# phoreproject/bls

Hardware: AMD Instinct MI355X
Metric: BLS12-381 pairings/sec (batch verify) (higher is better)
Workload: dtype int32 (14 x 28-bit limbs in the pairing / hash / curve kernels, 15 x 27 in the latency programs; int64 accumulate)

## Files before the change

bls_amd/csrc/fp.cuh:

```cuda
#pragma once
#include <hip/hip_runtime.h>
#include <stdint.h>

namespace blsmi {

typedef int32_t i32;
typedef int64_t i64;
typedef uint32_t u32;
typedef uint64_t u64;
typedef uint8_t u8;

#ifdef BLSMI_LIMBS28
constexpr int NL = 14;
constexpr int LB = 28;
constexpr int VU = 2;
constexpr int LMAX = 7;
constexpr int LPROD_MAX = 8;
constexpr int VPROD_MAX = 4096;
constexpr int VSTORE = 22;
#else
constexpr int NL = 15;
constexpr int LB = 27;
constexpr int VU = 1;
constexpr int LMAX = 15;
constexpr int LPROD_MAX = 33;
constexpr int VPROD_MAX = 1 << 23;
constexpr int VSTORE = 256;
#endif
constexpr i32 MASK = (1 << LB) - 1;
constexpr int VMAX = 1 << 12;
constexpr int VMUL = VU + (VU + 1) / 2;
constexpr int VRED = 2 * VU + 1;
#define BLSMI_DEV __device__ __forceinline__
#ifndef BLSMI_HASH_PRIO
#define BLSMI_HASH_PRIO 2
#endif
__device__ __forceinline__ void hash_prio() {
#if BLSMI_HASH_PRIO
    __builtin_amdgcn_s_setprio(BLSMI_HASH_PRIO);
#endif
}

#ifndef BLSMI_PAIR_YIELD_YOUNGER_STAYS
#define BLSMI_PAIR_YIELD_YOUNGER_STAYS 1
#endif
__device__ __forceinline__ void pair_yield_drop() {
#if BLSMI_PAIR_YIELD_YOUNGER_STAYS
    if ((__builtin_amdgcn_s_getreg(4) & 1) == 0)
#endif
        __builtin_amdgcn_s_setprio(0);
}

template <int L_, int V_>
struct Fp {
    static constexpr int L = L_, V = V_;
    i32 v[NL];
};
using FpS = Fp<1, VSTORE>;
using FpC = Fp<1, VU>;

}
#include "tower_fwd.cuh"
#ifdef BLSMI_LIMBS28
#include "consts28.cuh"
#else
#include "consts.cuh"
#endif
namespace blsmi {

template <int L2, int V2, int L, int V>
BLSMI_DEV Fp<L2, V2> fp_relabel(const Fp<L, V>& a) {
    static_assert(L2 >= L && V2 >= V, "relabel may only widen bounds");
    Fp<L2, V2> r;
#pragma unroll
    for (int i = 0; i < NL; i++) r.v[i] = a.v[i];
    return r;
}

template <int L, int V>
BLSMI_DEV Fp<1, V> fp_norm(const Fp<L, V>& x) {
    static_assert(L <= LMAX, "limb bound exceeded before norm");
    Fp<1, V> r;
    if constexpr (L == 1) {
#pragma unroll
        for (int i = 0; i < NL; i++) r.v[i] = x.v[i];
    } else {
        r.v[0] = x.v[0] & MASK;
#pragma unroll
        for (int i = 1; i < NL - 1; i++) r.v[i] = (x.v[i] & MASK) + (x.v[i - 1] >> LB);
        r.v[NL - 1] = x.v[NL - 1] + (x.v[NL - 2] >> LB);
    }
    return r;
}
template <bool C, int L, int V>
BLSMI_DEV auto fp_norm_if(const Fp<L, V>& x) {
    if constexpr (C) return fp_norm(x); else return x;
}

template <int La, int Va, int Lb, int Vb>
BLSMI_DEV auto fp_add(const Fp<La, Va>& a, const Fp<Lb, Vb>& b) {
    if constexpr (La + Lb > LMAX) {
        if constexpr (La >= Lb) return fp_add(fp_norm(a), fp_norm_if<(1 + Lb > LMAX)>(b));
        else return fp_add(fp_norm_if<(La + 1 > LMAX)>(a), fp_norm(b));
    } else {
        static_assert(Va + Vb <= VMAX, "value bound exceeded: insert fp_reduce");
        Fp<La + Lb, Va + Vb> r;
#pragma unroll
        for (int i = 0; i < NL; i++) r.v[i] = a.v[i] + b.v[i];
        return r;
    }
}
template <int La, int Va, int Lb, int Vb>
BLSMI_DEV auto fp_sub(const Fp<La, Va>& a, const Fp<Lb, Vb>& b) {
    if constexpr (La + Lb > LMAX) {
        if constexpr (La >= Lb) return fp_sub(fp_norm(a), fp_norm_if<(1 + Lb > LMAX)>(b));
        else return fp_sub(fp_norm_if<(La + 1 > LMAX)>(a), fp_norm(b));
    } else {
        static_assert(Va + Vb <= VMAX, "value bound exceeded: insert fp_reduce");
        Fp<La + Lb, Va + Vb> r;
#pragma unroll
        for (int i = 0; i < NL; i++) r.v[i] = a.v[i] - b.v[i];
        return r;
    }
}
template <int L, int V>
BLSMI_DEV Fp<L, V> fp_neg(const Fp<L, V>& a) {
    Fp<L, V> r;
#pragma unroll
    for (int i = 0; i < NL; i++) r.v[i] = -a.v[i];
    return r;
}
template <int K, int L, int V>
BLSMI_DEV auto fp_muls(const Fp<L, V>& a) {
    if constexpr (K > LMAX) {
        static_assert(K % 4 == 0 && K / 4 <= LMAX, "factor the constant");
        return fp_muls<K / 4>(fp_norm(fp_muls<4>(a)));
    } else if constexpr (L * K > LMAX) return fp_muls<K>(fp_norm(a));
    else {
        static_assert(V * K <= VMAX, "value bound exceeded: insert fp_reduce");
        Fp<L * K, V * K> r;
#pragma unroll
        for (int i = 0; i < NL; i++) r.v[i] = a.v[i] * K;
        return r;
    }
}
template <int L, int V> BLSMI_DEV auto fp_dbl(const Fp<L, V>& a) { return fp_muls<2>(a); }

template <int L, int V>
BLSMI_DEV Fp<1, VRED> fp_reduce(const Fp<L, V>& x) {
    static_assert(V <= VMAX, "value bound exceeded");
    static_assert(L <= LMAX, "limb bound exceeded before reduce");
    const Fp<L, V>& y = x;
    const float top = (float)y.v[NL - 1] * (float)(1 << LB) + (float)y.v[NL - 2];
    const i32 k = (i32)floorf(top * BLSMI_Q_TOP2_INV);
    Fp<1, VRED> r;
    i64 c = 0;
#pragma unroll
    for (int i = 0; i < NL - 1; i++) {
        c += (i64)y.v[i] - (i64)k * C_Q[i];
        r.v[i] = (i32)c & MASK;
        c >>= LB;
    }
    c += (i64)y.v[NL - 1] - (i64)k * C_Q[NL - 1];
    r.v[NL - 1] = (i32)c;
    return r;
}
template <int VT, int L, int V>
BLSMI_DEV auto fp_fit(const Fp<L, V>& x) {
    if constexpr (V <= VT) return x; else { static_assert(VRED <= VT, "no reduction can make this operand fit"); return fp_reduce(x); }
}
constexpr int isqrt_floor(int n) { int r = 0; while ((long long)(r + 1) * (r + 1) <= n) r++; return r; }
typedef i32 vlimbs __attribute__((ext_vector_type(NL)));

BLSMI_DEV vlimbs fp_mul_body(vlimbs a, vlimbs b) {
    i32 m[NL];
    vlimbs r;
    i64 acc = 0;
#pragma unroll
    for (int k = 0; k < NL; k++) {
#pragma unroll
        for (int i = 0; i <= k; i++) acc += (i64)a[i] * b[k - i];
#pragma unroll
        for (int i = 0; i < k; i++) acc += (i64)m[i] * C_Q[k - i];
        m[k] = (i32)((u32)(i32)acc * BLSMI_QINV) & MASK;
        acc += (i64)m[k] * C_Q[0];
        acc >>= LB;
    }
#pragma unroll
    for (int k = NL; k < 2 * NL - 1; k++) {
#pragma unroll
        for (int i = k - NL + 1; i < NL; i++) acc += (i64)a[i] * b[k - i];
#pragma unroll
        for (int i = k - NL + 1; i < NL; i++) acc += (i64)m[i] * C_Q[k - i];
        r[k - NL] = (i32)acc & MASK;
        acc >>= LB;
    }
    r[NL - 1] = (i32)acc;
    return r;
}
BLSMI_DEV vlimbs fp_sqr_body(vlimbs a) {
    i32 m[NL], a2[NL];
    vlimbs r;
#pragma unroll
    for (int i = 0; i < NL; i++) a2[i] = a[i] * 2;
    i64 acc = 0;
#pragma unroll
    for (int k = 0; k < NL; k++) {
#pragma unroll
        for (int i = 0; 2 * i < k; i++) acc += (i64)a[i] * a2[k - i];
        if (k % 2 == 0) acc += (i64)a[k / 2] * a[k / 2];
#pragma unroll
        for (int i = 0; i < k; i++) acc += (i64)m[i] * C_Q[k - i];
        m[k] = (i32)((u32)(i32)acc * BLSMI_QINV) & MASK;
        acc += (i64)m[k] * C_Q[0];
        acc >>= LB;
    }
#pragma unroll
    for (int k = NL; k < 2 * NL - 1; k++) {
#pragma unroll
        for (int i = k - NL + 1; 2 * i < k; i++) acc += (i64)a[i] * a2[k - i];
        if (k % 2 == 0) acc += (i64)a[k / 2] * a[k / 2];
#pragma unroll
        for (int i = k - NL + 1; i < NL; i++) acc += (i64)m[i] * C_Q[k - i];
        r[k - NL] = (i32)acc & MASK;
        acc >>= LB;
    }
    r[NL - 1] = (i32)acc;
    return r;
}
__device__ __noinline__ vlimbs fp_mul_core(vlimbs a, vlimbs b) { return fp_mul_body(a, b); }
__device__ __noinline__ vlimbs fp_sqr_core(vlimbs a) { return fp_sqr_body(a); }

template <int La, int Va, int Lb, int Vb>
BLSMI_DEV auto fp_mul(const Fp<La, Va>& a, const Fp<Lb, Vb>& b) {
    if constexpr (La * Lb > LPROD_MAX) {
        if constexpr (La >= Lb) return fp_mul(fp_norm(a), b);
        else return fp_mul(a, fp_norm(b));
    } else if constexpr ((long long)Va * Vb > VPROD_MAX) {
        if constexpr (Va >= Vb) return fp_mul(fp_reduce(a), b); else return fp_mul(a, fp_reduce(b));
    } else {
        vlimbs x, y;
#pragma unroll
        for (int i = 0; i < NL; i++) { x[i] = a.v[i]; y[i] = b.v[i]; }
        vlimbs z = fp_mul_core(x, y);
        Fp<1, VMUL> r;
#pragma unroll
        for (int i = 0; i < NL; i++) r.v[i] = z[i];
        return r;
    }
}
template <int L, int V>
BLSMI_DEV auto fp_sqr(const Fp<L, V>& a) {
    if constexpr (2 * L * L > LPROD_MAX) return fp_sqr(fp_norm(a));
    else if constexpr ((long long)V * V > VPROD_MAX) return fp_sqr(fp_reduce(a));
    else {
        vlimbs x;
#pragma unroll
        for (int i = 0; i < NL; i++) x[i] = a.v[i];
        vlimbs z = fp_sqr_core(x);
        Fp<1, VMUL> r;
#pragma unroll
        for (int i = 0; i < NL; i++) r.v[i] = z[i];
        return r;
    }
}

template <int L, int V>
BLSMI_DEV FpS fp_store(const Fp<L, V>& x) {
    if constexpr (V > FpS::V) return fp_relabel<1, FpS::V>(fp_reduce(x));
    else return fp_relabel<1, FpS::V>(fp_norm(x));
}

BLSMI_DEV void limbs_addsub_q(const i32 in[NL], i32 out[NL], i32 addmask, i32 submask) {
    i32 c = 0;
#pragma unroll
    for (int i = 0; i < NL; i++) {
        const i32 s = in[i] + (C_Q[i] & addmask) - (C_Q[i] & submask) + c;
        out[i] = (i < NL - 1) ? (s & MASK) : s;
        c = s >> LB;
    }
}
template <int L, int V>
BLSMI_DEV FpC fp_canon(const Fp<L, V>& x) {
    Fp<1, VRED> r = fp_reduce(x);
    i32 t[NL], d[NL];
    limbs_addsub_q(r.v, t, r.v[NL - 1] >> 31, 0);
#pragma unroll
    for (int pass = 0; pass < 2; pass++) {
        limbs_addsub_q(t, d, 0, -1);
        const i32 lt = d[NL - 1] >> 31;
#pragma unroll
        for (int i = 0; i < NL; i++) t[i] = (t[i] & lt) | (d[i] & ~lt);
    }
    FpC o;
#pragma unroll
    for (int i = 0; i < NL; i++) o.v[i] = t[i];
    return o;
}
template <int L, int V>
BLSMI_DEV bool fp_is_zero(const Fp<L, V>& x) {
    FpC c = fp_canon(x);
    i32 o = 0;
#pragma unroll
    for (int i = 0; i < NL; i++) o |= c.v[i];
    return o == 0;
}
template <int La, int Va, int Lb, int Vb>
BLSMI_DEV bool fp_eq(const Fp<La, Va>& a, const Fp<Lb, Vb>& b) { return fp_is_zero(fp_sub(a, b)); }

template <int L, int V>
BLSMI_DEV Fp<L, V> fp_select(i32 m, const Fp<L, V>& a, const Fp<L, V>& b) {
    Fp<L, V> r;
#pragma unroll
    for (int i = 0; i < NL; i++) r.v[i] = (a.v[i] & m) | (b.v[i] & ~m);
    return r;
}
BLSMI_DEV FpS fp_zero() {
    FpS r;
// ... 249 lines not shown
```

bls_amd/csrc/fp2_pair.inc:

```

template <int L_, int V_> struct Fp2 { static constexpr int L = L_, V = V_; Fp<L_, V_> c; };
template <int L_, int V_> struct Fp6 { static constexpr int L = L_, V = V_; Fp2<L_, V_> c0, c1, c2; };
template <int L_, int V_> struct Fp12 { static constexpr int L = L_, V = V_; Fp6<L_, V_> c0, c1; };
using Fp2S = Fp2<FpS::L, FpS::V>;
using Fp6S = Fp6<FpS::L, FpS::V>;
using Fp12S = Fp12<FpS::L, FpS::V>;

BLSMI_DEV i32 lane_odd() { return -(i32)(threadIdx.x & 1); }
BLSMI_DEV i32 bfi(i32 mask, i32 a, i32 b) {
    i32 r;
    asm("v_bfi_b32 %0, %1, %2, %3" : "=v"(r) : "v"(mask), "v"(a), "v"(b));
    return r;
}
BLSMI_DEV i32 dpp_swap(i32 x) { return __builtin_amdgcn_update_dpp(0, x, 0xB1, 0xf, 0xf, true); }
BLSMI_DEV i32 dpp_even(i32 x) { return __builtin_amdgcn_update_dpp(0, x, 0xA0, 0xf, 0xf, true); }
BLSMI_DEV i32 dpp_odd(i32 x) { return __builtin_amdgcn_update_dpp(0, x, 0xF5, 0xf, 0xf, true); }
template <int L, int V> BLSMI_DEV Fp<L, V> fp_partner(const Fp<L, V>& a) {
    Fp<L, V> r;
#pragma unroll
    for (int i = 0; i < NL; i++) r.v[i] = dpp_swap(a.v[i]);
    return r;
}
template <int L, int V> BLSMI_DEV Fp<L, V> fp_cneg(i32 m, const Fp<L, V>& a) {
    Fp<L, V> r;
#pragma unroll
    for (int i = 0; i < NL; i++) r.v[i] = (a.v[i] ^ m) - m;
    return r;
}
template <int L, int V> BLSMI_DEV Fp2<L, V> wrap(const Fp<L, V>& c) { Fp2<L, V> r; r.c = c; return r; }

template <int L2, int V2, int L, int V>
BLSMI_DEV Fp2<L2, V2> fp2_relabel(const Fp2<L, V>& a) { return wrap(fp_relabel<L2, V2>(a.c)); }
template <int La, int Va, int Lb, int Vb> BLSMI_DEV auto fp2_add(const Fp2<La, Va>& a, const Fp2<Lb, Vb>& b) { return wrap(fp_add(a.c, b.c)); }
template <int La, int Va, int Lb, int Vb> BLSMI_DEV auto fp2_sub(const Fp2<La, Va>& a, const Fp2<Lb, Vb>& b) { return wrap(fp_sub(a.c, b.c)); }
template <int L, int V> BLSMI_DEV auto fp2_neg(const Fp2<L, V>& a) { return wrap(fp_neg(a.c)); }
template <int L, int V> BLSMI_DEV auto fp2_dbl(const Fp2<L, V>& a) { return wrap(fp_dbl(a.c)); }
template <int K, int L, int V> BLSMI_DEV auto fp2_muls(const Fp2<L, V>& a) { return wrap(fp_muls<K>(a.c)); }
template <int L, int V> BLSMI_DEV auto fp2_conj(const Fp2<L, V>& a) { return wrap(fp_cneg(lane_odd(), a.c)); }
template <int L, int V> BLSMI_DEV auto fp2_norm(const Fp2<L, V>& a) { return wrap(fp_norm(a.c)); }
template <int L, int V> BLSMI_DEV Fp2S fp2_store(const Fp2<L, V>& a) { return wrap(fp_store(a.c)); }
template <int L, int V> BLSMI_DEV bool fp2_is_zero(const Fp2<L, V>& a) {
    const int z = fp_is_zero(a.c) ? 1 : 0;
    return (z & __shfl_xor(z, 1)) != 0;
}
template <int La, int Va, int Lb, int Vb> BLSMI_DEV bool fp2_eq(const Fp2<La, Va>& a, const Fp2<Lb, Vb>& b) { return fp2_is_zero(fp2_sub(a, b)); }
template <int L, int V> BLSMI_DEV Fp2<L, V> fp2_select(i32 m, const Fp2<L, V>& a, const Fp2<L, V>& b) { return wrap(fp_select(m, a.c, b.c)); }
BLSMI_DEV Fp2S fp2_zero() { return wrap(fp_zero()); }
BLSMI_DEV Fp2S fp2_one() { return wrap(fp_select(lane_odd(), fp_zero(), fp_one())); }
#undef BLSMI_FP2_K
#define BLSMI_FP2_K(x) fp2_pair_const(x)
#undef BLSMI_FP4_SQR_BY_PRODUCTS
#ifndef BLSMI_FP4_SQR_PAIR
#define BLSMI_FP4_SQR_PAIR 1
#endif
#define BLSMI_FP4_SQR_BY_PRODUCTS BLSMI_FP4_SQR_PAIR
BLSMI_DEV Fp2S fp2_pair_const(const blsmi::Fp2S& k) { return wrap(fp_select(lane_odd(), FpS(k.c1), FpS(k.c0))); }

BLSMI_DEV Fp2S fp2_table_load(const i32* t, int e) {
    const i32* src = t + (2 * e + (threadIdx.x & 1)) * NL_IO;
    FpS r;
#pragma unroll
    for (int i = 0; i < NL; i++) r.v[i] = src[i];
    return wrap(r);
}
BLSMI_DEV void fp2_table_store(i32* t, int e, const Fp2S& a) {
    i32* dst = t + (2 * e + (threadIdx.x & 1)) * NL_IO;
#pragma unroll
    for (int i = 0; i < NL; i++) dst[i] = a.c.v[i];
}
BLSMI_DEV void fp2_table_to_limbs27(i32* t, int e) {
    i32 w[NL_IO];
    fp_to_limbs27(fp2_table_load(t, e).c, w);
    i32* dst = t + (2 * e + (threadIdx.x & 1)) * NL_IO;
#pragma unroll
    for (int i = 0; i < NL_IO; i++) dst[i] = w[i];
}
template <int L, int V> BLSMI_DEV auto fp2_mul_nr(const Fp2<L, V>& a) { return wrap(fp_add(a.c, fp_cneg(~lane_odd(), fp_partner(a.c)))); }

BLSMI_DEV vlimbs fp2p_mul_body(vlimbs am, vlimbs bm, i32 odd) {
    vlimbs ao, p, q;
    const i32 zero = 0;
#pragma unroll
    for (int i = 0; i < NL; i++) {
        ao[i] = dpp_swap(am[i]);
        p[i] = dpp_even(bm[i]);
        q[i] = bfi(odd, bm[i], zero - dpp_swap(bm[i]));
    }
    i32 m[NL];
    vlimbs r;
    i64 acc = 0;
#pragma unroll
    for (int k = 0; k < NL; k++) {
#pragma unroll
        for (int i = 0; i <= k; i++) { acc += (i64)am[i] * p[k - i]; acc += (i64)ao[i] * q[k - i]; }
#pragma unroll
        for (int i = 0; i < k; i++) acc += (i64)m[i] * C_Q[k - i];
        m[k] = (i32)((u32)(i32)acc * BLSMI_QINV) & MASK;
        acc += (i64)m[k] * C_Q[0];
        acc >>= LB;
    }
#pragma unroll
    for (int k = NL; k < 2 * NL - 1; k++) {
#pragma unroll
        for (int i = k - NL + 1; i < NL; i++) { acc += (i64)am[i] * p[k - i]; acc += (i64)ao[i] * q[k - i]; }
#pragma unroll
        for (int i = k - NL + 1; i < NL; i++) acc += (i64)m[i] * C_Q[k - i];
        r[k - NL] = (i32)acc & MASK;
        acc >>= LB;
    }
    r[NL - 1] = (i32)acc;
    return r;
}
#ifdef BLSMI_ASM_CORES
typedef i32 v16i __attribute__((ext_vector_type(16)));
BLSMI_DEV vlimbs fp2p_mul_core(vlimbs a, vlimbs b) BLSMI_CORE_MUL2_STMT(a, b)
#elif defined(BLSMI_PAIR_CORE_INLINE)
BLSMI_DEV vlimbs fp2p_mul_core(vlimbs am, vlimbs bm) { return fp2p_mul_body(am, bm, lane_odd()); }
#else
__device__ __noinline__ vlimbs fp2p_mul_core(vlimbs am, vlimbs bm) { return fp2p_mul_body(am, bm, lane_odd()); }
#endif
BLSMI_DEV vlimbs fp2p_sqr_body(vlimbs am, i32 odd) {
    vlimbs x, y;
#pragma unroll
    for (int i = 0; i < NL; i++) {
        const i32 ao = dpp_swap(am[i]);
        x[i] = am[i] + bfi(odd, am[i], ao);
        y[i] = bfi(odd, ao, am[i] - ao);
    }
    return fp_mul_body(x, y);
}
#ifdef BLSMI_ASM_CORES
BLSMI_DEV vlimbs fp2p_sqr_core(vlimbs a) BLSMI_CORE_SQR2_STMT(a)
#else
__device__ __noinline__ vlimbs fp2p_sqr_core(vlimbs am) { return fp2p_sqr_body(am, lane_odd()); }
#endif
constexpr int LPROD_MAX2 = LPROD_MAX / 2;
template <int La, int Va, int Lb, int Vb>
BLSMI_DEV auto fp2_mul(const Fp2<La, Va>& a, const Fp2<Lb, Vb>& b) {
    if constexpr (La * Lb > LPROD_MAX2) {
        if constexpr (La >= Lb) return fp2_mul(fp2_norm(a), b);
        else return fp2_mul(a, fp2_norm(b));
    } else if constexpr (2LL * Va * Vb > VPROD_MAX) {
        if constexpr (Va >= Vb) return fp2_mul(wrap(fp_reduce(a.c)), b); else return fp2_mul(a, wrap(fp_reduce(b.c)));
    } else {
        vlimbs x, y;
#pragma unroll
        for (int i = 0; i < NL; i++) { x[i] = a.c.v[i]; y[i] = b.c.v[i]; }
        const vlimbs z = fp2p_mul_core(x, y);
        Fp2<1, VMUL> r;
#pragma unroll
        for (int i = 0; i < NL; i++) r.c.v[i] = z[i];
        return r;
    }
}
#ifdef BLSMI_PAIR_CORE_INLINE
__device__ __noinline__ vlimbs fp2p_mul_core_out(vlimbs am, vlimbs bm) { return fp2p_mul_body(am, bm, lane_odd()); }
template <int La, int Va, int Lb, int Vb>
BLSMI_DEV auto fp2_mul_call(const Fp2<La, Va>& a, const Fp2<Lb, Vb>& b) {
    if constexpr (La * Lb > LPROD_MAX2) {
        if constexpr (La >= Lb) return fp2_mul_call(fp2_norm(a), b);
        else return fp2_mul_call(a, fp2_norm(b));
    } else if constexpr (2LL * Va * Vb > VPROD_MAX) {
        if constexpr (Va >= Vb) return fp2_mul_call(wrap(fp_reduce(a.c)), b); else return fp2_mul_call(a, wrap(fp_reduce(b.c)));
    } else {
        vlimbs x, y;
#pragma unroll
        for (int i = 0; i < NL; i++) { x[i] = a.c.v[i]; y[i] = b.c.v[i]; }
        const vlimbs z = fp2p_mul_core_out(x, y);
        Fp2<1, VMUL> r;
#pragma unroll
        for (int i = 0; i < NL; i++) r.c.v[i] = z[i];
        return r;
    }
}
#else
template <int La, int Va, int Lb, int Vb> BLSMI_DEV auto fp2_mul_call(const Fp2<La, Va>& a, const Fp2<Lb, Vb>& b) { return fp2_mul(a, b); }
#endif
template <int L, int V>
BLSMI_DEV auto fp2_sqr(const Fp2<L, V>& a) {
    if constexpr (4 * L * L > LPROD_MAX) return fp2_sqr(fp2_norm(a));
    else if constexpr (4LL * V * V > VPROD_MAX) return fp2_sqr(wrap(fp_reduce(a.c)));
    else {
        vlimbs x;
#pragma unroll
        for (int i = 0; i < NL; i++) x[i] = a.c.v[i];
        const vlimbs z = fp2p_sqr_core(x);
        Fp2<1, VMUL> r;
#pragma unroll
        for (int i = 0; i < NL; i++) r.c.v[i] = z[i];
        return r;
    }
}
template <int La, int Va, int Lb, int Vb>
// ... 77 lines not shown
```

bls_amd/csrc/fp2_single.inc:

```
template <int La, int Va, int Lb, int Vb>
BLSMI_DEV auto make_fp2(const Fp<La, Va>& a, const Fp<Lb, Vb>& b) {
    constexpr int L = imax(La, Lb), V = imax(Va, Vb);
    Fp2<L, V> r;
    r.c0 = fp_relabel<L, V>(a);
    r.c1 = fp_relabel<L, V>(b);
    return r;
}
template <int L2, int V2, int L, int V>
BLSMI_DEV Fp2<L2, V2> fp2_relabel(const Fp2<L, V>& a) {
    Fp2<L2, V2> r;
    r.c0 = fp_relabel<L2, V2>(a.c0);
    r.c1 = fp_relabel<L2, V2>(a.c1);
    return r;
}
template <int La, int Va, int Lb, int Vb> BLSMI_DEV auto fp2_add(const Fp2<La, Va>& a, const Fp2<Lb, Vb>& b) { return make_fp2(fp_add(a.c0, b.c0), fp_add(a.c1, b.c1)); }
template <int La, int Va, int Lb, int Vb> BLSMI_DEV auto fp2_sub(const Fp2<La, Va>& a, const Fp2<Lb, Vb>& b) { return make_fp2(fp_sub(a.c0, b.c0), fp_sub(a.c1, b.c1)); }
template <int L, int V> BLSMI_DEV auto fp2_neg(const Fp2<L, V>& a) { return make_fp2(fp_neg(a.c0), fp_neg(a.c1)); }
template <int L, int V> BLSMI_DEV auto fp2_dbl(const Fp2<L, V>& a) { return make_fp2(fp_dbl(a.c0), fp_dbl(a.c1)); }
template <int K, int L, int V> BLSMI_DEV auto fp2_muls(const Fp2<L, V>& a) { return make_fp2(fp_muls<K>(a.c0), fp_muls<K>(a.c1)); }
template <int L, int V> BLSMI_DEV auto fp2_conj(const Fp2<L, V>& a) { return make_fp2(a.c0, fp_neg(a.c1)); }
template <int L, int V> BLSMI_DEV auto fp2_norm(const Fp2<L, V>& a) { return make_fp2(fp_norm(a.c0), fp_norm(a.c1)); }
template <int L, int V> BLSMI_DEV Fp2S fp2_store(const Fp2<L, V>& a) { Fp2S r; r.c0 = fp_store(a.c0); r.c1 = fp_store(a.c1); return r; }
template <int L, int V> BLSMI_DEV bool fp2_is_zero(const Fp2<L, V>& a) { return fp_is_zero(a.c0) & fp_is_zero(a.c1); }
template <int La, int Va, int Lb, int Vb> BLSMI_DEV bool fp2_eq(const Fp2<La, Va>& a, const Fp2<Lb, Vb>& b) { return fp2_is_zero(fp2_sub(a, b)); }
template <int L, int V> BLSMI_DEV Fp2<L, V> fp2_select(i32 m, const Fp2<L, V>& a, const Fp2<L, V>& b) { Fp2<L, V> r; r.c0 = fp_select(m, a.c0, b.c0); r.c1 = fp_select(m, a.c1, b.c1); return r; }
BLSMI_DEV Fp2S fp2_zero() { Fp2S r; r.c0 = fp_zero(); r.c1 = fp_zero(); return r; }
BLSMI_DEV Fp2S fp2_one() { Fp2S r; r.c0 = fp_one(); r.c1 = fp_zero(); return r; }

template <int L, int V> BLSMI_DEV auto fp2_mul_nr(const Fp2<L, V>& a) { return make_fp2(fp_sub(a.c0, a.c1), fp_add(a.c0, a.c1)); }
template <int La, int Va, int Lb, int Vb>
BLSMI_DEV auto fp2_mul(const Fp2<La, Va>& a, const Fp2<Lb, Vb>& b) {
    const auto aa = fp_mul(a.c0, b.c0);
    const auto bb = fp_mul(a.c1, b.c1);
    const auto t = fp_mul(fp_add(a.c0, a.c1), fp_add(b.c0, b.c1));
    return make_fp2(fp_sub(aa, bb), fp_sub(fp_sub(t, aa), bb));
}
template <int L, int V>
BLSMI_DEV auto fp2_sqr(const Fp2<L, V>& a) {
    const auto ab = fp_mul(a.c0, a.c1);
    const auto c0 = fp_mul(fp_add(a.c0, a.c1), fp_sub(a.c0, a.c1));
    return make_fp2(c0, fp_dbl(ab));
}
template <int La, int Va, int Lb, int Vb>
BLSMI_DEV auto fp2_mul_fp(const Fp2<La, Va>& a, const Fp<Lb, Vb>& s) { return make_fp2(fp_mul(a.c0, s), fp_mul(a.c1, s)); }
template <int L, int V>
BLSMI_DEV auto fp2_inv(const Fp2<L, V>& a) {
    const FpS t = fp_inv(fp_add(fp_sqr(a.c0), fp_sqr(a.c1)));
    return make_fp2(fp_mul(a.c0, t), fp_neg(fp_mul(a.c1, t)));
}
template <int P, int L, int V>
BLSMI_DEV auto fp2_frob(const Fp2<L, V>& a) {
    if constexpr (P % 2 == 0) return a; else return fp2_conj(a);
}

template <int L, int V>
BLSMI_DEV Fp2S fp2_pow_const(const Fp2<L, V>& a, const u32* ebits, int nbits) {
    const Fp2S base = fp2_store(a);
    Fp2S res = base;
    for (int i = nbits - 2; i >= 0; i--) {
        res = fp2_store(fp2_sqr(res));
        if ((ebits[i >> 5] >> (i & 31)) & 1) res = fp2_store(fp2_mul(res, base));
    }
    return res;
}
template <int L, int V>
BLSMI_DEV Fp2S fp2_sqrt(const Fp2<L, V>& a_in, bool& ok) {
    const Fp2S a = fp2_store(a_in);
    const bool zero = fp2_is_zero(a);
    const Fp2S a1 = fp2_pow_const(a, C_QM3O4, BLSMI_QM3O4_BITS);
    const Fp2S alpha = fp2_store(fp2_mul(fp2_sqr(a1), a));
    const Fp2S a0 = fp2_store(fp2_mul(fp2_conj(alpha), alpha));
    Fp2S neg1; neg1.c0 = C_NEGONE; neg1.c1 = fp_zero();
    const bool nonres = fp2_eq(a0, neg1);
    const Fp2S x0 = fp2_store(fp2_mul(a1, a));
    const bool alpha_m1 = fp2_eq(alpha, neg1);
    Fp2S xu; xu.c0 = fp_store(fp_neg(x0.c1)); xu.c1 = x0.c0;
    const Fp2S b = fp2_pow_const(fp2_add(alpha, fp2_one()), C_QM1O2, BLSMI_QM1O2_BITS);
    const Fp2S xb = fp2_store(fp2_mul(b, x0));
    Fp2S r = fp2_select(alpha_m1 ? -1 : 0, xu, xb);
    r = fp2_select(zero ? -1 : 0, fp2_zero(), r);
    ok = zero | !nonres;
    return r;
}

template <int WAVE = 0>
BLSMI_DEV FpS fp2_norm_root(const Fp2S& a, FpS& n, bool& ok) {
    n = fp_store(fp_add(fp_sqr(a.c0), fp_sqr(a.c1)));
    FpS e;
    if constexpr (WAVE != 0) e = fp_pow_spread<WAVE>(n, C_QM3O4, BLSMI_QM3O4_BITS);
    else e = fp_pow_qm3o4(n);
    const FpS s = fp_store(fp_mul(e, n));
    ok = fp_eq(fp_sqr(s), n);
    return s;
}
template <int WAVE = 0>
BLSMI_DEV Fp2S fp2_sqrt_from_norm_root(const Fp2S& a, const FpS& s) {
    FpS d = fp_store(fp_mul(fp_add(a.c0, s), C_HALF));
    d = fp_select(fp_is_zero(d) ? -1 : 0, a.c0, d);
    FpS f;
    if constexpr (WAVE != 0) f = fp_pow_spread<WAVE>(d, C_QM3O4, BLSMI_QM3O4_BITS);
    else f = fp_pow_qm3o4(d);
    const FpS r = fp_store(fp_mul(f, d));
    const FpS h = fp_store(fp_mul(fp_mul(a.c1, f), C_HALF));
    const i32 plus = fp_eq(fp_sqr(r), d) ? -1 : 0;
    Fp2S x;
    x.c0 = fp_select(plus, r, fp_store(fp_neg(h)));
    x.c1 = fp_select(plus, h, r);
    return x;
}
template <int WAVE = 0, int L, int V>
BLSMI_DEV Fp2S fp2_sqrt_any(const Fp2<L, V>& a_in, bool& ok) {
    const Fp2S a = fp2_store(a_in);
    FpS n;
    const FpS s = fp2_norm_root<WAVE>(a, n, ok);
    return fp2_sqrt_from_norm_root<WAVE>(a, s);
}

BLSMI_DEV Fp2S fp2_table_load(const i32* t, int e) {
    Fp2S r;
#pragma unroll
    for (int i = 0; i < NL; i++) { r.c0.v[i] = t[(2 * e) * NL + i]; r.c1.v[i] = t[(2 * e + 1) * NL + i]; }
    return r;
}
BLSMI_DEV void fp2_table_store(i32* t, int e, const Fp2S& a) {
#pragma unroll
    for (int i = 0; i < NL; i++) { t[(2 * e) * NL + i] = a.c0.v[i]; t[(2 * e + 1) * NL + i] = a.c1.v[i]; }
}

#undef BLSMI_FP2_K
#define BLSMI_FP2_K(x) (x)
#undef BLSMI_FP4_SQR_BY_PRODUCTS
#define BLSMI_FP4_SQR_BY_PRODUCTS 0
```

bls_amd/csrc/k_pairing_pair.hip:

```cpp
#include "pairing.cuh"
#include "device_io.cuh"

#define BLSMI_PAIR_MILLER_ONLY
#include "pair_kernels.inc"

template <int W2>
__device__ void pair_rec_load(FpS* c, const u64* p, size_t t, int par) { for (int j = 0; j < W2; j++) c[j] = load_m384(p + (size_t)6 * (2 * W2 * t + 2 * j + par)); }
template <int W2>
__device__ void pair_rec_store(u64* p, size_t t, int par, const FpS* c) { for (int j = 0; j < W2; j++) store_m384(p + (size_t)6 * (2 * W2 * t + 2 * j + par), c[j]); }
__global__ void __launch_bounds__(WG, BLSMI_PAIR_WAVES) k_debug_pairl(int op, const u64* a, const u64* b, u64* out, size_t n) {
    namespace P2 = blsmi::pairl;
    const int par = threadIdx.x & 1;
    const size_t t0 = (size_t)blockIdx.x * (WG / 2) + (threadIdx.x >> 1);
    const size_t t = t0 < n ? t0 : n - 1;
    if (op == BLSMI_OP_ROW_DBL_STEP || op == BLSMI_OP_ROW_ADD_STEP) {
        P2::Fp12S x; pair_rec_load<6>(reinterpret_cast<FpS*>(&x), a, t, par);
        P2::G2Proj r; r.x = x.c0.c0; r.y = x.c0.c1; r.z = x.c0.c2;
        const FpS px = load_m384(a + (size_t)6 * (12 * t + 10)), py = load_m384(a + (size_t)6 * (12 * t + 11));
        P2::Fp2S o0, o1, o2;
        if (op == BLSMI_OP_ROW_DBL_STEP) P2::doubling_step_h(r, o0, o1, o2); else P2::addition_step_h(r, x.c1.c0, x.c1.c1, o0, o1, o2);
        const FpS res[6] = {r.x.c, r.y.c, r.z.c, o2.c, P2::fp2_store(P2::fp2_mul_fp(o1, px)).c, P2::fp2_store(P2::fp2_mul_fp(o0, py)).c};
        if (t0 < n) pair_rec_store<6>(out, t, par, res);
        return;
    }
    if (op < 32) {
        P2::Fp2S x, y, r; pair_rec_load<1>(&x.c, a, t, par); y = x; if (b) pair_rec_load<1>(&y.c, b, t, par);
        switch (op) {
            case BLSMI_OP_FQ2_MUL: r = P2::fp2_store(P2::fp2_mul(x, y)); break;
            case BLSMI_OP_FQ2_SQR: r = P2::fp2_store(P2::fp2_sqr(x)); break;
            case BLSMI_OP_FQ2_INV: r = P2::fp2_store(P2::fp2_inv(x)); break;
            default: r = P2::fp2_store(P2::fp2_mul_nr(x)); break;
        }
        if (t0 < n) pair_rec_store<1>(out, t, par, &r.c);
    } else if (op < 48) {
        P2::Fp6S x, y, r; pair_rec_load<3>(reinterpret_cast<FpS*>(&x), a, t, par); y = x; if (b) pair_rec_load<3>(reinterpret_cast<FpS*>(&y), b, t, par);
        switch (op) {
            case BLSMI_OP_FQ6_MUL: r = P2::fp6_store(P2::fp6_mul(x, y)); break;
            case BLSMI_OP_FQ6_SQR: r = P2::fp6_store(P2::fp6_sqr(x)); break;
            case BLSMI_OP_FQ6_INV: r = P2::fp6_store(P2::fp6_inv(x)); break;
            case BLSMI_OP_FQ6_MUL_BY_1: r = P2::fp6_store(P2::fp6_mul_by_1(x, y.c0)); break;
            case BLSMI_OP_FQ6_MUL_BY_01: r = P2::fp6_store(P2::fp6_mul_by_01(x, y.c0, y.c1)); break;
            default: r = P2::fp6_store(P2::fp6_frob<1>(x)); break;
        }
        if (t0 < n) pair_rec_store<3>(out, t, par, reinterpret_cast<const FpS*>(&r));
    } else {
        P2::Fp12S x, y, r; pair_rec_load<6>(reinterpret_cast<FpS*>(&x), a, t, par); y = x; if (b) pair_rec_load<6>(reinterpret_cast<FpS*>(&y), b, t, par);
        switch (op) {
            case BLSMI_OP_FQ12_MUL: P2::nf_fp12_mul(r, x, y); break;
            case BLSMI_OP_FQ12_SQR: P2::nf_fp12_sqr(r, x); break;
            case BLSMI_OP_FQ12_INV: P2::nf_fp12_inv(r, x); break;
            case BLSMI_OP_FQ12_FROB1: P2::nf_fp12_frob1(r, x); break;
            case BLSMI_OP_FQ12_FROB2: P2::nf_fp12_frob2(r, x); break;
            case BLSMI_OP_FQ12_FROB3: P2::nf_fp12_frob3(r, x); break;
            case BLSMI_OP_FQ12_CYCLO_SQR: P2::nf_fp12_cyc_sqr(r, x); break;
            case BLSMI_OP_FQ12_CYCLO_RUN16: r = P2::cyc_sqr_run(x, 16); break;
            case BLSMI_OP_FQ12_MUL_BY_014: r = P2::fp12_store(P2::fp12_mul_by_014(x, y.c0.c0, y.c0.c1, y.c0.c2)); break;
            default: {
                const P2::LinePair m = P2::line_pair_product(y.c0.c0, y.c0.c1, y.c0.c2, y.c1.c0, y.c1.c1, y.c1.c2);
                r = P2::fp12_store(P2::fp12_mul_by_line_pair(x, m)); break;
            }
        }
        if (t0 < n) pair_rec_store<6>(out, t, par, reinterpret_cast<const FpS*>(&r));
    }
}
__global__ void __launch_bounds__(WG, 2) k_debug_prepare_pair(const u8* g2, i32* table) {
    namespace P2 = blsmi::pairl;
    if (threadIdx.x >= 2) return;
    const int par = threadIdx.x & 1;
    P2::prepare_lines(P2::wrap(load_be48(g2 + 48 * par)), P2::wrap(load_be48(g2 + 96 + 48 * par)), table);
    for (int e = 0; e < 68 * 3; e++) P2::fp2_table_to_limbs27(table, e);
}
__global__ void __launch_bounds__(WG, 2) k_prepare_generator_lines_pair(const u8* g2, i32* table) {
    namespace P2 = blsmi::pairl;
    if (threadIdx.x >= 2) return;
    const int par = threadIdx.x & 1;
    P2::prepare_lines(P2::wrap(load_be48(g2 + 48 * par)), P2::wrap(load_be48(g2 + 96 + 48 * par)), table);
}
```

bls_amd/csrc/k_wire.hip:

```cpp
#include "hash.cuh"
#include "device_io.cuh"
#include "subgroup.cuh"

BLSMI_DEV FpS load_be48_masked(const u8* p) {
    const u32* w32 = reinterpret_cast<const u32*>(p);
    u32 w[12];
#pragma unroll
    for (int j = 0; j < 12; j++) w[j] = __builtin_bswap32(w32[11 - j]);
    w[11] &= 0x1fffffffu;
    return fp_from_words(w);
}
struct WireRecord {
    using out_t = u8; static constexpr bool inf_optional = false;
    static BLSMI_DEV void put(u8* out, size_t t, const G1Aff& a) { store_g1(out + 96 * t, a); }
    static BLSMI_DEV void put(u8* out, size_t t, const G2Aff& a) { store_g2(out + 192 * t, a); }
};
struct JacRecord {
    using out_t = u64; static constexpr bool inf_optional = true;
    static BLSMI_DEV void put(u64* out, size_t t, const G1Aff& a) { store_jac_m384(out + 18 * t, a); }
    static BLSMI_DEV void put(u64* out, size_t t, const G2Aff& a) { store_jac_m384(out + 36 * t, a); }
};
template <bool WAVE, class W = WireRecord>
BLSMI_DEV void g1_decompress_body(const u8* in, int check, typename W::out_t* out, u8* out_inf, u8* err, size_t n) {
    const size_t t = WAVE ? (size_t)blockIdx.x : (size_t)blockIdx.x * WG + threadIdx.x;
// ... 9 lines not shown
    const i32 greatest = (b0 & 0x20) ? -1 : 0;
    G1Aff a; a.x = x; a.y = fp_select(lt ^ greatest, y, fp_store(fp_neg(y))); a.inf = 0;
    const bool sub = check == 2 ? in_subgroup_by_order(a) : check ? in_subgroup(a) : true;
    u8 e = 0; u8 inf = 0;
    if (!(b0 & 0x80)) e = 1;
    else if (b0 & 0x40) { if (rest) e = 2; else inf = 1; }
    else if (!ok) e = 3;
    else if (!sub) e = 4;
    if (t < n && (!WAVE || threadIdx.x == 0)) {
        a.inf = (inf || e) ? -1 : 0;
        W::put(out, t, a);
        if (!W::inf_optional || out_inf) out_inf[t] = inf;
        err[t] = e;
    }
}
KERNEL2 k_g1_decompress(const u8* in, int check, u8* out, u8* out_inf, u8* err, size_t n) { g1_decompress_body<false>(in, check, out, out_inf, err, n); }
KERNEL2 k_g1_decompress_jac(const u8* in, int check, u64* out, u8* out_inf, u8* err, size_t n) { g1_decompress_body<false, JacRecord>(in, check, out, out_inf, err, n); }
__global__ void __launch_bounds__(64, 2) k_g1_decompress_waves(const u8* in, u8* out, u8* out_inf, u8* err, size_t n) { g1_decompress_body<true>(in, 0, out, out_inf, err, n); }
template <bool WAVE, class W = WireRecord>
BLSMI_DEV void g2_decompress_body(const u8* in, int check, typename W::out_t* out, u8* out_inf, u8* err, size_t n) {
    const size_t t = WAVE ? (size_t)blockIdx.x : (size_t)blockIdx.x * WG + threadIdx.x;
    const size_t tt = t < n ? t : n - 1;
    const u8* c = in + 96 * tt;
    const u8 b0 = c[0];
    u32 rest = b0 & 0x3f;
    for (int i = 1; i < 96; i++) rest |= c[i];
    Fp2S x; x.c1 = load_be48_masked(c); x.c0 = load_be48(c + 48);
    bool ok;
    const Fp2S y = fp2_sqrt_any<WAVE>(fp2_add(fp2_mul(fp2_sqr(x), x), C_B2), ok);
    const i32 lt = ~fp2_sign_is_neg(y);
    const i32 greatest = (b0 & 0x20) ? -1 : 0;
    G2Aff a; a.x = x; a.y = fp2_select(lt ^ greatest, y, fp2_store(fp2_neg(y))); a.inf = 0;
    const bool sub = check == 2 ? in_subgroup_by_order(a) : check ? in_subgroup(a) : true;
    u8 e = 0; u8 inf = 0;
    if (!(b0 & 0x80)) e = 1;
    else if (b0 & 0x40) { if (rest) e = 2; else inf = 1; }
    else if (!ok) e = 3;
    else if (!sub) e = 4;
    if (t < n && (!WAVE || threadIdx.x == 0)) {
        a.inf = (inf || e) ? -1 : 0;
        W::put(out, t, a);
        if (!W::inf_optional || out_inf) out_inf[t] = inf;
        err[t] = e;
    }
}
KERNEL k_g2_decompress(const u8* in, int check, u8* out, u8* out_inf, u8* err, size_t n) { g2_decompress_body<false>(in, check, out, out_inf, err, n); }
KERNEL k_g2_decompress_jac(const u8* in, int check, u64* out, u8* out_inf, u8* err, size_t n) { g2_decompress_body<false, JacRecord>(in, check, out, out_inf, err, n); }
__global__ void __launch_bounds__(64) k_g2_decompress_waves(const u8* in, u8* out, u8* out_inf, u8* err, size_t n) { g2_decompress_body<true>(in, 0, out, out_inf, err, n); }
KERNEL k_apply_subgroup(const u8* in_subgroup, u8* out, int rec_words, const u8* out_inf, u8* err, size_t n) {
    const size_t t = (size_t)blockIdx.x * WG + threadIdx.x;
    if (t >= n || err[t] || out_inf[t] || in_subgroup[t]) return;
    err[t] = 4;
    u32* w = reinterpret_cast<u32*>(out) + (size_t)rec_words * t;
    for (int i = 0; i < rec_words; i++) w[i] = 0;
}
KERNEL k_merge_flags(const u8* inf_pk, const u8* err_pk, const u8* inf_sig, const u8* err_sig, u8* flags, size_t n) {
    const size_t t = (size_t)blockIdx.x * WG + threadIdx.x;
    if (t < n) flags[t] = (u8)(((inf_pk[t] | err_pk[t]) ? 1 : 0) | ((inf_sig[t] | err_sig[t]) ? 2 : 0));
}
KERNEL k_flag_zero_records(const u8* pks, int pk_words, const u8* sigs, int sig_words, const u8* in_flags, u8* flags, int* any, size_t n) {
    const size_t t = (size_t)blockIdx.x * WG + threadIdx.x;
    if (t >= n) return;
    u32 a = 0, b = 1;
    const u32* p = reinterpret_cast<const u32*>(pks) + (size_t)pk_words * t;
    for (int i = 0; i < pk_words; i++) a |= p[i];
    if (sigs) {
        b = 0;
        const u32* q = reinterpret_cast<const u32*>(sigs) + (size_t)sig_words * t;
        for (int i = 0; i < sig_words; i++) b |= q[i];
    }
    const u8 f = (u8)((in_flags ? in_flags[t] : 0) | (a ? 0 : 1) | (b ? 0 : 2));
    flags[t] = f;
    if (f && any) atomicOr(any, 1);
}
KERNEL k_flag_to_byte(const i32* flag, u8* out) { if (blockIdx.x == 0 && threadIdx.x == 0) *out = *flag ? 1 : 0; }
KERNEL k_pack_bitmap(const u8* ok, u8* bitmap, size_t n) {
    const size_t b = (size_t)blockIdx.x * WG + threadIdx.x;
    if (8 * b >= n) return;
    u32 v = 0;
    for (int i = 0; i < 8; i++) if (8 * b + i < n && ok[8 * b + i]) v |= 1u << i;
    bitmap[b] = (u8)v;
}
KERNEL k_g1_compress(const u8* pts, const u8* in_inf, u8* out, size_t n) {
    const size_t t = (size_t)blockIdx.x * WG + threadIdx.x;
    if (t >= n) return;
    u8* o = out + 48 * t;
    if (in_inf && in_inf[t]) { for (int i = 0; i < 48; i++) o[i] = 0; o[0] = 0xc0; return; }
    const u8* p = pts + 96 * t;
    for (int i = 0; i < 48; i++) o[i] = p[i];
    const FpS y = load_be48(p + 48);
    o[0] |= 0x80 | (fp_gt_half(y) ? 0x20 : 0);
}
KERNEL k_g2_compress(const u8* pts, const u8* in_inf, u8* out, size_t n) {
    const size_t t = (size_t)blockIdx.x * WG + threadIdx.x;
    if (t >= n) return;
    u8* o = out + 96 * t;
    if (in_inf && in_inf[t]) { for (int i = 0; i < 96; i++) o[i] = 0; o[0] = 0xc0; return; }
    const u8* p = pts + 192 * t;
    for (int i = 0; i < 48; i++) { o[i] = p[48 + i]; o[48 + i] = p[i]; }
    Fp2S y; y.c0 = load_be48(p + 96); y.c1 = load_be48(p + 144);
    o[0] |= 0x80 | (fp2_sign_is_neg(y) ? 0x20 : 0);
}

template <class F, int PB>
BLSMI_DEV void jac_to_affine_body(const u64* in, u8* out, u8* out_inf, size_t n) {
    constexpr int NC = sizeof(F) / sizeof(FpS);
    const size_t t = (size_t)blockIdx.x * WG + threadIdx.x;
    const size_t tt = t < n ? t : n - 1;
    bool z_one;
    const Jac<F> j = load_jac_m384<F>(in + (size_t)18 * NC * tt, &z_one);
    Aff<F> a;
    if (__all(z_one || j.inf)) { a.x = j.x; a.y = j.y; a.inf = j.inf; }
    else a = jac_to_affine(j);
    if (t < n) {
        if constexpr (NC == 1) store_g1(out + (size_t)PB * t, a); else store_g2(out + (size_t)PB * t, a);
        if (out_inf) out_inf[t] = a.inf ? 1 : 0;
    }
}
KERNEL2 k_g1_jac_to_affine(const u64* in, u8* out, u8* out_inf, size_t n) { jac_to_affine_body<FpS, 96>(in, out, out_inf, n); }
KERNEL k_g2_jac_to_affine(const u64* in, u8* out, u8* out_inf, size_t n) { jac_to_affine_body<Fp2S, 192>(in, out, out_inf, n); }
template <class F>
BLSMI_DEV void compress_jac_body(const u64* in, u8* out, size_t n) {
    constexpr int NC = sizeof(F) / sizeof(FpS);
    const size_t t = (size_t)blockIdx.x * WG + threadIdx.x;
    const size_t tt = t < n ? t : n - 1;
    bool z_one;
    const Jac<F> j = load_jac_m384<F>(in + (size_t)18 * NC * tt, &z_one);
    Aff<F> a;
    if (__all(z_one || j.inf)) { a.x = j.x; a.y = j.y; a.inf = j.inf; }
    else a = jac_to_affine(j);
    if (t >= n) return;
    u8* o = out + (size_t)48 * NC * t;
    if constexpr (NC == 1) store_wire48(o, a.x, a.inf, a.inf ? 0xc0u : 0x80u | (fp_gt_half(a.y) ? 0x20u : 0u));
    else {
        store_wire48(o, a.x.c1, a.inf, a.inf ? 0xc0u : 0x80u | (fp2_sign_is_neg(a.y) ? 0x20u : 0u));
        store_wire48(o + 48, a.x.c0, a.inf, 0u);
    }
}
KERNEL2 k_g1_compress_jac(const u64* in, u8* out, size_t n) { compress_jac_body<FpS>(in, out, n); }
KERNEL k_g2_compress_jac(const u64* in, u8* out, size_t n) { compress_jac_body<Fp2S>(in, out, n); }
KERNEL k_affine_to_jac(const u8* in, const void* in_inf, int inf_u8, int group, u64* out, size_t n) {
    const size_t t = (size_t)blockIdx.x * WG + threadIdx.x;
    if (t >= n) return;
    const bool inf = in_inf && (inf_u8 ? static_cast<const u8*>(in_inf)[t] != 0 : static_cast<const i32*>(in_inf)[t] != 0);
    if (group == 1) { G1Aff a = load_g1(in + 96 * t); if (inf) a.inf = -1; store_jac_m384(out + 18 * t, a); }
    else { G2Aff a = load_g2(in + 192 * t); if (inf) a.inf = -1; store_jac_m384(out + 36 * t, a); }
}

KERNEL k_debug_fq(int op, const u64* a, const u64* b, u64* out, u8* flag, size_t n) {
    const size_t t = (size_t)blockIdx.x * WG + threadIdx.x;
    if (t >= n) return;
    const FpS x = load_m384(a + 6 * t);
    FpS y = fp_zero();
    if (op == BLSMI_OP_FQ_MUL || op == BLSMI_OP_FQ_ADD || op == BLSMI_OP_FQ_SUB || op == BLSMI_OP_FQ_CMP) y = load_m384(b + 6 * t);
    FpS r = fp_zero();
    bool ok = true;
    int code = -1;
    switch (op) {
        case BLSMI_OP_FQ_DBL: r = fp_store(fp_dbl(x)); break;
        case BLSMI_OP_FQ_CMP: {
            u32 wx[12], wy[12];
            fp_to_words(x, wx); fp_to_words(y, wy);
            int c = 0;
            for (int j = 0; j < 12; j++) if (wx[j] != wy[j]) c = wx[j] > wy[j] ? 1 : -1;
            code = c + 1; r = x; break;
        }
        case BLSMI_OP_FQ_PARITY: code = fp_gt_half(x) ? 1 : 0; r = x; break;
        case BLSMI_OP_FQ_MUL: r = fp_store(fp_mul(x, y)); break;
        case BLSMI_OP_FQ_SQR: r = fp_store(fp_sqr(x)); break;
        case BLSMI_OP_FQ_ADD: r = fp_store(fp_add(x, y)); break;
        case BLSMI_OP_FQ_SUB: r = fp_store(fp_sub(x, y)); break;
        case BLSMI_OP_FQ_NEG: r = fp_store(fp_neg(x)); break;
        case BLSMI_OP_FQ_INV: r = fp_inv(x); ok = !fp_is_zero(x); break;
        case BLSMI_OP_FQ_SQRT: r = fp_sqrt(x, ok); break;
    }
    store_m384(out + 6 * t, r);
    if (flag) flag[t] = code >= 0 ? (u8)code : (ok ? 1 : 0);
}
KERNEL k_debug_fq2(int op, const u64* a, const u64* b, u64* out, u8* flag, size_t n) {
    const size_t t = (size_t)blockIdx.x * WG + threadIdx.x;
    if (t >= n) return;
    Rec<2> ra = rec_load<2>(a, t), rb = ra, ro;
    if (op == BLSMI_OP_FQ2_MUL) rb = rec_load<2>(b, t);
    const Fp2S x = as<Fp2S>(ra), y = as<Fp2S>(rb);
    Fp2S r = fp2_zero();
    bool ok = true;
    switch (op) {
        case BLSMI_OP_FQ2_MUL: r = fp2_store(fp2_mul(x, y)); break;
        case BLSMI_OP_FQ2_SQR: r = fp2_store(fp2_sqr(x)); break;
        case BLSMI_OP_FQ2_INV: r = fp2_store(fp2_inv(x)); ok = !fp2_is_zero(x); break;
        case BLSMI_OP_FQ2_MUL_NR: r = fp2_store(fp2_mul_nr(x)); break;
        case BLSMI_OP_FQ2_SQRT: r = fp2_sqrt(x, ok); break;
        case BLSMI_OP_FQ2_SQRT_ANY: r = fp2_sqrt_any(x, ok); break;
        case BLSMI_OP_FQ2_PARITY: ok = fp2_sign_is_neg(x) != 0; r = x; break;
    }
    as<Fp2S>(ro) = r;
    rec_store<2>(out, t, ro);
    if (flag) flag[t] = ok ? 1 : 0;
}
KERNEL2 k_debug_swu_g1(const u64* a, u64* out, size_t n) {
    const size_t t = (size_t)blockIdx.x * WG + threadIdx.x;
    if (t >= n) return;
    Rec<3> r = rec_load<3>(a, t);
    G1Aff p; swu_g1_helper(p, reinterpret_cast<FpS*>(&r)[0]);
    reinterpret_cast<FpS*>(&r)[0] = p.x; reinterpret_cast<FpS*>(&r)[1] = p.y; reinterpret_cast<FpS*>(&r)[2] = fp_zero();
    rec_store<3>(out, t, r);
}
KERNEL k_debug_swu_g2(const u64* a, u64* out, size_t n) {
    const size_t t = (size_t)blockIdx.x * WG + threadIdx.x;
    if (t >= n) return;
    Rec<6> r = rec_load<6>(a, t);
    G2Aff p; swu_g2_helper(p, reinterpret_cast<Fp2S*>(&r)[0]);
    reinterpret_cast<Fp2S*>(&r)[0] = p.x; reinterpret_cast<Fp2S*>(&r)[1] = p.y; reinterpret_cast<Fp2S*>(&r)[2] = fp2_zero();
    rec_store<6>(out, t, r);
}
```

bls_amd/csrc/pair_kernels.inc:

```
#ifndef BLSMI_PAIR_WAVES
#define BLSMI_PAIR_WAVES 2
#endif
#define KERNEL_PAIR __global__ void __launch_bounds__(WG, BLSMI_PAIR_WAVES)
namespace P2 = blsmi::pairl;
struct PairG1 { FpS x, y; };
struct PairG2 { P2::Fp2S x, y; };
constexpr int PT = WG / 2;

#ifndef BLSMI_PAIR_YIELD
#define BLSMI_PAIR_YIELD 1
#endif
#ifndef BLSMI_PAIR_YIELD_MILLER
#define BLSMI_PAIR_YIELD_MILLER 50
#endif
#ifndef BLSMI_PAIR_YIELD_FE
#define BLSMI_PAIR_YIELD_FE 4
#endif
constexpr int PAIR_YIELD_MILLER_BITS = BLSMI_PAIR_YIELD ? BLSMI_PAIR_YIELD_MILLER : 0;
constexpr int PAIR_YIELD_FE_EXP_X = BLSMI_PAIR_YIELD_FE;
BLSMI_DEV void pair_yield_enter() {
#if BLSMI_PAIR_YIELD
    __builtin_amdgcn_s_setprio(1);
#endif
}
struct PairYieldOps : P2::Fp12Ops {
    static BLSMI_DEV void before_exp_x(int k) { if (k == PAIR_YIELD_FE_EXP_X) pair_yield_drop(); }
};
BLSMI_DEV void final_exponentiation_yield(P2::Fp12S& f) {
#if BLSMI_PAIR_YIELD
    P2::final_exp_chain<PairYieldOps>(f);
#else
    P2::final_exponentiation(f);
#endif
}

#ifdef BLSMI_WAVE_CENSUS
constexpr int CENSUS_WAVES = 4096, CENSUS_WORDS = 4;
#ifdef BLSMI_PAIR_FE_ONLY
#define BLSMI_CENSUS_BUF blsmi_census_fe
#define BLSMI_CENSUS_READ blsmi_census_read_fe
#else
#define BLSMI_CENSUS_BUF blsmi_census_miller
#define BLSMI_CENSUS_READ blsmi_census_read_miller
#endif
__device__ unsigned long long BLSMI_CENSUS_BUF[CENSUS_WAVES * CENSUS_WORDS];
extern "C" __attribute__((visibility("default"))) int BLSMI_CENSUS_READ(unsigned long long* out) {
    return (int)hipMemcpyFromSymbol(out, HIP_SYMBOL(BLSMI_CENSUS_BUF), sizeof(BLSMI_CENSUS_BUF));
}
struct WaveCensus {
    u64 t0;
    BLSMI_DEV WaveCensus() : t0(__builtin_amdgcn_s_memrealtime()) {}
    BLSMI_DEV void leave(int kernel) const {
        const u64 t1 = __builtin_amdgcn_s_memrealtime();
        const u32 hw = __builtin_amdgcn_s_getreg(4 | (31 << 11)), xcc = __builtin_amdgcn_s_getreg(20 | (31 << 11));
        if (threadIdx.x == 0 && blockIdx.x < CENSUS_WAVES) {
            unsigned long long* rec = BLSMI_CENSUS_BUF + (size_t)blockIdx.x * CENSUS_WORDS;
            rec[0] = (u64)hw | ((u64)xcc << 32); rec[1] = t0; rec[2] = t1; rec[3] = (u64)kernel + 1;
        }
    }
};
#else
struct WaveCensus { BLSMI_DEV void leave(int) const {} };
#endif

template <int WORDS>
BLSMI_DEV void tile_load_pair(u32* lds, const u8* gbase, size_t first, size_t n) {
    const u32* g = reinterpret_cast<const u32*>(gbase) + first * WORDS;
    const size_t valid = (n - first < (size_t)PT ? n - first : (size_t)PT) * WORDS;
    for (int idx = threadIdx.x; idx < PT * WORDS; idx += WG)
        if ((size_t)idx < valid) lds[(idx / WORDS) * (WORDS + 1) + (idx % WORDS)] = g[idx];
    __syncthreads();
}
template <int WORDS>
BLSMI_DEV void tile_store_pair(const u32* lds, u8* gbase, size_t first, size_t n) {
    __syncthreads();
    u32* g = reinterpret_cast<u32*>(gbase) + first * WORDS;
    const size_t valid = (n - first < (size_t)PT ? n - first : (size_t)PT) * WORDS;
    for (int idx = threadIdx.x; idx < PT * WORDS; idx += WG)
        if ((size_t)idx < valid) g[idx] = lds[(idx / WORDS) * (WORDS + 1) + (idx % WORDS)];
}
BLSMI_DEV void pair_store12(i32* buf, size_t n, size_t t, int par, const P2::Fp12S& f) {
    const FpS* c = reinterpret_cast<const FpS*>(&f);
#pragma unroll
    for (int j = 0; j < 6; j++) soa_store(buf, n, t, 2 * j + par, c[j]);
}
BLSMI_DEV P2::Fp12S pair_load12(const i32* buf, size_t n, size_t t, int par) {
    P2::Fp12S f;
    FpS* c = reinterpret_cast<FpS*>(&f);
#pragma unroll
    for (int j = 0; j < 6; j++) c[j] = soa_load(buf, n, t, 2 * j + par);
    return f;
}
#ifndef BLSMI_PAIR_FE_ONLY
template <bool EXACT> BLSMI_DEV void miller1_pair_body(const u8* g1, const u8* g2, i32* fbuf, size_t n) {
    __shared__ u32 lds[PT * 49];
    const int par = threadIdx.x & 1, loc = threadIdx.x >> 1;
    const size_t first = (size_t)blockIdx.x * PT;
    const size_t t = first + loc;
    const int rec = (t < n) ? loc : (int)(n - 1 - first);
    PairG1 p[1]; PairG2 q[1];
    const WaveCensus census;
    pair_yield_enter();
    tile_load_pair<24>(lds, g1, first, n);
    p[0].x = lds_be48(lds + rec * 25); p[0].y = lds_be48(lds + rec * 25 + 12);
    __syncthreads();
    tile_load_pair<48>(lds, g2, first, n);
    q[0].x = P2::wrap(lds_be48(lds + rec * 49 + 12 * par));
    q[0].y = P2::wrap(lds_be48(lds + rec * 49 + 24 + 12 * par));
    P2::Fp12S f;
    if constexpr (EXACT) P2::miller_loop<1, false, EXACT, false, PAIR_YIELD_MILLER_BITS>(f, p, q);
    else {
        __shared__ i32 lds_r[45 * WG];
        __syncthreads();
        P2::miller_loop<1, false, EXACT, false, PAIR_YIELD_MILLER_BITS>(f, p, q, nullptr, nullptr, lds_r);
    }
    if (t < n) pair_store12(fbuf, n, t, par, f);
    census.leave(0);
}
KERNEL_PAIR k_miller1_pair(const u8* g1, const u8* g2, i32* fbuf, size_t n) { miller1_pair_body<true>(g1, g2, fbuf, n); }
KERNEL_PAIR k_miller1h_pair(const u8* g1, const u8* g2, i32* fbuf, size_t n) { miller1_pair_body<false>(g1, g2, fbuf, n); }
#endif
#ifndef BLSMI_PAIR_MILLER_ONLY
KERNEL_PAIR k_final_exp_pair(const i32* fbuf, u64* out, size_t n, int mode) {
    __shared__ u32 lds[PT * 145];
    const int par = threadIdx.x & 1, loc = threadIdx.x >> 1;
    const size_t first = (size_t)blockIdx.x * PT;
    const size_t t = first + loc;
    const size_t tt = t < n ? t : n - 1;
    const WaveCensus census;
    pair_yield_enter();
    P2::Fp12S f = pair_load12(fbuf, n, tt, par);
    if (mode == 0) final_exponentiation_yield(f);
    const FpS* c = reinterpret_cast<const FpS*>(&f);
    for (int j = 0; j < 6; j++) {
        u32 w[12];
        fp_to_mont384_words(c[j], w);
#pragma unroll
        for (int k = 0; k < 12; k++) lds[loc * 145 + 12 * (2 * j + par) + k] = w[k];
    }
    tile_store_pair<144>(lds, reinterpret_cast<u8*>(out), first, n);
    census.leave(1);
}
#endif
#ifndef BLSMI_PAIR_FE_ONLY

KERNEL_PAIR k_miller1x2_pair(const u8* g1, const u8* g2, i32* fbuf, size_t n, size_t m) {
    const int par = threadIdx.x & 1;
    const size_t t = (size_t)blockIdx.x * PT + (threadIdx.x >> 1);
    const size_t tt = t < m ? t : m - 1;
    const size_t i0 = 2 * tt, i1 = 2 * tt + 1 < n ? 2 * tt + 1 : i0;
    PairG1 p[2]; PairG2 q[2];
    p[0].x = load_be48(g1 + 96 * i0); p[0].y = load_be48(g1 + 96 * i0 + 48);
    p[1].x = load_be48(g1 + 96 * i1); p[1].y = load_be48(g1 + 96 * i1 + 48);
    q[0].x = P2::wrap(load_be48(g2 + 192 * i0 + 48 * par)); q[0].y = P2::wrap(load_be48(g2 + 192 * i0 + 96 + 48 * par));
    q[1].x = P2::wrap(load_be48(g2 + 192 * i1 + 48 * par)); q[1].y = P2::wrap(load_be48(g2 + 192 * i1 + 96 + 48 * par));
    P2::Fp12S f;
    __shared__ i32 lds_r[45 * WG];
    if (__all(2 * tt + 1 < n)) P2::miller_loop<2, false, false>(f, p, q, nullptr, nullptr, lds_r);
    else {
        P2::Fp12S f2, f1;
        P2::miller_loop<2, false, false>(f2, p, q, nullptr, nullptr, lds_r);
        PairG1 p1[1] = {p[0]}; PairG2 q1[1] = {q[0]};
        P2::miller_loop<1, false, false>(f1, p1, q1, nullptr, nullptr, lds_r);
        const i32 both = 2 * tt + 1 < n ? -1 : 0;
        FpS* a = reinterpret_cast<FpS*>(&f2); const FpS* b = reinterpret_cast<const FpS*>(&f1);
        for (int j = 0; j < 6; j++) a[j] = fp_select(both, a[j], b[j]);
        f = f2;
    }
    if (t < m) pair_store12(fbuf, m, t, par, f);
}

KERNEL_PAIR k_miller2_pair(const u8* p0, size_t sp0, const u8* q0, size_t sq0, const u8* p1, size_t sp1, const u8* q1, size_t sq1, i32* fbuf, size_t n, const i32* pre) {
    __shared__ u32 lds[PT * 49];
    const int par = threadIdx.x & 1, loc = threadIdx.x >> 1;
    const size_t first = (size_t)blockIdx.x * PT;
    const size_t t = first + loc;
    const int rec = (t < n) ? loc : (int)(n - 1 - first);
    PairG1 p[2]; PairG2 q[2];
    const WaveCensus census;
    pair_yield_enter();
    if (sp0) { tile_load_pair<24>(lds, p0, first, n); p[0].x = lds_be48(lds + rec * 25); p[0].y = lds_be48(lds + rec * 25 + 12); __syncthreads(); }
    else { p[0].x = load_be48(p0); p[0].y = load_be48(p0 + 48); }
    if (sq0) { tile_load_pair<48>(lds, q0, first, n); q[0].x = P2::wrap(lds_be48(lds + rec * 49 + 12 * par)); q[0].y = P2::wrap(lds_be48(lds + rec * 49 + 24 + 12 * par)); __syncthreads(); }
    else { q[0].x = P2::wrap(load_be48(q0 + 48 * par)); q[0].y = P2::wrap(load_be48(q0 + 96 + 48 * par)); }
    tile_load_pair<24>(lds, p1, first, n);
    p[1].x = lds_be48(lds + rec * 25); p[1].y = fp_store(fp_neg(lds_be48(lds + rec * 25 + 12)));
    __syncthreads();
    tile_load_pair<48>(lds, q1, first, n);
    q[1].x = P2::wrap(lds_be48(lds + rec * 49 + 12 * par)); q[1].y = P2::wrap(lds_be48(lds + rec * 49 + 24 + 12 * par));
    (void)sp1; (void)sq1;
    P2::Fp12S f;
    __shared__ i32 lds_r[45 * WG];
    __syncthreads();
    if (pre) P2::miller_loop<2, true, false, false, PAIR_YIELD_MILLER_BITS>(f, p, q, pre, nullptr, lds_r);
    else P2::miller_loop<2, false, false, false, PAIR_YIELD_MILLER_BITS>(f, p, q, nullptr, nullptr, lds_r);
    if (t < n) pair_store12(fbuf, n, t, par, f);
    census.leave(2);
}
#endif
#ifndef BLSMI_PAIR_MILLER_ONLY
KERNEL_PAIR k_final_exp_is_one_pair(const i32* fbuf, const u8* inf_flags, u8* ok, size_t n) {
    const int par = threadIdx.x & 1, loc = threadIdx.x >> 1;
    const size_t t = (size_t)blockIdx.x * PT + loc;
    const size_t tt = t < n ? t : n - 1;
    const WaveCensus census;
    pair_yield_enter();
    P2::Fp12S f = pair_load12(fbuf, n, tt, par);
    final_exponentiation_yield(f);
    const bool one = P2::fp12_eq(f, P2::fp12_one());
    if (t < n && par == 0) ok[t] = (one && !(inf_flags && inf_flags[t])) ? 1 : 0;
    census.leave(3);
}
#endif
```

bls_amd/csrc/pairing_body.inc:

```

struct G2Proj { Fp2S x, y, z; };

BLSMI_NOINLINE void nf_fp12_mul(Fp12S& r, const Fp12S& a, const Fp12S& b) { r = fp12_store(fp12_mul(a, b)); }
BLSMI_NOINLINE void nf_fp12_sqr(Fp12S& r, const Fp12S& a) { r = fp12_store(fp12_sqr(a)); }
BLSMI_NOINLINE void nf_fp12_cyc_sqr(Fp12S& r, const Fp12S& a) { r = fp12_cyclotomic_sqr(a); }
BLSMI_NOINLINE void nf_fp12_inv(Fp12S& r, const Fp12S& a) { r = fp12_store(fp12_inv(a)); }
BLSMI_NOINLINE void nf_fp12_frob1(Fp12S& r, const Fp12S& a) { r = fp12_store(fp12_frob<1>(a)); }
BLSMI_NOINLINE void nf_fp12_frob2(Fp12S& r, const Fp12S& a) { r = fp12_store(fp12_frob<2>(a)); }
BLSMI_NOINLINE void nf_fp12_frob3(Fp12S& r, const Fp12S& a) { r = fp12_store(fp12_frob<3>(a)); }
BLSMI_DEV void fp12_conj_inplace(Fp12S& a) { a.c1 = fp6_store(fp6_neg(a.c1)); }

BLSMI_NOINLINE void doubling_step(G2Proj& r, Fp2S& o0, Fp2S& o1, Fp2S& o2) {
    const auto tmp0 = fp2_norm(fp2_sqr(r.x));
    const auto tmp1 = fp2_norm(fp2_sqr(r.y));
    const auto tmp2 = fp2_norm(fp2_sqr(tmp1));
    const auto tmp3 = fp2_norm(fp2_dbl(fp2_sub(fp2_sub(fp2_sqr(fp2_add(tmp1, r.x)), tmp0), tmp2)));
    const auto tmp4 = fp2_norm(fp2_muls<3>(tmp0));
    const auto tmp6 = fp2_norm(fp2_add(r.x, tmp4));
    const auto tmp5 = fp2_norm(fp2_sqr(tmp4));
    const auto zsq = fp2_norm(fp2_sqr(r.z));
    const auto nx = fp2_norm(fp2_sub(fp2_sub(tmp5, tmp3), tmp3));
    const auto nz = fp2_norm(fp2_sub(fp2_sub(fp2_sqr(fp2_add(r.z, r.y)), tmp1), zsq));
    const auto ny = fp2_norm(fp2_sub(fp2_mul(fp2_sub(tmp3, nx), tmp4), fp2_muls<8>(tmp2)));
    o1 = fp2_store(fp2_neg(fp2_dbl(fp2_mul(tmp4, zsq))));
    o2 = fp2_store(fp2_sub(fp2_sub(fp2_sub(fp2_sqr(tmp6), tmp0), tmp5), fp2_muls<4>(tmp1)));
    o0 = fp2_store(fp2_dbl(fp2_mul(nz, zsq)));
    r.x = fp2_store(nx); r.y = fp2_store(ny); r.z = fp2_store(nz);
}
BLSMI_NOINLINE void addition_step(G2Proj& r, const Fp2S& qx, const Fp2S& qy, Fp2S& o0, Fp2S& o1, Fp2S& o2) {
    const auto zsq = fp2_norm(fp2_sqr(r.z));
    const auto ysq = fp2_norm(fp2_sqr(qy));
    const auto t0 = fp2_norm(fp2_mul(zsq, qx));
    const auto t1 = fp2_norm(fp2_mul(fp2_sub(fp2_sub(fp2_sqr(fp2_add(qy, r.z)), ysq), zsq), zsq));
    const auto t2 = fp2_norm(fp2_sub(t0, r.x));
    const auto t3 = fp2_norm(fp2_sqr(t2));
    const auto t4 = fp2_norm(fp2_muls<4>(t3));
    const auto t5 = fp2_norm(fp2_mul(t4, t2));
    const auto t6 = fp2_norm(fp2_sub(fp2_sub(t1, r.y), r.y));
    const auto t9 = fp2_norm(fp2_mul(t6, qx));
    const auto t7 = fp2_norm(fp2_mul(t4, r.x));
    const auto nx = fp2_norm(fp2_sub(fp2_sub(fp2_sub(fp2_sqr(t6), t5), t7), t7));
    const auto nz = fp2_norm(fp2_sub(fp2_sub(fp2_sqr(fp2_add(r.z, t2)), zsq), t3));
    const auto t8 = fp2_norm(fp2_mul(fp2_sub(t7, nx), t6));
    const auto ny = fp2_norm(fp2_sub(t8, fp2_dbl(fp2_mul(r.y, t5))));
    const auto t10 = fp2_norm(fp2_sub(fp2_sub(fp2_sqr(fp2_add(qy, nz)), ysq), fp2_sqr(nz)));
    o2 = fp2_store(fp2_sub(fp2_dbl(t9), t10));
    o0 = fp2_store(fp2_dbl(nz));
    o1 = fp2_store(fp2_dbl(fp2_neg(t6)));
    r.x = fp2_store(nx); r.y = fp2_store(ny); r.z = fp2_store(nz);
}
BLSMI_DEV void doubling_step_h_i(G2Proj& r, Fp2S& o0, Fp2S& o1, Fp2S& o2) {
    const auto A = fp2_norm(fp2_mul(r.x, r.y));
    const auto B = fp2_norm(fp2_sqr(r.y));
    const auto X2 = fp2_norm(fp2_sqr(r.x));
    const auto H = fp2_norm(fp2_dbl(fp2_mul(r.y, r.z)));
    const auto E = fp2_norm(fp2_muls<12>(fp2_norm(fp2_mul_nr(fp2_norm(fp2_sqr(r.z))))));
    const auto F = fp2_norm(fp2_muls<3>(E));
    const auto G = fp2_norm(fp2_add(B, F));
    const auto nx = fp2_norm(fp2_dbl(fp2_mul(A, fp2_norm(fp2_sub(B, F)))));
    const auto ny = fp2_norm(fp2_sub(fp2_sqr(G), fp2_muls<12>(fp2_norm(fp2_sqr(E)))));
    const auto nz = fp2_norm(fp2_muls<4>(fp2_norm(fp2_mul(B, H))));
    o2 = fp2_store(fp2_sub(B, E));
    o1 = fp2_store(fp2_neg(fp2_muls<3>(X2)));
    o0 = fp2_store(H);
    r.x = fp2_store(nx); r.y = fp2_store(ny); r.z = fp2_store(nz);
}
BLSMI_NOINLINE void doubling_step_h(G2Proj& r, Fp2S& o0, Fp2S& o1, Fp2S& o2) { doubling_step_h_i(r, o0, o1, o2); }
BLSMI_NOINLINE void addition_step_h(G2Proj& r, const Fp2S& qx, const Fp2S& qy, Fp2S& o0, Fp2S& o1, Fp2S& o2) {
    const auto th = fp2_norm(fp2_sub(r.y, fp2_mul(qy, r.z)));
    const auto la = fp2_norm(fp2_sub(r.x, fp2_mul(qx, r.z)));
    const auto C = fp2_norm(fp2_sqr(th));
    const auto D = fp2_norm(fp2_sqr(la));
    const auto E = fp2_norm(fp2_mul(la, D));
    const auto F = fp2_norm(fp2_mul(r.z, C));
    const auto G = fp2_norm(fp2_mul(r.x, D));
    const auto Hh = fp2_norm(fp2_sub(fp2_add(E, F), fp2_dbl(G)));
    const auto nx = fp2_norm(fp2_mul(la, Hh));
    const auto ny = fp2_norm(fp2_sub(fp2_mul(th, fp2_norm(fp2_sub(G, Hh))), fp2_mul(E, r.y)));
    const auto nz = fp2_norm(fp2_mul(r.z, E));
    o2 = fp2_store(fp2_sub(fp2_mul(th, qx), fp2_mul(la, qy)));
    o1 = fp2_store(fp2_neg(th));
    o0 = fp2_store(la);
    r.x = fp2_store(nx); r.y = fp2_store(ny); r.z = fp2_store(nz);
}
template <bool EXACT> BLSMI_DEV void dbl_step(G2Proj& r, Fp2S& o0, Fp2S& o1, Fp2S& o2) {
    if constexpr (EXACT) doubling_step(r, o0, o1, o2); else doubling_step_h(r, o0, o1, o2);
}
template <bool EXACT> BLSMI_DEV void add_step(G2Proj& r, const Fp2S& qx, const Fp2S& qy, Fp2S& o0, Fp2S& o1, Fp2S& o2) {
    if constexpr (EXACT) addition_step(r, qx, qy, o0, o1, o2); else addition_step_h(r, qx, qy, o0, o1, o2);
}
BLSMI_NOINLINE void ell(Fp12S& f, const Fp2S& o0, const Fp2S& o1, const Fp2S& o2, const FpS& px, const FpS& py) {
    const auto c0 = fp2_mul_fp(o0, py);
    const auto c1 = fp2_mul_fp(o1, px);
    f = fp12_store(fp12_mul_by_014(f, o2, c1, c0));
}

BLSMI_NOINLINE void ell_sqr(Fp12S& f, const Fp2S& o0, const Fp2S& o1, const Fp2S& o2, const FpS& px, const FpS& py) {
    const auto c0 = fp2_mul_fp(o0, py);
    const auto c1 = fp2_mul_fp(o1, px);
    const Fp12S g = fp12_store(fp12_mul_by_014(f, o2, c1, c0));
    f = fp12_store(fp12_sqr(g));
}

template <bool SQR>
BLSMI_NOINLINE void ell2(Fp12S& f, const Fp2S& a0, const Fp2S& a1, const Fp2S& a2, const FpS& ax, const FpS& ay,
                         const Fp2S& b0, const Fp2S& b1, const Fp2S& b2, const FpS& bx, const FpS& by) {
    const LinePair m = line_pair_product(a2, fp2_mul_fp(a1, ax), fp2_mul_fp(a0, ay), b2, fp2_mul_fp(b1, bx), fp2_mul_fp(b0, by));
    const Fp12S g = fp12_store(fp12_mul_by_line_pair(f, m));
    if (SQR) f = fp12_store(fp12_sqr(g)); else f = g;
}

struct NoTick { BLSMI_DEV void operator()(int) const {} };
template <class Dbl, class Add, class Mul, class MulSqr, class Tick = NoTick>
BLSMI_DEV void x_bit_walk(Dbl dbl, Add add, Mul mul, MulSqr mul_sqr, Tick tick = Tick()) {
    const u64 xr = BLSMI_X_ABS >> 1;
    for (int i = 61; i >= 0; i--) {
        tick(61 - i);
        dbl();
        if ((xr >> i) & 1) { mul(); add(); }
        mul_sqr();
    }
    dbl();
    mul();
}

BLSMI_DEV void load_line(const i32* pre, int line, Fp2S& o0, Fp2S& o1, Fp2S& o2) {
    o0 = fp2_table_load(pre, 3 * line); o1 = fp2_table_load(pre, 3 * line + 1); o2 = fp2_table_load(pre, 3 * line + 2);
}
BLSMI_DEV void store_line(i32* table, int line, const Fp2S& o0, const Fp2S& o1, const Fp2S& o2) {
    fp2_table_store(table, 3 * line, o0); fp2_table_store(table, 3 * line + 1, o1); fp2_table_store(table, 3 * line + 2, o2);
}
BLSMI_DEV void lds_put_proj(i32* l, const G2Proj& r) {
    const FpS* c = reinterpret_cast<const FpS*>(&r);
#pragma unroll
    for (int j = 0; j < 3; j++)
#pragma unroll
        for (int i = 0; i < NL; i++) l[(j * NL + i) * 64 + threadIdx.x] = c[j].v[i];
}
BLSMI_DEV G2Proj lds_get_proj(const i32* l) {
    G2Proj r;
    FpS* c = reinterpret_cast<FpS*>(&r);
#pragma unroll
    for (int j = 0; j < 3; j++)
#pragma unroll
        for (int i = 0; i < NL; i++) c[j].v[i] = l[(j * NL + i) * 64 + threadIdx.x];
    return r;
}
template <int NP, bool PRE0 = false, bool EXACT = true, bool PRE1 = false, int YIELD = 0, class G1P, class G2P>
BLSMI_DEV void miller_loop(Fp12S& f, const G1P (&p)[NP], const G2P (&q)[NP], const i32* pre = nullptr, const i32* pre1 = nullptr, i32* lds_r = nullptr) {
    static_assert(NP == 1 || NP == 2, "one pair, or two pairs sharing the squarings");
    constexpr int LAST = NP - 1;
    constexpr bool PRE_LAST = NP == 1 ? PRE0 : PRE1;
    G2Proj r[NP];
#pragma unroll
    for (int k = 0; k < NP; k++) { r[k].x = q[k].x; r[k].y = q[k].y; r[k].z = fp2_one(); }
    f = fp12_one();
    const bool in_lds = !EXACT && !PRE_LAST && lds_r != nullptr;
    if (in_lds) lds_put_proj(lds_r, r[LAST]);
    auto dbl_last = [&](Fp2S& a0, Fp2S& a1, Fp2S& a2) {
        if (in_lds) { G2Proj t = lds_get_proj(lds_r); doubling_step_h_i(t, a0, a1, a2); lds_put_proj(lds_r, t); }
        else dbl_step<EXACT>(r[LAST], a0, a1, a2);
    };
    auto add_last = [&](Fp2S& a0, Fp2S& a1, Fp2S& a2) {
        if (in_lds) { G2Proj t = lds_get_proj(lds_r); add_step<EXACT>(t, q[LAST].x, q[LAST].y, a0, a1, a2); lds_put_proj(lds_r, t); }
        else add_step<EXACT>(r[LAST], q[LAST].x, q[LAST].y, a0, a1, a2);
    };
    Fp2S o0, o1, o2;
    int line = 0;
    auto tick = [](int done) {
        if constexpr (YIELD > 0) { if (done == YIELD) pair_yield_drop(); }
        else (void)done;
    };
    if constexpr (NP == 1) {
        x_bit_walk([&] { if (PRE0) load_line(pre, line++, o0, o1, o2); else dbl_last(o0, o1, o2); },
                   [&] { if (PRE0) load_line(pre, line++, o0, o1, o2); else add_last(o0, o1, o2); },
                   [&] { ell(f, o0, o1, o2, p[0].x, p[0].y); },
                   [&] { ell_sqr(f, o0, o1, o2, p[0].x, p[0].y); }, tick);
    } else {
        Fp2S n0, n1, n2;
        int line1 = 0;
        x_bit_walk([&] { if (PRE0) load_line(pre, line++, o0, o1, o2); else dbl_step<EXACT>(r[0], o0, o1, o2);
                         if (PRE1) load_line(pre1, line1++, n0, n1, n2); else dbl_last(n0, n1, n2); },
                   [&] { if (PRE0) load_line(pre, line++, o0, o1, o2); else add_step<EXACT>(r[0], q[0].x, q[0].y, o0, o1, o2);
                         if (PRE1) load_line(pre1, line1++, n0, n1, n2); else add_last(n0, n1, n2); },
                   [&] { ell2<false>(f, o0, o1, o2, p[0].x, p[0].y, n0, n1, n2, p[1].x, p[1].y); },
                   [&] { ell2<true>(f, o0, o1, o2, p[0].x, p[0].y, n0, n1, n2, p[1].x, p[1].y); }, tick);
    }
    fp12_conj_inplace(f);
}
BLSMI_DEV void prepare_lines(const Fp2S& qx, const Fp2S& qy, i32* table) {
    G2Proj r; r.x = qx; r.y = qy; r.z = fp2_one();
    Fp2S o0, o1, o2;
    int line = 0;
    x_bit_walk([&] { doubling_step(r, o0, o1, o2); store_line(table, line++, o0, o1, o2); },
               [&] { addition_step(r, qx, qy, o0, o1, o2); store_line(table, line++, o0, o1, o2); },
               [] {}, [] {});
}

template <class O>
BLSMI_DEV void exp_by_x_loop(typename O::T& out, const typename O::T& f, u64 e) {
    typename O::T res = f;
    int i = 62 - __builtin_clzll(e);
    while (i >= 0) {
        const u64 below = e & ((2ull << i) - 1);
        const int next = below ? 63 - __builtin_clzll(below) : -1;
        const int run = next < 0 ? i + 1 : i - next + 1;
        bool plain = true;
        if constexpr (O::MIN_RUN > 0)
            if (run >= O::MIN_RUN) { O::x_sqr_run(res, res, run); plain = false; }
        if (plain) for (int j = 0; j < run; j++) O::x_sqr(res, res);
        if (next >= 0) { typename O::T t = res; O::mul(t, t, f); res = t; }
        i = next - 1;
        if (next < 0) break;
    }
    O::conj(res);
    out = res;
}
template <class O, class = void> struct ExpXHook { static BLSMI_DEV void at(int) {} };
template <class O> struct ExpXHook<O, decltype(O::before_exp_x(0))> { static BLSMI_DEV void at(int k) { O::before_exp_x(k); } };
template <class O>
BLSMI_DEV void final_exp_chain(typename O::T& r) {
    typename O::T f2, y0, y1, y2, y3;
    O::inv(f2, r);
    O::conj(r);
    O::mul(r, r, f2);
    O::frob2(f2, r);
    O::mul(r, f2, r);
    const u64 x = BLSMI_X_ABS;
    O::cyc_sqr(y0, r);
    ExpXHook<O>::at(0); O::exp_x(y1, y0, x);
    ExpXHook<O>::at(1); O::exp_x(y2, y1, x >> 1);
    y3 = r; O::conj(y3);
    O::mul(y1, y1, y3);
    O::conj(y1);
    O::mul(y1, y1, y2);
    ExpXHook<O>::at(2); O::exp_x(y2, y1, x);
    ExpXHook<O>::at(3); O::exp_x(y3, y2, x);
    O::conj(y1);
    O::mul(y3, y3, y1);
    O::conj(y1);
    O::frob3(y1, y1);
    O::frob2(y2, y2);
    O::mul(y1, y1, y2);
    ExpXHook<O>::at(4); O::exp_x(y2, y3, x);
    O::mul(y2, y2, y0);
    O::mul(y2, y2, r);
    O::mul(y1, y1, y2);
    O::frob1(y3, y3);
    O::mul(r, y1, y3);
}

BLSMI_DEV Fp12S cyc_sqr_run(const Fp12S& g, int m) {
    CycCompressed c = cyc_compress(g);
    for (int j = 0; j < m; j++) c = cyc_compressed_sqr(c);
    Fp2S num, den;
    cyc_z1_fraction(c, num, den);
    return cyc_decompress(c, fp2_store(fp2_mul(num, fp2_store(fp2_inv(den)))));
}
BLSMI_NOINLINE void exp_by_x(Fp12S& out, const Fp12S& f, u64 e);
struct Fp12Ops {
    using T = Fp12S;
    static constexpr int MIN_RUN = 12;
    static BLSMI_DEV void inv(T& r, const T& a) { nf_fp12_inv(r, a); }
    static BLSMI_DEV void mul(T& r, const T& a, const T& b) { nf_fp12_mul(r, a, b); }
    static BLSMI_DEV void cyc_sqr(T& r, const T& a) { nf_fp12_cyc_sqr(r, a); }
    static BLSMI_DEV void x_sqr(T& r, const T& a) { r = fp12_cyclotomic_sqr(a); }
    static BLSMI_DEV void x_sqr_run(T& r, const T& a, int m) { r = cyc_sqr_run(a, m); }
    static BLSMI_DEV void frob1(T& r, const T& a) { nf_fp12_frob1(r, a); }
    static BLSMI_DEV void frob2(T& r, const T& a) { nf_fp12_frob2(r, a); }
    static BLSMI_DEV void frob3(T& r, const T& a) { nf_fp12_frob3(r, a); }
    static BLSMI_DEV void conj(T& a) { fp12_conj_inplace(a); }
    static BLSMI_DEV void exp_x(T& r, const T& a, u64 e) { exp_by_x(r, a, e); }
};
BLSMI_NOINLINE void exp_by_x(Fp12S& out, const Fp12S& f, u64 e) { exp_by_x_loop<Fp12Ops>(out, f, e); }
BLSMI_DEV void final_exponentiation(Fp12S& r) { final_exp_chain<Fp12Ops>(r); }
```

bls_amd/csrc/tower_body.inc:

```
template <int L2, int V2, int L, int V>
BLSMI_DEV Fp6<L2, V2> fp6_relabel(const Fp6<L, V>& a) {
    Fp6<L2, V2> r;
    r.c0 = fp2_relabel<L2, V2>(a.c0);
    r.c1 = fp2_relabel<L2, V2>(a.c1);
    r.c2 = fp2_relabel<L2, V2>(a.c2);
    return r;
}
template <int La, int Va, int Lb, int Vb, int Lc, int Vc>
BLSMI_DEV auto make_fp6(const Fp2<La, Va>& a, const Fp2<Lb, Vb>& b, const Fp2<Lc, Vc>& c) {
    constexpr int L = imax(La, imax(Lb, Lc)), V = imax(Va, imax(Vb, Vc));
    Fp6<L, V> r;
    r.c0 = fp2_relabel<L, V>(a);
    r.c1 = fp2_relabel<L, V>(b);
    r.c2 = fp2_relabel<L, V>(c);
    return r;
}
template <int La, int Va, int Lb, int Vb>
BLSMI_DEV auto make_fp12(const Fp6<La, Va>& a, const Fp6<Lb, Vb>& b) {
    constexpr int L = imax(La, Lb), V = imax(Va, Vb);
    Fp12<L, V> r;
    r.c0 = fp6_relabel<L, V>(a);
    r.c1 = fp6_relabel<L, V>(b);
    return r;
}

template <int La, int Va, int Lb, int Vb> BLSMI_DEV auto fp6_add(const Fp6<La, Va>& a, const Fp6<Lb, Vb>& b) { return make_fp6(fp2_add(a.c0, b.c0), fp2_add(a.c1, b.c1), fp2_add(a.c2, b.c2)); }
template <int La, int Va, int Lb, int Vb> BLSMI_DEV auto fp6_sub(const Fp6<La, Va>& a, const Fp6<Lb, Vb>& b) { return make_fp6(fp2_sub(a.c0, b.c0), fp2_sub(a.c1, b.c1), fp2_sub(a.c2, b.c2)); }
template <int L, int V> BLSMI_DEV auto fp6_neg(const Fp6<L, V>& a) { return make_fp6(fp2_neg(a.c0), fp2_neg(a.c1), fp2_neg(a.c2)); }
template <int L, int V> BLSMI_DEV auto fp6_norm(const Fp6<L, V>& a) { return make_fp6(fp2_norm(a.c0), fp2_norm(a.c1), fp2_norm(a.c2)); }
template <int L, int V> BLSMI_DEV Fp6S fp6_store(const Fp6<L, V>& a) { Fp6S r; r.c0 = fp2_store(a.c0); r.c1 = fp2_store(a.c1); r.c2 = fp2_store(a.c2); return r; }
BLSMI_DEV Fp6S fp6_zero() { Fp6S r; r.c0 = fp2_zero(); r.c1 = fp2_zero(); r.c2 = fp2_zero(); return r; }
BLSMI_DEV Fp6S fp6_one() { Fp6S r; r.c0 = fp2_one(); r.c1 = fp2_zero(); r.c2 = fp2_zero(); return r; }
template <int L, int V> BLSMI_DEV auto fp6_mul_nr(const Fp6<L, V>& a) { return make_fp6(fp2_mul_nr(a.c2), a.c0, a.c1); }
template <int La, int Va, int Lb, int Vb>
BLSMI_DEV auto fp6_mul(const Fp6<La, Va>& a, const Fp6<Lb, Vb>& b) {
    const auto aa = fp2_mul(a.c0, b.c0);
    const auto bb = fp2_mul(a.c1, b.c1);
    const auto cc = fp2_mul(a.c2, b.c2);
    const auto t1 = fp2_add(fp2_mul_nr(fp2_sub(fp2_sub(fp2_mul(fp2_add(b.c1, b.c2), fp2_add(a.c1, a.c2)), bb), cc)), aa);
    const auto t3 = fp2_sub(fp2_add(fp2_sub(fp2_mul(fp2_add(b.c0, b.c2), fp2_add(a.c0, a.c2)), aa), bb), cc);
    const auto t2 = fp2_add(fp2_sub(fp2_sub(fp2_mul(fp2_add(b.c0, b.c1), fp2_add(a.c0, a.c1)), aa), bb), fp2_mul_nr(cc));
    return make_fp6(t1, t2, t3);
}
template <int L, int V>
BLSMI_DEV auto fp6_sqr(const Fp6<L, V>& a) {
    const auto s0 = fp2_sqr(a.c0);
    const auto s1 = fp2_dbl(fp2_mul(a.c0, a.c1));
    const auto s2 = fp2_sqr(fp2_add(fp2_sub(a.c0, a.c1), a.c2));
    const auto s3 = fp2_dbl(fp2_mul(a.c1, a.c2));
    const auto s4 = fp2_sqr(a.c2);
    const auto c0 = fp2_add(fp2_mul_nr(s3), s0);
    const auto c1 = fp2_add(fp2_mul_nr(s4), s1);
    const auto c2 = fp2_sub(fp2_sub(fp2_add(fp2_add(s1, s2), s3), s0), s4);
    return make_fp6(c0, c1, c2);
}
template <int L, int V, int Lc, int Vc>
BLSMI_DEV auto fp6_mul_by_1(const Fp6<L, V>& a, const Fp2<Lc, Vc>& c1) {
    const auto b = fp2_mul(a.c1, c1);
    const auto t1 = fp2_mul_nr(fp2_sub(fp2_mul(c1, fp2_add(a.c1, a.c2)), b));
    const auto t2 = fp2_sub(fp2_mul(c1, fp2_add(a.c0, a.c1)), b);
    return make_fp6(t1, t2, b);
}
template <int L, int V, int L0, int V0, int L1, int V1>
BLSMI_DEV auto fp6_mul_by_01(const Fp6<L, V>& a, const Fp2<L0, V0>& c0, const Fp2<L1, V1>& c1) {
    const auto aa = fp2_mul(a.c0, c0);
    const auto b = fp2_mul(a.c1, c1);
    const auto t1 = fp2_add(fp2_mul_nr(fp2_sub(fp2_mul(c1, fp2_add(a.c1, a.c2)), b)), aa);
    const auto t3 = fp2_add(fp2_sub(fp2_mul(c0, fp2_add(a.c0, a.c2)), aa), b);
    const auto t2 = fp2_sub(fp2_sub(fp2_mul(fp2_add(c0, c1), fp2_add(a.c0, a.c1)), aa), b);
    return make_fp6(t1, t2, t3);
}
template <int L, int V>
BLSMI_DEV auto fp6_inv(const Fp6<L, V>& a) {
    const Fp2S c0 = fp2_store(fp2_add(fp2_neg(fp2_mul(fp2_mul_nr(a.c2), a.c1)), fp2_sqr(a.c0)));
    const Fp2S c1 = fp2_store(fp2_sub(fp2_mul_nr(fp2_sqr(a.c2)), fp2_mul(a.c0, a.c1)));
    const Fp2S c2 = fp2_store(fp2_sub(fp2_sqr(a.c1), fp2_mul(a.c0, a.c2)));
    auto t = fp2_mul_nr(fp2_add(fp2_mul(a.c2, c1), fp2_mul(a.c1, c2)));
    const Fp2S ti = fp2_store(fp2_inv(fp2_store(fp2_add(t, fp2_mul(a.c0, c0)))));
    return make_fp6(fp2_mul(ti, c0), fp2_mul(ti, c1), fp2_mul(ti, c2));
}
template <int P, int L, int V>
BLSMI_DEV auto fp6_frob(const Fp6<L, V>& a) {
    return make_fp6(fp2_frob<P>(a.c0), fp2_mul(fp2_frob<P>(a.c1), BLSMI_FP2_K(C_FROB6_C1[P % 6])), fp2_mul(fp2_frob<P>(a.c2), BLSMI_FP2_K(C_FROB6_C2[P % 6])));
}

template <int L, int V> BLSMI_DEV Fp12S fp12_store(const Fp12<L, V>& a) { Fp12S r; r.c0 = fp6_store(a.c0); r.c1 = fp6_store(a.c1); return r; }
BLSMI_DEV Fp12S fp12_one() { Fp12S r; r.c0 = fp6_one(); r.c1 = fp6_zero(); return r; }
template <int L, int V> BLSMI_DEV auto fp12_conj(const Fp12<L, V>& a) { return make_fp12(a.c0, fp6_neg(a.c1)); }
template <int La, int Va, int Lb, int Vb>
BLSMI_DEV auto fp12_mul(const Fp12<La, Va>& a, const Fp12<Lb, Vb>& b) {
    const auto aa = fp6_norm(fp6_mul(a.c0, b.c0));
    const auto bb = fp6_norm(fp6_mul(a.c1, b.c1));
    const auto t = fp6_mul(fp6_add(a.c1, a.c0), fp6_add(b.c0, b.c1));
    return make_fp12(fp6_add(fp6_mul_nr(bb), aa), fp6_sub(fp6_sub(t, aa), bb));
}
template <int L, int V>
BLSMI_DEV auto fp12_sqr(const Fp12<L, V>& a) {
    const auto ab = fp6_norm(fp6_mul(a.c0, a.c1));
    const auto t = fp6_mul(fp6_add(fp6_mul_nr(a.c1), a.c0), fp6_add(a.c0, a.c1));
    return make_fp12(fp6_sub(fp6_sub(t, ab), fp6_mul_nr(ab)), fp6_add(ab, ab));
}
template <int L, int V, int L0, int V0, int L1, int V1, int L4, int V4>
BLSMI_DEV auto fp12_mul_by_014(const Fp12<L, V>& a, const Fp2<L0, V0>& c0, const Fp2<L1, V1>& c1, const Fp2<L4, V4>& c4) {
    const auto aa = fp6_norm(fp6_mul_by_01(a.c0, c0, c1));
    const auto bb = fp6_norm(fp6_mul_by_1(a.c1, c4));
    const auto t = fp6_mul_by_01(fp6_add(a.c1, a.c0), c0, fp2_add(c1, c4));
    return make_fp12(fp6_add(fp6_mul_nr(bb), aa), fp6_sub(fp6_sub(t, aa), bb));
}
template <int L, int V>
BLSMI_DEV auto fp12_inv(const Fp12<L, V>& a) {
    const Fp6S t = fp6_store(fp6_inv(fp6_store(fp6_sub(fp6_sqr(a.c0), fp6_mul_nr(fp6_store(fp6_sqr(a.c1)))))));
    return make_fp12(fp6_mul(t, a.c0), fp6_neg(fp6_mul(t, a.c1)));
}
template <int P, int L, int V>
BLSMI_DEV auto fp12_frob(const Fp12<L, V>& a) {
    const auto c0 = fp6_frob<P>(a.c0);
    const auto c1 = fp6_frob<P>(a.c1);
    const Fp2S k = BLSMI_FP2_K(C_FROB12_C1[P % 12]);
    return make_fp12(c0, make_fp6(fp2_mul(fp2_store(c1.c0), k), fp2_mul(fp2_store(c1.c1), k), fp2_mul(fp2_store(c1.c2), k)));
}
struct LinePair { Fp2S l0, l1, l2, l4, l5; };
template <int L0, int V0, int L1, int V1, int L4, int V4, int M0, int W0, int M1, int W1, int M4, int W4>
BLSMI_DEV LinePair line_pair_product(const Fp2<L0, V0>& a0, const Fp2<L1, V1>& a1, const Fp2<L4, V4>& a4,
                                     const Fp2<M0, W0>& b0, const Fp2<M1, W1>& b1, const Fp2<M4, W4>& b4) {
    const auto p00 = fp2_norm(fp2_mul(a0, b0)), p11 = fp2_norm(fp2_mul(a1, b1)), p44 = fp2_norm(fp2_mul(a4, b4));
    LinePair r;
    r.l0 = fp2_store(fp2_add(p00, fp2_mul_nr(p44)));
    r.l1 = fp2_store(fp2_sub(fp2_sub(fp2_mul(fp2_add(a0, a1), fp2_add(b0, b1)), p00), p11));
    r.l2 = fp2_store(p11);
    r.l4 = fp2_store(fp2_sub(fp2_sub(fp2_mul(fp2_add(a0, a4), fp2_add(b0, b4)), p00), p44));
    r.l5 = fp2_store(fp2_sub(fp2_sub(fp2_mul(fp2_add(a1, a4), fp2_add(b1, b4)), p11), p44));
    return r;
}
template <int L, int V>
BLSMI_DEV auto fp6_mul_by_12(const Fp6<L, V>& a, const Fp2S& b1, const Fp2S& b2) {
    const auto p11 = fp2_norm(fp2_mul(a.c1, b1)), p22 = fp2_norm(fp2_mul(a.c2, b2));
    const auto cross = fp2_sub(fp2_sub(fp2_mul(fp2_add(a.c1, a.c2), fp2_add(b1, b2)), p11), p22);
    const auto c0 = fp2_mul_nr(cross);
    const auto c1 = fp2_add(fp2_mul(a.c0, b1), fp2_mul_nr(p22));
    const auto c2 = fp2_add(fp2_mul(a.c0, b2), p11);
    return make_fp6(c0, c1, c2);
}
template <int L, int V>
BLSMI_DEV auto fp12_mul_by_line_pair(const Fp12<L, V>& f, const LinePair& m) {
    const Fp6S m0 = make_fp6(m.l0, m.l1, m.l2);
    const auto t0 = fp6_norm(fp6_mul(f.c0, m0));
    const auto t1 = fp6_norm(fp6_mul_by_12(f.c1, m.l4, m.l5));
    const auto m01 = make_fp6(m.l0, fp2_add(m.l1, m.l4), fp2_add(m.l2, m.l5));
    const auto t2 = fp6_mul(fp6_add(f.c0, f.c1), m01);
    return make_fp12(fp6_add(fp6_mul_nr(t1), t0), fp6_sub(fp6_sub(t2, t0), t1));
}
template <class A, class B> struct Pair { A first; B second; };
template <int La, int Va, int Lb, int Vb>
BLSMI_DEV auto fp4_sqr(const Fp2<La, Va>& a, const Fp2<Lb, Vb>& b) {
#if BLSMI_FP4_SQR_BY_PRODUCTS
    const auto v = fp2_mul(a, b);
    const auto c0 = fp2_sub(fp2_sub(fp2_mul(fp2_add(a, b), fp2_add(a, fp2_mul_nr(b))), v), fp2_mul_nr(v));
    const auto c1 = fp2_dbl(v);
    return Pair<decltype(c0), decltype(c1)>{c0, c1};
#else
    const auto t0 = fp2_norm(fp2_sqr(a));
    const auto t1 = fp2_norm(fp2_sqr(b));
    const auto c0 = fp2_add(fp2_mul_nr(t1), t0);
    const auto c1 = fp2_sub(fp2_sub(fp2_sqr(fp2_add(a, b)), t0), t1);
    return Pair<decltype(c0), decltype(c1)>{c0, c1};
#endif
}
BLSMI_DEV Fp12S fp12_cyclotomic_sqr(const Fp12S& f) {
    const Fp2S z0 = f.c0.c0, z4 = f.c0.c1, z3 = f.c0.c2, z2 = f.c1.c0, z1 = f.c1.c1, z5 = f.c1.c2;
    Fp12S r;
    const auto a = fp4_sqr(z0, z1);
    r.c0.c0 = fp2_store(fp2_add(fp2_dbl(fp2_sub(a.first, z0)), a.first));
    r.c1.c1 = fp2_store(fp2_add(fp2_dbl(fp2_add(a.second, z1)), a.second));
    const auto b = fp4_sqr(z2, z3);
    const auto c = fp4_sqr(z4, z5);
    r.c0.c1 = fp2_store(fp2_add(fp2_dbl(fp2_sub(b.first, z4)), b.first));
    r.c1.c2 = fp2_store(fp2_add(fp2_dbl(fp2_add(b.second, z5)), b.second));
    const auto t3n = fp2_mul_nr(c.second);
    r.c1.c0 = fp2_store(fp2_add(fp2_dbl(fp2_add(t3n, z2)), t3n));
    r.c0.c2 = fp2_store(fp2_add(fp2_dbl(fp2_sub(c.first, z3)), c.first));
    return r;
}
struct CycCompressed { Fp2S z2, z3, z4, z5; };
BLSMI_DEV CycCompressed cyc_compress(const Fp12S& f) {
    CycCompressed c; c.z4 = f.c0.c1; c.z3 = f.c0.c2; c.z2 = f.c1.c0; c.z5 = f.c1.c2; return c;
}
BLSMI_DEV CycCompressed cyc_compressed_sqr(const CycCompressed& g) {
    CycCompressed r;
    const auto b = fp4_sqr(g.z2, g.z3);
    const auto c = fp4_sqr(g.z4, g.z5);
    r.z4 = fp2_store(fp2_add(fp2_dbl(fp2_sub(b.first, g.z4)), b.first));
    r.z5 = fp2_store(fp2_add(fp2_dbl(fp2_add(b.second, g.z5)), b.second));
    const auto t3n = fp2_mul_nr(c.second);
    r.z2 = fp2_store(fp2_add(fp2_dbl(fp2_add(t3n, g.z2)), t3n));
    r.z3 = fp2_store(fp2_add(fp2_dbl(fp2_sub(c.first, g.z3)), c.first));
    return r;
}
BLSMI_DEV void cyc_z1_fraction(const CycCompressed& g, Fp2S& num, Fp2S& den) {
    const i32 z2zero = fp2_is_zero(g.z2) ? -1 : 0;
    const Fp2S n_reg = fp2_store(fp2_sub(fp2_add(fp2_mul_nr(fp2_sqr(g.z5)), fp2_muls<3>(fp2_sqr(g.z4))), fp2_dbl(g.z3)));
    const Fp2S n_alt = fp2_store(fp2_dbl(fp2_mul(g.z4, g.z5)));
    const Fp2S d_reg = fp2_store(fp2_muls<4>(g.z2));
    num = fp2_select(z2zero, n_alt, n_reg);
    den = fp2_select(z2zero, g.z3, d_reg);
    den = fp2_select(fp2_is_zero(den) ? -1 : 0, fp2_one(), den);
}
BLSMI_DEV Fp12S cyc_decompress(const CycCompressed& g, const Fp2S& z1) {
    const Fp2S z0 = fp2_store(fp2_add(fp2_mul_nr(fp2_sub(fp2_add(fp2_dbl(fp2_sqr(z1)), fp2_mul(g.z2, g.z5)), fp2_muls<3>(fp2_mul(g.z3, g.z4)))), fp2_one()));
    Fp12S r;
    r.c0.c0 = z0; r.c0.c1 = g.z4; r.c0.c2 = g.z3; r.c1.c0 = g.z2; r.c1.c1 = z1; r.c1.c2 = g.z5;
    return r;
}
template <int La, int Va, int Lb, int Vb>
BLSMI_DEV bool fp12_eq(const Fp12<La, Va>& a, const Fp12<Lb, Vb>& b) {
    bool e = true;
    e &= fp2_eq(a.c0.c0, b.c0.c0); e &= fp2_eq(a.c0.c1, b.c0.c1); e &= fp2_eq(a.c0.c2, b.c0.c2);
    e &= fp2_eq(a.c1.c0, b.c1.c0); e &= fp2_eq(a.c1.c1, b.c1.c1); e &= fp2_eq(a.c1.c2, b.c1.c2);
    return e;
}
```

bls_amd/csrc/tower_fwd.cuh:

```cuda
#pragma once
namespace blsmi {
template <int L_, int V_> struct Fp2 { static constexpr int L = L_, V = V_; Fp<L_, V_> c0, c1; };
template <int L_, int V_> struct Fp6 { static constexpr int L = L_, V = V_; Fp2<L_, V_> c0, c1, c2; };
template <int L_, int V_> struct Fp12 { static constexpr int L = L_, V = V_; Fp6<L_, V_> c0, c1; };
using Fp2S = Fp2<FpS::L, FpS::V>;
using Fp6S = Fp6<FpS::L, FpS::V>;
using Fp12S = Fp12<FpS::L, FpS::V>;
}
```

bls_amd/engine.py:

```python
import ctypes as C

import numpy as np

from . import _native

_u8p = C.POINTER(C.c_uint8)
_u32p = C.POINTER(C.c_uint32)
_u64p = C.POINTER(C.c_uint64)


class BlsmiError(RuntimeError):
    pass


_ERR = {-1: "no usable HIP device", -2: "HIP runtime call failed", -3: "bad argument", -4: "out of memory", -5: "RCCL unavailable or collective failed", -6: "OS random source failed"}


def _check(rc, what):
    if rc != 0:
        raise BlsmiError("%s failed: %s (%d)" % (what, _ERR.get(rc, "unknown"), rc))


def _lib():
    return _native.load()
# ... 462 lines not shown
def _scalars(scalars, n):
    if scalars is None:
        return None
    r = np.ascontiguousarray(np.asarray([int(x) for x in scalars], dtype=np.uint64))
    if r.shape != (n,):
        raise ValueError("need one scalar per tuple")
    return _p64(r)


def _block(block):
    block = int(block)
    if block < 0:
        raise ValueError("block is 0 (automatic) or a number of items, got %d" % block)
    return block


def _msg_idx(msg_idx, n):
    ix = np.ascontiguousarray(np.asarray(msg_idx, dtype=np.uint32))
    if ix.shape != (n,):
        raise ValueError("need one message index per tuple")
    return _p32(ix) if n else None


def _grouped_head(msgs, msg_idx, n, domain8=None):
    pix = _msg_idx(msg_idx, n)
    return (_msg_head(msgs) if domain8 is None else _domain_head(msgs, domain8, 32)) + (len(msgs), pix)


def _verify(name, kind, jac, head, n, pks, sigs, inf_flags=None, rlc=False, scalars=None, block=None, bitmap=True):
    pkb, sgb = _sizes(kind, jac)
    args = head + (_recs(pks, pkb * n, jac), _recs(sigs, sgb * n, jac)) + (() if jac else (_flags(inf_flags, n),))
    ok = np.zeros(n, dtype=np.uint8)
    bm = np.zeros((n + 7) // 8, dtype=np.uint8)
    comb, nre = C.c_int(0), C.c_size_t(0)
    if rlc:
        args += (_scalars(scalars, n),)
    if block is not None:
        args += (_block(block),)
    args += (_p8(ok), _p8(bm) if bitmap else None, n) + ((C.byref(comb),) if rlc else ()) + ((C.byref(nre),) if block is not None else ())
    _call(name, *args)
    return (ok.astype(bool), bm) + ((comb.value,) if rlc else ()) + ((nre.value,) if block is not None else ())


def g2pubs_verify_batch(msgs, pks, sigs, inf_flags=None):
    return _verify("blsmi_g2pubs_verify_batch", 0, False, _msg_head(msgs), len(msgs), pks, sigs, inf_flags)


def g1pubs_verify_batch(msgs, pks, sigs, inf_flags=None):
    return _verify("blsmi_g1pubs_verify_batch", 1, False, _msg_head(msgs), len(msgs), pks, sigs, inf_flags)


def g2pubs_verify_batch_rlc(msgs, pks, sigs, inf_flags=None, scalars=None):
    return _verify("blsmi_g2pubs_verify_batch_rlc", 0, False, _msg_head(msgs), len(msgs), pks, sigs, inf_flags, True, scalars)


def g1pubs_verify_batch_rlc(msgs, pks, sigs, inf_flags=None, scalars=None):
    return _verify("blsmi_g1pubs_verify_batch_rlc", 1, False, _msg_head(msgs), len(msgs), pks, sigs, inf_flags, True, scalars)


def g1pubs_verify_with_domain_batch_rlc(msgs32, domain8, pks, sigs, inf_flags=None, scalars=None):
    ok, _, comb = _verify("blsmi_g1pubs_verify_with_domain_batch_rlc", 1, False, _domain_head(msgs32, domain8), len(msgs32), pks, sigs, inf_flags, True, scalars, bitmap=False)
    return ok, comb


def verify_serialized_batch(group, msgs, pks, sigs, check_subgroup=True):
    n = len(msgs)
    pkc, sgc = (96, 48) if group == "g2pubs" else (48, 96)
    ok = np.zeros(n, dtype=np.uint8); ep = np.zeros(n, dtype=np.uint8); es = np.zeros(n, dtype=np.uint8)
    _call("blsmi_%s_verify_serialized_batch" % _pubs(group), *_msg_head(msgs), _recs(pks, pkc * n, pad=True), _recs(sigs, sgc * n, pad=True), 1 if check_subgroup else 0,
          _p8(ok), _p8(ep), _p8(es), n)
    return ok.astype(bool), ep, es


def g1pubs_verify_with_domain_batch(msgs32, domain8, pks, sigs, inf_flags=None):
    return _verify("blsmi_g1pubs_verify_with_domain_batch", 1, False, _domain_head(msgs32, domain8), len(msgs32), pks, sigs, inf_flags, bitmap=False)[0]


def _verify_aggregate(name, kind, jac, head, n, pks, sig):
    pkb, sgb = _sizes(kind, jac)
    ok = C.c_int(0)
    _call(name, *head, _recs(pks, pkb * n, jac, pad=True), _recs(sig, sgb, jac), n, C.byref(ok))
    return bool(ok.value)


def g2pubs_verify_aggregate(msgs, pks, sig):
    return _verify_aggregate("blsmi_g2pubs_verify_aggregate", 0, False, _msg_head(msgs), len(msgs), pks, sig)


def g1pubs_verify_aggregate(msgs, pks, sig):
    return _verify_aggregate("blsmi_g1pubs_verify_aggregate", 1, False, _msg_head(msgs), len(msgs), pks, sig)


def g1pubs_verify_aggregate_with_domain(msgs32, domain8, pks, sig):
    return _verify_aggregate("blsmi_g1pubs_verify_aggregate_with_domain", 1, False, _domain_head(msgs32, domain8, 1), len(msgs32), pks, sig)


def g2pubs_verify_aggregate_common(msg, pks, sig, n):
    return _verify_aggregate("blsmi_g2pubs_verify_aggregate_common", 0, False, _one_msg(msg), n, pks, sig)


def g1pubs_verify_aggregate_common(msg, pks, sig, n):
    return _verify_aggregate("blsmi_g1pubs_verify_aggregate_common", 1, False, _one_msg(msg), n, pks, sig)


def g1pubs_verify_aggregate_common_with_domain(msg32, domain8, pks, sig, n):
    return _verify_aggregate("blsmi_g1pubs_verify_aggregate_common_with_domain", 1, False, (_p8(_u8(msg32, 32)), _p8(_u8(domain8, 8))), n, pks, sig)


def aggregate_partial(group, msgs, pks):
    n = len(msgs)
    out = np.zeros(72, dtype=np.uint64)
    bad = C.c_int(0)
    _call("blsmi_%s_aggregate_partial" % _pubs(group), *_msg_head(msgs), _recs(pks, (192 if group == "g2pubs" else 96) * n, pad=True), n, _p64(out), C.byref(bad))
    return out, bool(bad.value)


def fq12_product(vals):
    x = np.ascontiguousarray(vals, dtype=np.uint64).reshape(-1, 72)
    out = np.zeros(72, dtype=np.uint64)
    _call("blsmi_fq12_product", _p64(x), x.shape[0], _p64(out))
    return out


def _decompress(name, ib, ob, data, n, check):
    out = np.zeros((n, ob), dtype=np.uint8)
    inf = np.zeros(n, dtype=np.uint8)
    err = np.zeros(n, dtype=np.uint8)
    _call(name, _recs(data, ib * n), int(check), _p8(out.reshape(-1)), _p8(inf), _p8(err), n)
    return out, inf.astype(bool), err


def g1_decompress_batch(data, n, check_subgroup=True):
    return _decompress("blsmi_g1_decompress_batch", 48, 96, data, n, check_subgroup)


def g2_decompress_batch(data, n, check_subgroup=True):
    return _decompress("blsmi_g2_decompress_batch", 96, 192, data, n, check_subgroup)


def _compress(name, ib, ob, pts, n, in_inf):
    out = np.zeros((n, ob), dtype=np.uint8)
    _call(name, _recs(pts, ib * n), _flags(in_inf, n), _p8(out.reshape(-1)), n)
    return out


def g1_compress_batch(pts, n, in_inf=None):
    return _compress("blsmi_g1_compress_batch", 96, 48, pts, n, in_inf)


def g2_compress_batch(pts, n, in_inf=None):
    return _compress("blsmi_g2_compress_batch", 192, 96, pts, n, in_inf)


OPS = dict(FQ_MUL=1, FQ_SQR=2, FQ_ADD=3, FQ_SUB=4, FQ_NEG=5, FQ_INV=6, FQ_SQRT=7, FQ_DBL=8, FQ_CMP=9, FQ_PARITY=10,
           FQ2_MUL=16, FQ2_SQR=17, FQ2_INV=18, FQ2_MUL_NR=19, FQ2_SQRT=20, FQ2_SQRT_ANY=21, FQ2_PARITY=22,
           FQ6_MUL=32, FQ6_SQR=33, FQ6_INV=34, FQ6_FROB1=35, FQ6_MUL_BY_1=36, FQ6_MUL_BY_01=37,
           FQ12_MUL=48, FQ12_SQR=49, FQ12_INV=50, FQ12_FROB1=51, FQ12_FROB2=52, FQ12_FROB3=53, FQ12_CYCLO_SQR=54, FQ12_CYCLO_RUN16=55,
           FQ12_MUL_BY_014=56, FQ12_MUL_BY_LINE_PAIR=57, FQ12_FINAL_EXP=58,
           G1_DOUBLE=64, G1_ADD=65, G2_DOUBLE=66, G2_ADD=67, SWU_G1=68, SWU_G2=69, G1_MUL_U64=70,
           ROW_DBL_STEP=80, ROW_DBL_STEP_REF=81, ROW_ADD_STEP=82, ROW_ADD_STEP_REF=83, ROW_G2_DOUBLE=84, ROW_G2_ADD=85, ROW_CLEAR_H2=86)


LANE_PAIR = 0x100


def debug_g2_prepare(g2_aff=None, mode=0):
    out = np.zeros(68 * 3 * 12, dtype=np.uint64)
    _call("blsmi_debug_g2_prepare", _p8(_u8(g2_aff, 192)) if g2_aff is not None else None, mode, _p64(out))
    return out.reshape(68, 3, 12)


def debug_hash_tail(kind, pts, n):
    rec, hb = (384 if kind == 1 else 192), (96 if kind == 0 else 192)
    out = np.zeros((n, hb), dtype=np.uint8); good = np.zeros(n, dtype=np.uint8)
    _call("blsmi_debug_hash_tail", kind, _recs(pts, rec * n), _p8(out.reshape(-1)), _p8(good), n)
    return out, good


def debug_hash_redo(kind, msgs, good, out, domain8=None):
    n = len(msgs)
    hb = 96 if kind == 0 else 192
    o = np.ascontiguousarray(out, dtype=np.uint8).reshape(n, hb).copy()
    g = _u8(good, n)
    if kind == 2:
        head = _p8(_u8(b"".join(bytes(m) for m in msgs), 32 * n)), _p64(_u8(domain8, 8))
    else:
        head = _msg_head(msgs)
    _call("blsmi_debug_hash_redo", kind, *head, _p8(g), _p8(o.reshape(-1)), n)
    return o


def debug_lat_unit(which, in_raw, nout):
    a = np.ascontiguousarray(in_raw, dtype=np.int32)
    n, nin, nl = a.shape
    assert nl == 15
    out = np.zeros((nout, 15, n), dtype=np.int32)
    ok = np.zeros(n, dtype=np.uint8)
    i32p = C.POINTER(C.c_int32)
    _call("blsmi_debug_lat_unit", which, _ptr(a, i32p), nin, n, _ptr(out, i32p) if nout else None, _p8(ok))
    return np.ascontiguousarray(out.transpose(2, 0, 1)), ok


LANE_QUAD = 0x200
LANE_ROW = 0x400


def debug_op(name, a, b=None, lane_pair=False, raw_flag=False, lane_quad=False, lane_row=False):
    op = OPS[name]
    width = 1 if op < 16 else 2 if op < 32 else 6 if op < 48 else 12 if op < 64 or op >= 80 else (3 if op in (64, 65, 68, 70) else 6)
    a = np.ascontiguousarray(a, dtype=np.uint64).reshape(-1, 6 * width)
    n = a.shape[0]
    out = np.zeros_like(a)
    flag = np.zeros(n, dtype=np.uint8)
    bp = None
    if b is not None:
        b = np.ascontiguousarray(b, dtype=np.uint64).reshape(-1, 6 * width)
        assert b.shape == a.shape
        bp = _p64(b)
    _call("blsmi_debug_op", op | (LANE_PAIR if lane_pair else 0) | (LANE_QUAD if lane_quad else 0) | (LANE_ROW if lane_row else 0), _p64(a), bp, _p64(out), _p8(flag), n)
    return out, (flag.copy() if raw_flag else flag.astype(bool))


G1_JAC_BYTES, G2_JAC_BYTES = 144, 288


def _jac_to_affine(name, jb, wb, jac, n):
    out = np.zeros(max(1, wb * n), dtype=np.uint8)
    inf = np.zeros(max(1, n), dtype=np.uint8)
    _call(name, _recs(jac, jb * n, True), _p8(out), _p8(inf), n)
    return out[:wb * n].tobytes(), inf[:n].astype(bool)


def g1_jac_to_affine_batch(jac, n):
    return _jac_to_affine("blsmi_g1_jac_to_affine_batch", 144, 96, jac, n)


def g2_jac_to_affine_batch(jac, n):
    return _jac_to_affine("blsmi_g2_jac_to_affine_batch", 288, 192, jac, n)


def pairing_batch_jac(g1_jac, g2_jac, n):
    out = np.zeros((n, 72), dtype=np.uint64)
    _call("blsmi_pairing_batch_jac", _recs(g1_jac, 144 * n, True), _recs(g2_jac, 288 * n, True), _p64(out), n)
    return out


def _sum_jac(name, jb, pts, n):
    out = np.zeros(jb // 8, dtype=np.uint64)
    oinf = C.c_int(0)
    _call(name, _recs(pts, jb * n, True), n, _p64(out), C.byref(oinf))
    return out.tobytes(), bool(oinf.value)


def g1_sum_jac(pts, n):
    return _sum_jac("blsmi_g1_sum_jac", 144, pts, n)


def g2_sum_jac(pts, n):
    return _sum_jac("blsmi_g2_sum_jac", 288, pts, n)


def g2pubs_verify_batch_jac(msgs, pks, sigs):
    return _verify("blsmi_g2pubs_verify_batch_jac", 0, True, _msg_head(msgs), len(msgs), pks, sigs)


def g1pubs_verify_batch_jac(msgs, pks, sigs):
    return _verify("blsmi_g1pubs_verify_batch_jac", 1, True, _msg_head(msgs), len(msgs), pks, sigs)


def g1pubs_verify_with_domain_batch_jac(msgs32, domain8, pks, sigs):
    return _verify("blsmi_g1pubs_verify_with_domain_batch_jac", 1, True, _domain_head(msgs32, domain8), len(msgs32), pks, sigs, bitmap=False)[0]


def g2pubs_verify_batch_rlc_jac(msgs, pks, sigs, scalars=None):
    return _verify("blsmi_g2pubs_verify_batch_rlc_jac", 0, True, _msg_head(msgs), len(msgs), pks, sigs, None, True, scalars)


def g1pubs_verify_batch_rlc_jac(msgs, pks, sigs, scalars=None):
    return _verify("blsmi_g1pubs_verify_batch_rlc_jac", 1, True, _msg_head(msgs), len(msgs), pks, sigs, None, True, scalars)


def g1pubs_verify_with_domain_batch_rlc_jac(msgs32, domain8, pks, sigs, scalars=None):
    ok, _, comb = _verify("blsmi_g1pubs_verify_with_domain_batch_rlc_jac", 1, True, _domain_head(msgs32, domain8), len(msgs32), pks, sigs, None, True, scalars, bitmap=False)
    return ok, comb


def g2pubs_verify_aggregate_jac(msgs, pks, sig):
    return _verify_aggregate("blsmi_g2pubs_verify_aggregate_jac", 0, True, _msg_head(msgs), len(msgs), pks, sig)


def g1pubs_verify_aggregate_jac(msgs, pks, sig):
    return _verify_aggregate("blsmi_g1pubs_verify_aggregate_jac", 1, True, _msg_head(msgs), len(msgs), pks, sig)


def g1pubs_verify_aggregate_with_domain_jac(msgs32, domain8, pks, sig):
    return _verify_aggregate("blsmi_g1pubs_verify_aggregate_with_domain_jac", 1, True, _domain_head(msgs32, domain8, 1), len(msgs32), pks, sig)


def g2pubs_verify_aggregate_common_jac(msg, pks, sig, n):
    return _verify_aggregate("blsmi_g2pubs_verify_aggregate_common_jac", 0, True, _one_msg(msg), n, pks, sig)


def g1pubs_verify_aggregate_common_jac(msg, pks, sig, n):
    return _verify_aggregate("blsmi_g1pubs_verify_aggregate_common_jac", 1, True, _one_msg(msg), n, pks, sig)


def g1pubs_verify_aggregate_common_with_domain_jac(msg32, domain8, pks, sig, n):
# ... 513 lines not shown
```

include/blsmi.h:

```cpp
#ifndef BLSMI_H
#define BLSMI_H
#include <stddef.h>
#include <stdint.h>

#ifdef __cplusplus
extern "C" {
#endif

#define BLSMI_OK 0
#define BLSMI_E_NODEVICE (-1)
#define BLSMI_E_HIP (-2)
#define BLSMI_E_ARG (-3)
#define BLSMI_E_NOMEM (-4)
#define BLSMI_E_RCCL (-5)
#define BLSMI_E_RNG (-6)

int blsmi_init(int device);
int blsmi_init_devices(int ndev);
int blsmi_debug_alias_own(const void *d_ptr, size_t bytes, int device_index);
int blsmi_device_count(void);
long long blsmi_debug_device_leases(int device_index);
int blsmi_shard_count(void);
void blsmi_shutdown(void);
const char *blsmi_version(void);
// ... 54 lines not shown

int blsmi_g2pubs_verify_batch(const uint8_t *msgs, const uint64_t *off, const uint8_t *pks , const uint8_t *sigs ,
                              const uint8_t *inf_flags, uint8_t *ok , uint8_t *ok_bitmap , size_t n);
int blsmi_g2pubs_verify_aggregate(const uint8_t *msgs, const uint64_t *off, const uint8_t *pks, const uint8_t sig[96], size_t n, int *ok);
int blsmi_g2pubs_verify_aggregate_common(const uint8_t *msg, size_t msg_len, const uint8_t *pks, const uint8_t sig[96], size_t n, int *ok);

int blsmi_g1pubs_verify_batch(const uint8_t *msgs, const uint64_t *off, const uint8_t *pks , const uint8_t *sigs ,
                              const uint8_t *inf_flags, uint8_t *ok, uint8_t *ok_bitmap, size_t n);
int blsmi_g1pubs_verify_aggregate(const uint8_t *msgs, const uint64_t *off, const uint8_t *pks, const uint8_t sig[192], size_t n, int *ok);
int blsmi_g1pubs_verify_aggregate_common(const uint8_t *msg, size_t msg_len, const uint8_t *pks, const uint8_t sig[192], size_t n, int *ok);
int blsmi_g1pubs_verify_with_domain_batch(const uint8_t *msgs32, const uint8_t domain[8], const uint8_t *pks, const uint8_t *sigs,
                                          const uint8_t *inf_flags, uint8_t *ok, uint8_t *ok_bitmap, size_t n);
int blsmi_g1pubs_verify_aggregate_with_domain(const uint8_t *msgs32, const uint8_t domain[8], const uint8_t *pks, const uint8_t sig[192], size_t n, int *ok);
int blsmi_g1pubs_verify_aggregate_common_with_domain(const uint8_t msg32[32], const uint8_t domain[8], const uint8_t *pks, const uint8_t sig[192], size_t n, int *ok);

#define BLSMI_G2_PREPARED_BYTES 24704
int blsmi_g2_prepare_batch_dev(const void *d_g2_aff , size_t n, void *d_prepared , void *stream);
int blsmi_g2_prepared_export_dev(const void *d_prepared, size_t n, void *d_out , void *stream);
int blsmi_g2_prepare_batch(const uint8_t *g2_aff , size_t n, uint64_t *out_coeffs );
int blsmi_g2_prepared_create(const uint8_t *g2_aff , size_t n, void **handle);
int blsmi_g2_prepared_destroy(void *handle);
int blsmi_g2pubs_verify_batch_prepared(const uint8_t *msgs, const uint64_t *msg_off, const void *d_prepared, const uint32_t *key_idx ,
                                       const uint8_t *sigs, const uint8_t *inf_flags, uint8_t *ok, uint8_t *ok_bitmap, size_t n);
int blsmi_pairing_batch_prepared_dev(const void *d_g1_aff, const void *d_prepared, const void *d_key_idx, void *d_out_fq12, size_t n, void *stream);
int blsmi_g2pubs_verify_batch_prepared_dev(const void *d_msgs, const void *d_off, const void *d_prepared, const void *d_key_idx,
                                           const void *d_sigs, const void *d_inf_flags, void *d_ok, size_t n, void *stream);
int blsmi_g2pubs_verify_aggregate_prepared(const uint8_t *msgs, const uint64_t *msg_off, const void *d_prepared, const uint32_t *key_idx ,
                                           const uint8_t sig[96], size_t n, int *ok);
int blsmi_g2pubs_verify_aggregate_prepared_dev(const void *d_msgs, const void *d_off, const void *d_prepared, const void *d_key_idx,
                                               const uint8_t sig[96], size_t n, int *ok, void *stream);

#define BLSMI_G1_JAC_BYTES 144
#define BLSMI_G2_JAC_BYTES 288
int blsmi_g1_jac_to_affine_batch(const uint64_t *g1_jac , uint8_t *out , uint8_t *out_inf , size_t n);
int blsmi_g2_jac_to_affine_batch(const uint64_t *g2_jac , uint8_t *out , uint8_t *out_inf , size_t n);
int blsmi_pairing_batch_jac(const uint64_t *g1_jac , const uint64_t *g2_jac , uint64_t *out_fq12 , size_t n);
int blsmi_g1_sum_jac(const uint64_t *g1_jac , size_t n, uint64_t out_jac[18], int *out_inf);
int blsmi_g2_sum_jac(const uint64_t *g2_jac , size_t n, uint64_t out_jac[36], int *out_inf);
int blsmi_g1_mul_generator_batch_jac(const uint8_t *scalars , uint64_t *out_jac , size_t n);
int blsmi_g2_mul_generator_batch_jac(const uint8_t *scalars , uint64_t *out_jac , size_t n);
int blsmi_g2pubs_sign_batch_jac(const uint8_t *msgs, const uint64_t *off , const uint8_t *sks , uint64_t *out_sigs_jac , size_t n);
int blsmi_g1pubs_sign_batch_jac(const uint8_t *msgs, const uint64_t *off , const uint8_t *sks , uint64_t *out_sigs_jac , size_t n);
int blsmi_g1pubs_sign_with_domain_batch_jac(const uint8_t *msgs32 , const uint8_t domain[8], const uint8_t *sks , uint64_t *out_sigs_jac , size_t n);
int blsmi_g2pubs_verify_batch_jac(const uint8_t *msgs, const uint64_t *off, const uint64_t *pks , const uint64_t *sigs ,
                                  uint8_t *ok , uint8_t *ok_bitmap , size_t n);
int blsmi_g2pubs_verify_aggregate_jac(const uint8_t *msgs, const uint64_t *off, const uint64_t *pks , const uint64_t sig[18], size_t n, int *ok);
int blsmi_g2pubs_verify_aggregate_common_jac(const uint8_t *msg, size_t msg_len, const uint64_t *pks , const uint64_t sig[18], size_t n, int *ok);
int blsmi_g1pubs_verify_batch_jac(const uint8_t *msgs, const uint64_t *off, const uint64_t *pks , const uint64_t *sigs ,
                                  uint8_t *ok, uint8_t *ok_bitmap, size_t n);
int blsmi_g1pubs_verify_with_domain_batch_jac(const uint8_t *msgs32, const uint8_t domain[8], const uint64_t *pks , const uint64_t *sigs ,
                                              uint8_t *ok, uint8_t *ok_bitmap, size_t n);
int blsmi_g1pubs_verify_aggregate_jac(const uint8_t *msgs, const uint64_t *off, const uint64_t *pks , const uint64_t sig[36], size_t n, int *ok);
int blsmi_g1pubs_verify_aggregate_with_domain_jac(const uint8_t *msgs32, const uint8_t domain[8], const uint64_t *pks , const uint64_t sig[36], size_t n, int *ok);
int blsmi_g1pubs_verify_aggregate_common_jac(const uint8_t *msg, size_t msg_len, const uint64_t *pks , const uint64_t sig[36], size_t n, int *ok);
int blsmi_g1pubs_verify_aggregate_common_with_domain_jac(const uint8_t msg32[32], const uint8_t domain[8], const uint64_t *pks , const uint64_t sig[36], size_t n, int *ok);
int blsmi_g2pubs_verify_batch_rlc(const uint8_t *msgs, const uint64_t *off, const uint8_t *pks , const uint8_t *sigs , const uint8_t *inf_flags,
                                  const uint64_t *scalars , uint8_t *ok , uint8_t *ok_bitmap , size_t n, int *combined);
int blsmi_g1pubs_verify_batch_rlc(const uint8_t *msgs, const uint64_t *off, const uint8_t *pks , const uint8_t *sigs , const uint8_t *inf_flags,
                                  const uint64_t *scalars, uint8_t *ok, uint8_t *ok_bitmap, size_t n, int *combined);
int blsmi_g1pubs_verify_with_domain_batch_rlc(const uint8_t *msgs32, const uint8_t domain[8], const uint8_t *pks, const uint8_t *sigs, const uint8_t *inf_flags,
                                              const uint64_t *scalars, uint8_t *ok, uint8_t *ok_bitmap, size_t n, int *combined);
int blsmi_g2pubs_verify_batch_rlc_jac(const uint8_t *msgs, const uint64_t *off, const uint64_t *pks , const uint64_t *sigs ,
                                      const uint64_t *scalars, uint8_t *ok, uint8_t *ok_bitmap, size_t n, int *combined);
int blsmi_g1pubs_verify_batch_rlc_jac(const uint8_t *msgs, const uint64_t *off, const uint64_t *pks , const uint64_t *sigs ,
                                      const uint64_t *scalars, uint8_t *ok, uint8_t *ok_bitmap, size_t n, int *combined);
int blsmi_g1pubs_verify_with_domain_batch_rlc_jac(const uint8_t *msgs32, const uint8_t domain[8], const uint64_t *pks , const uint64_t *sigs ,
                                                  const uint64_t *scalars, uint8_t *ok, uint8_t *ok_bitmap, size_t n, int *combined);
int blsmi_g2pubs_verify_batch_rlc_grouped(const uint8_t *msgs, const uint64_t *msg_off , size_t d, const uint32_t *msg_idx ,
                                          const uint8_t *pks , const uint8_t *sigs , const uint8_t *inf_flags,
                                          const uint64_t *scalars , uint8_t *ok , uint8_t *ok_bitmap , size_t n, int *combined);
int blsmi_g1pubs_verify_batch_rlc_grouped(const uint8_t *msgs, const uint64_t *msg_off , size_t d, const uint32_t *msg_idx ,
                                          const uint8_t *pks , const uint8_t *sigs , const uint8_t *inf_flags,
                                          const uint64_t *scalars, uint8_t *ok, uint8_t *ok_bitmap, size_t n, int *combined);
int blsmi_g1pubs_verify_with_domain_batch_rlc_grouped(const uint8_t *msgs32 , const uint8_t domain[8], size_t d, const uint32_t *msg_idx ,
                                                      const uint8_t *pks, const uint8_t *sigs, const uint8_t *inf_flags,
                                                      const uint64_t *scalars, uint8_t *ok, uint8_t *ok_bitmap, size_t n, int *combined);
int blsmi_g2pubs_verify_batch_rlc_grouped_jac(const uint8_t *msgs, const uint64_t *msg_off, size_t d, const uint32_t *msg_idx, const uint64_t *pks , const uint64_t *sigs ,
                                              const uint64_t *scalars, uint8_t *ok, uint8_t *ok_bitmap, size_t n, int *combined);
int blsmi_g1pubs_verify_batch_rlc_grouped_jac(const uint8_t *msgs, const uint64_t *msg_off, size_t d, const uint32_t *msg_idx, const uint64_t *pks , const uint64_t *sigs ,
                                              const uint64_t *scalars, uint8_t *ok, uint8_t *ok_bitmap, size_t n, int *combined);
int blsmi_g1pubs_verify_with_domain_batch_rlc_grouped_jac(const uint8_t *msgs32, const uint8_t domain[8], size_t d, const uint32_t *msg_idx, const uint64_t *pks ,
                                                          const uint64_t *sigs , const uint64_t *scalars, uint8_t *ok, uint8_t *ok_bitmap, size_t n, int *combined);
int blsmi_g2pubs_verify_batch_rlc_locate(const uint8_t *msgs, const uint64_t *off, const uint8_t *pks , const uint8_t *sigs , const uint8_t *inf_flags,
                                         const uint64_t *scalars , size_t block, uint8_t *ok , uint8_t *ok_bitmap , size_t n,
                                         int *combined, size_t *rechecked);
int blsmi_g1pubs_verify_batch_rlc_locate(const uint8_t *msgs, const uint64_t *off, const uint8_t *pks , const uint8_t *sigs , const uint8_t *inf_flags,
                                         const uint64_t *scalars, size_t block, uint8_t *ok, uint8_t *ok_bitmap, size_t n, int *combined, size_t *rechecked);
int blsmi_g1pubs_verify_with_domain_batch_rlc_locate(const uint8_t *msgs32, const uint8_t domain[8], const uint8_t *pks, const uint8_t *sigs, const uint8_t *inf_flags,
                                                     const uint64_t *scalars, size_t block, uint8_t *ok, uint8_t *ok_bitmap, size_t n, int *combined, size_t *rechecked);
int blsmi_g2pubs_verify_batch_rlc_locate_jac(const uint8_t *msgs, const uint64_t *off, const uint64_t *pks , const uint64_t *sigs ,
                                             const uint64_t *scalars, size_t block, uint8_t *ok, uint8_t *ok_bitmap, size_t n, int *combined, size_t *rechecked);
int blsmi_g1pubs_verify_batch_rlc_locate_jac(const uint8_t *msgs, const uint64_t *off, const uint64_t *pks , const uint64_t *sigs ,
                                             const uint64_t *scalars, size_t block, uint8_t *ok, uint8_t *ok_bitmap, size_t n, int *combined, size_t *rechecked);
int blsmi_g1pubs_verify_with_domain_batch_rlc_locate_jac(const uint8_t *msgs32, const uint8_t domain[8], const uint64_t *pks , const uint64_t *sigs ,
                                                         const uint64_t *scalars, size_t block, uint8_t *ok, uint8_t *ok_bitmap, size_t n, int *combined, size_t *rechecked);
int blsmi_g2pubs_verify_batch_rlc_grouped_locate(const uint8_t *msgs, const uint64_t *msg_off , size_t d, const uint32_t *msg_idx ,
                                                 const uint8_t *pks , const uint8_t *sigs , const uint8_t *inf_flags,
                                                 const uint64_t *scalars , size_t block, uint8_t *ok , uint8_t *ok_bitmap ,
                                                 size_t n, int *combined, size_t *rechecked);
int blsmi_g1pubs_verify_batch_rlc_grouped_locate(const uint8_t *msgs, const uint64_t *msg_off , size_t d, const uint32_t *msg_idx ,
                                                 const uint8_t *pks , const uint8_t *sigs , const uint8_t *inf_flags,
                                                 const uint64_t *scalars, size_t block, uint8_t *ok, uint8_t *ok_bitmap, size_t n, int *combined, size_t *rechecked);
int blsmi_g1pubs_verify_with_domain_batch_rlc_grouped_locate(const uint8_t *msgs32 , const uint8_t domain[8], size_t d, const uint32_t *msg_idx ,
                                                             const uint8_t *pks, const uint8_t *sigs, const uint8_t *inf_flags,
                                                             const uint64_t *scalars, size_t block, uint8_t *ok, uint8_t *ok_bitmap, size_t n, int *combined, size_t *rechecked);
int blsmi_g2pubs_verify_batch_rlc_grouped_locate_jac(const uint8_t *msgs, const uint64_t *msg_off, size_t d, const uint32_t *msg_idx, const uint64_t *pks ,
                                                     const uint64_t *sigs , const uint64_t *scalars, size_t block, uint8_t *ok, uint8_t *ok_bitmap, size_t n,
                                                     int *combined, size_t *rechecked);
int blsmi_g1pubs_verify_batch_rlc_grouped_locate_jac(const uint8_t *msgs, const uint64_t *msg_off, size_t d, const uint32_t *msg_idx, const uint64_t *pks ,
                                                     const uint64_t *sigs , const uint64_t *scalars, size_t block, uint8_t *ok, uint8_t *ok_bitmap, size_t n,
                                                     int *combined, size_t *rechecked);
int blsmi_g1pubs_verify_with_domain_batch_rlc_grouped_locate_jac(const uint8_t *msgs32, const uint8_t domain[8], size_t d, const uint32_t *msg_idx, const uint64_t *pks ,
                                                                 const uint64_t *sigs , const uint64_t *scalars, size_t block, uint8_t *ok, uint8_t *ok_bitmap, size_t n,
                                                                 int *combined, size_t *rechecked);
int blsmi_pairing_batch_jac_dev(const void *d_g1_jac, const void *d_g2_jac, void *d_out_fq12, size_t n, void *stream);
int blsmi_g2pubs_verify_batch_jac_dev(const void *d_msgs, const void *d_off, const void *d_pks_jac, const void *d_sigs_jac, void *d_ok, size_t n, void *stream);
int blsmi_g1pubs_verify_batch_jac_dev(const void *d_msgs, const void *d_off, const void *d_pks_jac, const void *d_sigs_jac, void *d_ok, size_t n, void *stream);
int blsmi_g1pubs_verify_with_domain_batch_jac_dev(const void *d_msgs32, const void *d_domain8, const void *d_pks_jac, const void *d_sigs_jac, void *d_ok, size_t n, void *stream);
int blsmi_g2_prepared_create_jac(const uint64_t *g2_jac , size_t n, void **handle);
int blsmi_g2pubs_verify_batch_prepared_jac(const uint8_t *msgs, const uint64_t *msg_off, const void *d_prepared, const uint32_t *key_idx ,
                                           const uint64_t *sigs , uint8_t *ok, uint8_t *ok_bitmap, size_t n);
int blsmi_g2pubs_verify_aggregate_prepared_jac(const uint8_t *msgs, const uint64_t *msg_off, const void *d_prepared, const uint32_t *key_idx ,
                                               const uint64_t sig[18], size_t n, int *ok);

int blsmi_g2pubs_aggregate_partial(const uint8_t *msgs, const uint64_t *off, const uint8_t *pks, size_t n, uint64_t *out_fq12 , int *bad );
int blsmi_g1pubs_aggregate_partial(const uint8_t *msgs, const uint64_t *off, const uint8_t *pks, size_t n, uint64_t *out_fq12 , int *bad);
int blsmi_fq12_product(const uint64_t *in_fq12 , size_t n, uint64_t *out_fq12 );

int blsmi_g2pubs_verify_batch_dev(const void *d_msgs, const void *d_off, const void *d_pks, const void *d_sigs, const void *d_inf_flags, void *d_ok, size_t n, void *stream);
int blsmi_g1pubs_verify_batch_dev(const void *d_msgs, const void *d_off, const void *d_pks, const void *d_sigs, const void *d_inf_flags, void *d_ok, size_t n, void *stream);
int blsmi_g1pubs_verify_with_domain_batch_dev(const void *d_msgs32, const void *d_domain8, const void *d_pks, const void *d_sigs, const void *d_inf_flags, void *d_ok, size_t n, void *stream);

int blsmi_g2pubs_verify_aggregate_dev(const void *d_msgs, const void *d_off, const void *d_pks, const uint8_t sig[96], size_t n, int *ok, void *stream);
int blsmi_g1pubs_verify_aggregate_dev(const void *d_msgs, const void *d_off, const void *d_pks, const uint8_t sig[192], size_t n, int *ok, void *stream);
int blsmi_g1pubs_verify_aggregate_with_domain_dev(const void *d_msgs32, const void *d_domain, const void *d_pks, const uint8_t sig[192], size_t n, int *ok, void *stream);

int blsmi_g2pubs_verify_aggregate_common_dev(const void *d_pks , size_t n, const uint8_t *msg, size_t msg_len, const uint8_t sig[96], int *ok, void *stream);
int blsmi_g1pubs_verify_aggregate_common_dev(const void *d_pks , size_t n, const uint8_t *msg, size_t msg_len, const uint8_t sig[192], int *ok, void *stream);
int blsmi_g1pubs_verify_aggregate_common_with_domain_dev(const void *d_pks , size_t n, const uint8_t msg32[32], const uint8_t domain[8], const uint8_t sig[192], int *ok, void *stream);

int blsmi_g2pubs_verify_serialized_batch(const uint8_t *msgs, const uint64_t *off , const uint8_t *pks , const uint8_t *sigs ,
                                         int check_subgroup, uint8_t *ok , uint8_t *err_pk, uint8_t *err_sig, size_t n);
int blsmi_g1pubs_verify_serialized_batch(const uint8_t *msgs, const uint64_t *off , const uint8_t *pks , const uint8_t *sigs ,
                                         int check_subgroup, uint8_t *ok , uint8_t *err_pk, uint8_t *err_sig, size_t n);

int blsmi_g1_decompress_batch(const uint8_t *in , int check_subgroup, uint8_t *out , uint8_t *out_inf, uint8_t *err, size_t n);
int blsmi_g2_decompress_batch(const uint8_t *in , int check_subgroup, uint8_t *out , uint8_t *out_inf, uint8_t *err, size_t n);
int blsmi_g1_compress_batch(const uint8_t *pts, const uint8_t *in_inf, uint8_t *out , size_t n);
int blsmi_g2_compress_batch(const uint8_t *pts, const uint8_t *in_inf, uint8_t *out , size_t n);

enum blsmi_debug_op {
    BLSMI_OP_FQ_MUL = 1, BLSMI_OP_FQ_SQR, BLSMI_OP_FQ_ADD, BLSMI_OP_FQ_SUB, BLSMI_OP_FQ_NEG, BLSMI_OP_FQ_INV, BLSMI_OP_FQ_SQRT,
    BLSMI_OP_FQ_DBL , BLSMI_OP_FQ_CMP , BLSMI_OP_FQ_PARITY ,
    BLSMI_OP_FQ2_MUL = 16, BLSMI_OP_FQ2_SQR, BLSMI_OP_FQ2_INV, BLSMI_OP_FQ2_MUL_NR, BLSMI_OP_FQ2_SQRT, BLSMI_OP_FQ2_SQRT_ANY , BLSMI_OP_FQ2_PARITY ,
    BLSMI_OP_FQ6_MUL = 32, BLSMI_OP_FQ6_SQR, BLSMI_OP_FQ6_INV, BLSMI_OP_FQ6_FROB1,
    BLSMI_OP_FQ6_MUL_BY_1 , BLSMI_OP_FQ6_MUL_BY_01 ,
    BLSMI_OP_FQ12_MUL = 48, BLSMI_OP_FQ12_SQR, BLSMI_OP_FQ12_INV, BLSMI_OP_FQ12_FROB1, BLSMI_OP_FQ12_FROB2, BLSMI_OP_FQ12_FROB3, BLSMI_OP_FQ12_CYCLO_SQR, BLSMI_OP_FQ12_CYCLO_RUN16 ,
    BLSMI_OP_FQ12_MUL_BY_014 , BLSMI_OP_FQ12_MUL_BY_LINE_PAIR ,
    BLSMI_OP_FQ12_FINAL_EXP = 58 ,
    BLSMI_OP_G1_DOUBLE = 64, BLSMI_OP_G1_ADD, BLSMI_OP_G2_DOUBLE, BLSMI_OP_G2_ADD,
    BLSMI_OP_SWU_G1 = 68 , BLSMI_OP_SWU_G2 ,
    BLSMI_OP_G1_MUL_U64 = 70 ,
    BLSMI_OP_ROW_DBL_STEP = 80, BLSMI_OP_ROW_DBL_STEP_REF, BLSMI_OP_ROW_ADD_STEP, BLSMI_OP_ROW_ADD_STEP_REF,
    BLSMI_OP_ROW_G2_DOUBLE = 84, BLSMI_OP_ROW_G2_ADD, BLSMI_OP_ROW_CLEAR_H2
};
#define BLSMI_OP_LANE_PAIR 0x100
#define BLSMI_OP_LANE_QUAD 0x200
#define BLSMI_OP_LANE_ROW 0x400
int blsmi_debug_op(int op, const uint64_t *a, const uint64_t *b, uint64_t *out, uint8_t *flag , size_t n);
int blsmi_debug_g2_prepare(const uint8_t *g2_aff , int mode, uint64_t *out );

int blsmi_debug_hash_tail(int kind, const uint8_t *pts, uint8_t *out, uint8_t *good, size_t n);
int blsmi_debug_hash_g1_finish(const uint8_t *pts , int clear , uint8_t *out , int *special, size_t n);
int blsmi_debug_hash_redo(int kind, const uint8_t *msgs, const uint64_t *off_or_domain, const uint8_t *good, uint8_t *out , size_t n);
int blsmi_debug_lat_unit(int which, const int32_t *in_raw , size_t nin, size_t n, int32_t *out_raw , uint8_t *ok );

int blsmi_g1_sum_segmented(const uint8_t *pts , const uint8_t *in_inf , size_t npk,
                           const uint32_t *idx , const uint64_t *seg_off , size_t m,
                           uint8_t *out , uint8_t *out_inf );
int blsmi_g2_sum_segmented(const uint8_t *pts , const uint8_t *in_inf , size_t npk,
                           const uint32_t *idx , const uint64_t *seg_off , size_t m,
                           uint8_t *out , uint8_t *out_inf );
int blsmi_g1_sum_segmented_jac(const uint64_t *pts_jac , size_t npk, const uint32_t *idx, const uint64_t *seg_off, size_t m,
                               uint8_t *out , uint8_t *out_inf );
int blsmi_g2_sum_segmented_jac(const uint64_t *pts_jac , size_t npk, const uint32_t *idx, const uint64_t *seg_off, size_t m,
                               uint8_t *out , uint8_t *out_inf );
int blsmi_g1_sum_segmented_dev(const void *d_pts, const void *d_in_inf, size_t npk, const void *d_idx, const void *d_seg_off, size_t m,
                               void *d_out, void *d_out_inf, void *stream);
int blsmi_g2_sum_segmented_dev(const void *d_pts, const void *d_in_inf, size_t npk, const void *d_idx, const void *d_seg_off, size_t m,
                               void *d_out, void *d_out_inf, void *stream);
int blsmi_g1_sum_segmented_u64(const uint8_t *pts , const uint8_t *in_inf , size_t npk, const uint64_t *scalars ,
                               const uint32_t *idx , const uint64_t *seg_off , size_t m,
                               uint8_t *out , uint8_t *out_inf );
int blsmi_g2_sum_segmented_u64(const uint8_t *pts , const uint8_t *in_inf , size_t npk, const uint64_t *scalars ,
                               const uint32_t *idx , const uint64_t *seg_off , size_t m,
                               uint8_t *out , uint8_t *out_inf );
int blsmi_g2pubs_verify_aggregate_common_batch(const uint8_t *msgs, const uint64_t *msg_off , const uint8_t *pks , size_t npk,
                                               const uint32_t *idx, const uint64_t *seg_off , const uint8_t *sigs ,
                                               uint8_t *ok , uint8_t *ok_bitmap , size_t m);
int blsmi_g1pubs_verify_aggregate_common_batch(const uint8_t *msgs, const uint64_t *msg_off , const uint8_t *pks , size_t npk,
                                               const uint32_t *idx, const uint64_t *seg_off , const uint8_t *sigs ,
                                               uint8_t *ok, uint8_t *ok_bitmap, size_t m);
int blsmi_g1pubs_verify_aggregate_common_with_domain_batch(const uint8_t *msgs32 , const uint8_t domain[8], const uint8_t *pks , size_t npk,
                                                           const uint32_t *idx, const uint64_t *seg_off , const uint8_t *sigs ,
                                                           uint8_t *ok, uint8_t *ok_bitmap, size_t m);
int blsmi_g2pubs_verify_aggregate_common_batch_jac(const uint8_t *msgs, const uint64_t *msg_off, const uint64_t *pks , size_t npk,
                                                   const uint32_t *idx, const uint64_t *seg_off, const uint64_t *sigs ,
                                                   uint8_t *ok, uint8_t *ok_bitmap, size_t m);
int blsmi_g1pubs_verify_aggregate_common_batch_jac(const uint8_t *msgs, const uint64_t *msg_off, const uint64_t *pks , size_t npk,
                                                   const uint32_t *idx, const uint64_t *seg_off, const uint64_t *sigs ,
                                                   uint8_t *ok, uint8_t *ok_bitmap, size_t m);
int blsmi_g1pubs_verify_aggregate_common_with_domain_batch_jac(const uint8_t *msgs32, const uint8_t domain[8], const uint64_t *pks , size_t npk,
                                                               const uint32_t *idx, const uint64_t *seg_off, const uint64_t *sigs ,
                                                               uint8_t *ok, uint8_t *ok_bitmap, size_t m);
int blsmi_g2pubs_verify_aggregate_common_batch_dev(const void *d_msgs, const void *d_msg_off, const void *d_pks, size_t npk, const void *d_idx,
                                                   const void *d_seg_off, const void *d_sigs, void *d_ok, size_t m, void *stream);
int blsmi_g1pubs_verify_aggregate_common_batch_dev(const void *d_msgs, const void *d_msg_off, const void *d_pks, size_t npk, const void *d_idx,
                                                   const void *d_seg_off, const void *d_sigs, void *d_ok, size_t m, void *stream);
int blsmi_g1pubs_verify_aggregate_common_with_domain_batch_dev(const void *d_msgs32, const void *d_domain, const void *d_pks, size_t npk, const void *d_idx,
                                                               const void *d_seg_off, const void *d_sigs, void *d_ok, size_t m, void *stream);

int blsmi_pairing_product_batch(const uint8_t *g1_aff , const uint8_t *g2_aff ,
                                const uint8_t *inf_flags , size_t np,
                                const uint64_t *seg_off , size_t m,
                                uint64_t *out_fq12 , uint8_t *is_one );
int blsmi_pairing_product_batch_jac(const uint64_t *g1_jac , const uint64_t *g2_jac , size_t np,
                                    const uint64_t *seg_off, size_t m, uint64_t *out_fq12, uint8_t *is_one);
int blsmi_pairing_product_batch_dev(const void *d_g1_aff, const void *d_g2_aff, const void *d_inf_flags, size_t np,
                                    const void *d_seg_off, size_t m, void *d_out_fq12, void *d_is_one, void *stream);
int blsmi_pairing_product_batch_jac_dev(const void *d_g1_jac, const void *d_g2_jac, size_t np,
                                        const void *d_seg_off, size_t m, void *d_out_fq12, void *d_is_one, void *stream);

#define BLSMI_POINT_OK 0
#define BLSMI_POINT_INFINITY 1
#define BLSMI_POINT_NOT_ON_CURVE 3
#define BLSMI_POINT_NOT_IN_SUBGROUP 4
int blsmi_g1_check_batch(const uint8_t *pts , const uint8_t *in_inf , int check, uint8_t *status , size_t n);
int blsmi_g2_check_batch(const uint8_t *pts , const uint8_t *in_inf , int check, uint8_t *status , size_t n);
int blsmi_g1_check_batch_jac(const uint64_t *pts_jac , int check, uint8_t *status , size_t n);
int blsmi_g2_check_batch_jac(const uint64_t *pts_jac , int check, uint8_t *status , size_t n);
int blsmi_g1_check_batch_dev(const void *d_pts, const void *d_in_inf, int jac, int check, void *d_status, size_t n, void *stream);
int blsmi_g2_check_batch_dev(const void *d_pts, const void *d_in_inf, int jac, int check, void *d_status, size_t n, void *stream);

int blsmi_g1_decompress_batch_jac(const uint8_t *in , int check_subgroup, uint64_t *out_jac , uint8_t *out_inf ,
                                  uint8_t *err , size_t n);
int blsmi_g2_decompress_batch_jac(const uint8_t *in , int check_subgroup, uint64_t *out_jac , uint8_t *out_inf ,
                                  uint8_t *err , size_t n);
int blsmi_g1_compress_batch_jac(const uint64_t *pts_jac , uint8_t *out , size_t n);
int blsmi_g2_compress_batch_jac(const uint64_t *pts_jac , uint8_t *out , size_t n);
int blsmi_g1_decompress_batch_jac_dev(const void *d_in, int check_subgroup, void *d_out_jac, void *d_out_inf , void *d_err, size_t n, void *stream);
int blsmi_g2_decompress_batch_jac_dev(const void *d_in, int check_subgroup, void *d_out_jac, void *d_out_inf , void *d_err, size_t n, void *stream);
int blsmi_g1_compress_batch_jac_dev(const void *d_pts_jac, void *d_out, size_t n, void *stream);
int blsmi_g2_compress_batch_jac_dev(const void *d_pts_jac, void *d_out, size_t n, void *stream);

int blsmi_g2pubs_verify_aggregate_common_batch_rlc(const uint8_t *msgs, const uint64_t *msg_off , size_t d, const uint32_t *msg_idx ,
                                                   const uint8_t *pks , size_t npk, const uint32_t *idx, const uint64_t *seg_off ,
                                                   const uint8_t *sigs , const uint64_t *scalars ,
                                                   uint8_t *ok , uint8_t *ok_bitmap , size_t m, int *combined);
int blsmi_g1pubs_verify_aggregate_common_batch_rlc(const uint8_t *msgs, const uint64_t *msg_off , size_t d, const uint32_t *msg_idx ,
                                                   const uint8_t *pks , size_t npk, const uint32_t *idx, const uint64_t *seg_off ,
                                                   const uint8_t *sigs , const uint64_t *scalars, uint8_t *ok, uint8_t *ok_bitmap, size_t m, int *combined);
int blsmi_g1pubs_verify_aggregate_common_with_domain_batch_rlc(const uint8_t *msgs32 , const uint8_t domain[8], size_t d, const uint32_t *msg_idx ,
                                                               const uint8_t *pks , size_t npk, const uint32_t *idx, const uint64_t *seg_off ,
                                                               const uint8_t *sigs , const uint64_t *scalars, uint8_t *ok, uint8_t *ok_bitmap, size_t m, int *combined);
int blsmi_g2pubs_verify_aggregate_common_batch_rlc_jac(const uint8_t *msgs, const uint64_t *msg_off, size_t d, const uint32_t *msg_idx,
                                                       const uint64_t *pks , size_t npk, const uint32_t *idx, const uint64_t *seg_off,
                                                       const uint64_t *sigs , const uint64_t *scalars, uint8_t *ok, uint8_t *ok_bitmap, size_t m, int *combined);
int blsmi_g1pubs_verify_aggregate_common_batch_rlc_jac(const uint8_t *msgs, const uint64_t *msg_off, size_t d, const uint32_t *msg_idx,
                                                       const uint64_t *pks , size_t npk, const uint32_t *idx, const uint64_t *seg_off,
                                                       const uint64_t *sigs , const uint64_t *scalars, uint8_t *ok, uint8_t *ok_bitmap, size_t m, int *combined);
int blsmi_g1pubs_verify_aggregate_common_with_domain_batch_rlc_jac(const uint8_t *msgs32, const uint8_t domain[8], size_t d, const uint32_t *msg_idx,
                                                                   const uint64_t *pks , size_t npk, const uint32_t *idx, const uint64_t *seg_off,
                                                                   const uint64_t *sigs , const uint64_t *scalars, uint8_t *ok, uint8_t *ok_bitmap, size_t m, int *combined);
int blsmi_g2pubs_verify_aggregate_common_batch_rlc_dev(const void *d_msgs, const void *d_msg_off, size_t d, const void *d_msg_idx, const void *d_pks, size_t npk,
                                                       const void *d_idx, const void *d_seg_off, const void *d_sigs, const uint64_t *scalars ,
                                                       void *d_ok, size_t m, int *combined , void *stream);
int blsmi_g1pubs_verify_aggregate_common_batch_rlc_dev(const void *d_msgs, const void *d_msg_off, size_t d, const void *d_msg_idx, const void *d_pks, size_t npk,
                                                       const void *d_idx, const void *d_seg_off, const void *d_sigs, const uint64_t *scalars, void *d_ok, size_t m,
                                                       int *combined, void *stream);
int blsmi_g1pubs_verify_aggregate_common_with_domain_batch_rlc_dev(const void *d_msgs32, const void *d_domain, size_t d, const void *d_msg_idx, const void *d_pks, size_t npk,
                                                                   const void *d_idx, const void *d_seg_off, const void *d_sigs, const uint64_t *scalars, void *d_ok, size_t m,
                                                                   int *combined, void *stream);
int blsmi_debug_g2_sum_segmented_u64_pair(const uint8_t *pts , const uint8_t *in_inf , size_t npk, const uint64_t *scalars ,
                                          const uint32_t *idx , const uint64_t *seg_off , size_t m,
                                          uint8_t *out , uint8_t *out_inf );

int blsmi_pairing_product_batch_rlc(const uint8_t *g1_aff , const uint8_t *inf_flags ,
                                    const uint8_t *g2_tab , size_t nq, const uint32_t *q_idx ,
                                    size_t np, const uint64_t *seg_off , size_t m,
                                    const uint64_t *scalars , uint8_t *is_one , int *combined );
int blsmi_pairing_product_batch_rlc_jac(const uint64_t *g1_jac , const uint64_t *g2_tab_jac , size_t nq, const uint32_t *q_idx,
                                        size_t np, const uint64_t *seg_off, size_t m, const uint64_t *scalars, uint8_t *is_one, int *combined);
int blsmi_pairing_product_batch_rlc_dev(const void *d_g1_aff, const void *d_inf_flags, const void *d_g2_tab, size_t nq, const void *d_q_idx,
                                        size_t np, const void *d_seg_off, size_t m, const uint64_t *scalars ,
                                        void *d_is_one, int *combined , void *stream);
int blsmi_pairing_product_batch_rlc_jac_dev(const void *d_g1_jac, const void *d_g2_tab_jac, size_t nq, const void *d_q_idx,
                                            size_t np, const void *d_seg_off, size_t m, const uint64_t *scalars, void *d_is_one, int *combined, void *stream);
int blsmi_debug_pairing_product_batch_rlc_dev_nosplit(const void *d_g1_aff, const void *d_inf_flags, const void *d_g2_tab, size_t nq, const void *d_q_idx,
                                                      size_t np, const void *d_seg_off, size_t m, const uint64_t *scalars, void *d_is_one, int *combined,
                                                      void *stream);

int blsmi_pairing_product_batch_rlc_locate(const uint8_t *g1_aff , const uint8_t *inf_flags ,
                                           const uint8_t *g2_tab , size_t nq, const uint32_t *q_idx ,
                                           size_t np, const uint64_t *seg_off , size_t m,
                                           const uint64_t *scalars , size_t block ,
                                           uint8_t *is_one , int *combined , size_t *rechecked );
// ... 50 lines not shown
```

Baseline: 3.909 million.

## Keep Fp12 accumulators in reduced work form and use int32 carries in reduce

Introduces a work representation (FpW) for Fp12 values in the Miller loop and final exponentiation. In the 28-bit limb build it keeps results only partially reduced (VRED bound) instead of converting to the storage form after every tower operation, which removes the full store normalisation from the hot path. It also narrows the carry in fp_reduce from int64 to int32, with static asserts on the bounds, so the carry chain uses cheaper arithmetic. A debug op is added to exercise the lazy bound chain. The risk is that the tighter bounds flow into the multiply routines differently, which may change register pressure or force extra reductions elsewhere.

```diff
diff --git a/bls_amd/csrc/fp.cuh b/bls_amd/csrc/fp.cuh
--- a/bls_amd/csrc/fp.cuh
+++ b/bls_amd/csrc/fp.cuh
@@ -1,6 +1,7 @@
 #pragma once
 #include <hip/hip_runtime.h>
 #include <stdint.h>
+#include <type_traits>
 
 namespace blsmi {
 
@@ -58,6 +59,12 @@
 };
 using FpS = Fp<1, VSTORE>;
 using FpC = Fp<1, VU>;
+using FpR = Fp<1, VRED>;
+#ifdef BLSMI_LIMBS28
+using FpW = FpR;
+#else
+using FpW = FpS;
+#endif
 
 }
 #include "tower_fwd.cuh"
@@ -153,17 +160,22 @@
     const Fp<L, V>& y = x;
     const float top = (float)y.v[NL - 1] * (float)(1 << LB) + (float)y.v[NL - 2];
     const i32 k = (i32)floorf(top * BLSMI_Q_TOP2_INV);
+    static_assert((i64)LMAX * ((1ll << LB) + 64) + (1ll << 13) < (1ll << 31), "limb plus carry must fit int32");
+    static_assert((1 << (31 - LB)) + VMAX / VU + 2 < (1 << 13), "carry bound");
     Fp<1, VRED> r;
-    i64 c = 0;
+    i32 c = 0;
 #pragma unroll
     for (int i = 0; i < NL - 1; i++) {
-        c += (i64)y.v[i] - (i64)k * C_Q[i];
-        r.v[i] = (i32)c & MASK;
-        c >>= LB;
-    }
-    c += (i64)y.v[NL - 1] - (i64)k * C_Q[NL - 1];
-    r.v[NL - 1] = (i32)c;
-    return r;
+        const i64 s = (i64)(y.v[i] + c) - (i64)k * C_Q[i];
+        r.v[i] = (i32)s & MASK;
+        c = (i32)(s >> LB);
+    }
+    r.v[NL - 1] = (i32)((i64)(y.v[NL - 1] + c) - (i64)k * C_Q[NL - 1]);
+    return r;
+}
+template <int L, int V>
+BLSMI_DEV Fp<1, VRED> fp_reduced(const Fp<L, V>& x) {
+    if constexpr (V <= VRED) return fp_relabel<1, VRED>(fp_norm(x)); else return fp_reduce(x);
 }
 template <int VT, int L, int V>
 BLSMI_DEV auto fp_fit(const Fp<L, V>& x) {
diff --git a/bls_amd/csrc/fp2_pair.inc b/bls_amd/csrc/fp2_pair.inc
--- a/bls_amd/csrc/fp2_pair.inc
+++ b/bls_amd/csrc/fp2_pair.inc
@@ -5,6 +5,12 @@
 using Fp2S = Fp2<FpS::L, FpS::V>;
 using Fp6S = Fp6<FpS::L, FpS::V>;
 using Fp12S = Fp12<FpS::L, FpS::V>;
+using Fp2R = Fp2<FpR::L, FpR::V>;
+using Fp6R = Fp6<FpR::L, FpR::V>;
+using Fp12R = Fp12<FpR::L, FpR::V>;
+using Fp2W = Fp2<FpW::L, FpW::V>;
+using Fp6W = Fp6<FpW::L, FpW::V>;
+using Fp12W = Fp12<FpW::L, FpW::V>;
 
 BLSMI_DEV i32 lane_odd() { return -(i32)(threadIdx.x & 1); }
 BLSMI_DEV i32 bfi(i32 mask, i32 a, i32 b) {
@@ -39,6 +45,7 @@
 template <int L, int V> BLSMI_DEV auto fp2_conj(const Fp2<L, V>& a) { return wrap(fp_cneg(lane_odd(), a.c)); }
 template <int L, int V> BLSMI_DEV auto fp2_norm(const Fp2<L, V>& a) { return wrap(fp_norm(a.c)); }
 template <int L, int V> BLSMI_DEV Fp2S fp2_store(const Fp2<L, V>& a) { return wrap(fp_store(a.c)); }
+template <int L, int V> BLSMI_DEV Fp2R fp2_reduced(const Fp2<L, V>& a) { return wrap(fp_reduced(a.c)); }
 template <int L, int V> BLSMI_DEV bool fp2_is_zero(const Fp2<L, V>& a) {
     const int z = fp_is_zero(a.c) ? 1 : 0;
     return (z & __shfl_xor(z, 1)) != 0;
diff --git a/bls_amd/csrc/fp2_single.inc b/bls_amd/csrc/fp2_single.inc
--- a/bls_amd/csrc/fp2_single.inc
+++ b/bls_amd/csrc/fp2_single.inc
@@ -21,6 +21,7 @@
 template <int L, int V> BLSMI_DEV auto fp2_conj(const Fp2<L, V>& a) { return make_fp2(a.c0, fp_neg(a.c1)); }
 template <int L, int V> BLSMI_DEV auto fp2_norm(const Fp2<L, V>& a) { return make_fp2(fp_norm(a.c0), fp_norm(a.c1)); }
 template <int L, int V> BLSMI_DEV Fp2S fp2_store(const Fp2<L, V>& a) { Fp2S r; r.c0 = fp_store(a.c0); r.c1 = fp_store(a.c1); return r; }
+template <int L, int V> BLSMI_DEV Fp2R fp2_reduced(const Fp2<L, V>& a) { Fp2R r; r.c0 = fp_reduced(a.c0); r.c1 = fp_reduced(a.c1); return r; }
 template <int L, int V> BLSMI_DEV bool fp2_is_zero(const Fp2<L, V>& a) { return fp_is_zero(a.c0) & fp_is_zero(a.c1); }
 template <int La, int Va, int Lb, int Vb> BLSMI_DEV bool fp2_eq(const Fp2<La, Va>& a, const Fp2<Lb, Vb>& b) { return fp2_is_zero(fp2_sub(a, b)); }
 template <int L, int V> BLSMI_DEV Fp2<L, V> fp2_select(i32 m, const Fp2<L, V>& a, const Fp2<L, V>& b) { Fp2<L, V> r; r.c0 = fp_select(m, a.c0, b.c0); r.c1 = fp_select(m, a.c1, b.c1); return r; }
diff --git a/bls_amd/csrc/k_pairing_pair.hip b/bls_amd/csrc/k_pairing_pair.hip
--- a/bls_amd/csrc/k_pairing_pair.hip
+++ b/bls_amd/csrc/k_pairing_pair.hip
@@ -45,15 +45,17 @@
         if (t0 < n) pair_rec_store<3>(out, t, par, reinterpret_cast<const FpS*>(&r));
     } else {
         P2::Fp12S x, y, r; pair_rec_load<6>(reinterpret_cast<FpS*>(&x), a, t, par); y = x; if (b) pair_rec_load<6>(reinterpret_cast<FpS*>(&y), b, t, par);
+        const P2::Fp12W xw = P2::fp12_work(x), yw = P2::fp12_work(y);
+        P2::Fp12W rw = xw;
         switch (op) {
-            case BLSMI_OP_FQ12_MUL: P2::nf_fp12_mul(r, x, y); break;
-            case BLSMI_OP_FQ12_SQR: P2::nf_fp12_sqr(r, x); break;
-            case BLSMI_OP_FQ12_INV: P2::nf_fp12_inv(r, x); break;
-            case BLSMI_OP_FQ12_FROB1: P2::nf_fp12_frob1(r, x); break;
-            case BLSMI_OP_FQ12_FROB2: P2::nf_fp12_frob2(r, x); break;
-            case BLSMI_OP_FQ12_FROB3: P2::nf_fp12_frob3(r, x); break;
-            case BLSMI_OP_FQ12_CYCLO_SQR: P2::nf_fp12_cyc_sqr(r, x); break;
-            case BLSMI_OP_FQ12_CYCLO_RUN16: r = P2::cyc_sqr_run(x, 16); break;
+            case BLSMI_OP_FQ12_MUL: P2::nf_fp12_mul(rw, xw, yw); r = P2::fp12_widen(rw); break;
+            case BLSMI_OP_FQ12_SQR: P2::nf_fp12_sqr(rw, xw); r = P2::fp12_widen(rw); break;
+            case BLSMI_OP_FQ12_INV: P2::nf_fp12_inv(rw, xw); r = P2::fp12_widen(rw); break;
+            case BLSMI_OP_FQ12_FROB1: P2::nf_fp12_frob1(rw, xw); r = P2::fp12_widen(rw); break;
+            case BLSMI_OP_FQ12_FROB2: P2::nf_fp12_frob2(rw, xw); r = P2::fp12_widen(rw); break;
+            case BLSMI_OP_FQ12_FROB3: P2::nf_fp12_frob3(rw, xw); r = P2::fp12_widen(rw); break;
+            case BLSMI_OP_FQ12_CYCLO_SQR: P2::nf_fp12_cyc_sqr(rw, xw); r = P2::fp12_widen(rw); break;
+            case BLSMI_OP_FQ12_CYCLO_RUN16: r = P2::fp12_widen(P2::cyc_sqr_run(xw, 16)); break;
             case BLSMI_OP_FQ12_MUL_BY_014: r = P2::fp12_store(P2::fp12_mul_by_014(x, y.c0.c0, y.c0.c1, y.c0.c2)); break;
             default: {
                 const P2::LinePair m = P2::line_pair_product(y.c0.c0, y.c0.c1, y.c0.c2, y.c1.c0, y.c1.c1, y.c1.c2);
diff --git a/bls_amd/csrc/k_wire.hip b/bls_amd/csrc/k_wire.hip
--- a/bls_amd/csrc/k_wire.hip
+++ b/bls_amd/csrc/k_wire.hip
@@ -185,7 +185,7 @@
     if (t >= n) return;
     const FpS x = load_m384(a + 6 * t);
     FpS y = fp_zero();
-    if (op == BLSMI_OP_FQ_MUL || op == BLSMI_OP_FQ_ADD || op == BLSMI_OP_FQ_SUB || op == BLSMI_OP_FQ_CMP) y = load_m384(b + 6 * t);
+    if (op == BLSMI_OP_FQ_MUL || op == BLSMI_OP_FQ_ADD || op == BLSMI_OP_FQ_SUB || op == BLSMI_OP_FQ_CMP || op == BLSMI_OP_FQ_LAZY) y = load_m384(b + 6 * t);
     FpS r = fp_zero();
     bool ok = true;
     int code = -1;
@@ -206,6 +206,13 @@
         case BLSMI_OP_FQ_NEG: r = fp_store(fp_neg(x)); break;
         case BLSMI_OP_FQ_INV: r = fp_inv(x); ok = !fp_is_zero(x); break;
         case BLSMI_OP_FQ_SQRT: r = fp_sqrt(x, ok); break;
+        case BLSMI_OP_FQ_LAZY: {
+            const auto p = fp_mul(x, y);
+            const auto big = fp_muls<3>(fp_norm(fp_muls<7>(fp_norm(fp_muls<7>(fp_norm(fp_muls<7>(p)))))));
+            const auto hi = fp_add(big, fp_muls<4>(x)), lo = fp_sub(fp_muls<4>(y), big);
+            static_assert(decltype(hi)::L == 7 && decltype(lo)::L == 7 && 4 * decltype(hi)::V > 3 * VMAX, "the chain reaches the bounds it is here for");
+            r = fp_store(fp_mul(fp_reduce(hi), fp_reduce(lo))); break;
+        }
     }
     store_m384(out + 6 * t, r);
     if (flag) flag[t] = code >= 0 ? (u8)code : (ok ? 1 : 0);
diff --git a/bls_amd/csrc/pair_kernels.inc b/bls_amd/csrc/pair_kernels.inc
--- a/bls_amd/csrc/pair_kernels.inc
+++ b/bls_amd/csrc/pair_kernels.inc
@@ -26,11 +26,11 @@
 struct PairYieldOps : P2::Fp12Ops {
     static BLSMI_DEV void before_exp_x(int k) { if (k == PAIR_YIELD_FE_EXP_X) pair_yield_drop(); }
 };
-BLSMI_DEV void final_exponentiation_yield(P2::Fp12S& f) {
+BLSMI_DEV void final_exponentiation_yield(P2::Fp12W& f) {
 #if BLSMI_PAIR_YIELD
     P2::final_exp_chain<PairYieldOps>(f);
 #else
-    P2::final_exponentiation(f);
+    P2::final_exp_chain<P2::Fp12Ops>(f);
 #endif
 }
 
@@ -129,9 +129,9 @@
     const size_t tt = t < n ? t : n - 1;
     const WaveCensus census;
     pair_yield_enter();
-    P2::Fp12S f = pair_load12(fbuf, n, tt, par);
+    P2::Fp12W f = P2::fp12_work(pair_load12(fbuf, n, tt, par));
     if (mode == 0) final_exponentiation_yield(f);
-    const FpS* c = reinterpret_cast<const FpS*>(&f);
+    const FpW* c = reinterpret_cast<const FpW*>(&f);
     for (int j = 0; j < 6; j++) {
         u32 w[12];
         fp_to_mont384_words(c[j], w);
@@ -205,7 +205,7 @@
     const size_t tt = t < n ? t : n - 1;
     const WaveCensus census;
     pair_yield_enter();
-    P2::Fp12S f = pair_load12(fbuf, n, tt, par);
+    P2::Fp12W f = P2::fp12_work(pair_load12(fbuf, n, tt, par));
     final_exponentiation_yield(f);
     const bool one = P2::fp12_eq(f, P2::fp12_one());
     if (t < n && par == 0) ok[t] = (one && !(inf_flags && inf_flags[t])) ? 1 : 0;
diff --git a/bls_amd/csrc/pairing_body.inc b/bls_amd/csrc/pairing_body.inc
--- a/bls_amd/csrc/pairing_body.inc
+++ b/bls_amd/csrc/pairing_body.inc
@@ -1,14 +1,14 @@
 
 struct G2Proj { Fp2S x, y, z; };
 
-BLSMI_NOINLINE void nf_fp12_mul(Fp12S& r, const Fp12S& a, const Fp12S& b) { r = fp12_store(fp12_mul(a, b)); }
-BLSMI_NOINLINE void nf_fp12_sqr(Fp12S& r, const Fp12S& a) { r = fp12_store(fp12_sqr(a)); }
-BLSMI_NOINLINE void nf_fp12_cyc_sqr(Fp12S& r, const Fp12S& a) { r = fp12_cyclotomic_sqr(a); }
-BLSMI_NOINLINE void nf_fp12_inv(Fp12S& r, const Fp12S& a) { r = fp12_store(fp12_inv(a)); }
-BLSMI_NOINLINE void nf_fp12_frob1(Fp12S& r, const Fp12S& a) { r = fp12_store(fp12_frob<1>(a)); }
-BLSMI_NOINLINE void nf_fp12_frob2(Fp12S& r, const Fp12S& a) { r = fp12_store(fp12_frob<2>(a)); }
-BLSMI_NOINLINE void nf_fp12_frob3(Fp12S& r, const Fp12S& a) { r = fp12_store(fp12_frob<3>(a)); }
-BLSMI_DEV void fp12_conj_inplace(Fp12S& a) { a.c1 = fp6_store(fp6_neg(a.c1)); }
+BLSMI_NOINLINE void nf_fp12_mul(Fp12W& r, const Fp12W& a, const Fp12W& b) { r = fp12_work(fp12_mul(a, b)); }
+BLSMI_NOINLINE void nf_fp12_sqr(Fp12W& r, const Fp12W& a) { r = fp12_work(fp12_sqr(a)); }
+BLSMI_NOINLINE void nf_fp12_cyc_sqr(Fp12W& r, const Fp12W& a) { r = fp12_cyclotomic_sqr(a); }
+BLSMI_NOINLINE void nf_fp12_inv(Fp12W& r, const Fp12W& a) { r = fp12_work(fp12_inv(a)); }
+BLSMI_NOINLINE void nf_fp12_frob1(Fp12W& r, const Fp12W& a) { r = fp12_work(fp12_frob<1>(a)); }
+BLSMI_NOINLINE void nf_fp12_frob2(Fp12W& r, const Fp12W& a) { r = fp12_work(fp12_frob<2>(a)); }
+BLSMI_NOINLINE void nf_fp12_frob3(Fp12W& r, const Fp12W& a) { r = fp12_work(fp12_frob<3>(a)); }
+BLSMI_DEV void fp12_conj_inplace(Fp12W& a) { a.c1 = fp6_work(fp6_neg(a.c1)); }
 
 BLSMI_NOINLINE void doubling_step(G2Proj& r, Fp2S& o0, Fp2S& o1, Fp2S& o2) {
     const auto tmp0 = fp2_norm(fp2_sqr(r.x));
@@ -54,7 +54,7 @@
     const auto B = fp2_norm(fp2_sqr(r.y));
     const auto X2 = fp2_norm(fp2_sqr(r.x));
     const auto H = fp2_norm(fp2_dbl(fp2_mul(r.y, r.z)));
-    const auto E = fp2_norm(fp2_muls<12>(fp2_norm(fp2_mul_nr(fp2_norm(fp2_sqr(r.z))))));
+    const auto E = fp2_trim(fp2_muls<12>(fp2_norm(fp2_mul_nr(fp2_norm(fp2_sqr(r.z))))));
     const auto F = fp2_norm(fp2_muls<3>(E));
     const auto G = fp2_norm(fp2_add(B, F));
     const auto nx = fp2_norm(fp2_dbl(fp2_mul(A, fp2_norm(fp2_sub(B, F)))));
@@ -89,25 +89,25 @@
 template <bool EXACT> BLSMI_DEV void add_step(G2Proj& r, const Fp2S& qx, const Fp2S& qy, Fp2S& o0, Fp2S& o1, Fp2S& o2) {
     if constexpr (EXACT) addition_step(r, qx, qy, o0, o1, o2); else addition_step_h(r, qx, qy, o0, o1, o2);
 }
-BLSMI_NOINLINE void ell(Fp12S& f, const Fp2S& o0, const Fp2S& o1, const Fp2S& o2, const FpS& px, const FpS& py) {
+BLSMI_NOINLINE void ell(Fp12W& f, const Fp2S& o0, const Fp2S& o1, const Fp2S& o2, const FpS& px, const FpS& py) {
     const auto c0 = fp2_mul_fp(o0, py);
     const auto c1 = fp2_mul_fp(o1, px);
-    f = fp12_store(fp12_mul_by_014(f, o2, c1, c0));
-}
-
-BLSMI_NOINLINE void ell_sqr(Fp12S& f, const Fp2S& o0, const Fp2S& o1, const Fp2S& o2, const FpS& px, const FpS& py) {
+    f = fp12_work(fp12_mul_by_014(fp12_widen(f), o2, c1, c0));
+}
+
+BLSMI_NOINLINE void ell_sqr(Fp12W& f, const Fp2S& o0, const Fp2S& o1, const Fp2S& o2, const FpS& px, const FpS& py) {
     const auto c0 = fp2_mul_fp(o0, py);
     const auto c1 = fp2_mul_fp(o1, px);
-    const Fp12S g = fp12_store(fp12_mul_by_014(f, o2, c1, c0));
-    f = fp12_store(fp12_sqr(g));
+    const Fp12W g = fp12_work(fp12_mul_by_014(f, o2, c1, c0));
+    f = fp12_work(fp12_sqr(g));
 }
 
 template <bool SQR>
-BLSMI_NOINLINE void ell2(Fp12S& f, const Fp2S& a0, const Fp2S& a1, const Fp2S& a2, const FpS& ax, const FpS& ay,
+BLSMI_NOINLINE void ell2(Fp12W& f, const Fp2S& a0, const Fp2S& a1, const Fp2S& a2, const FpS& ax, const FpS& ay,
                          const Fp2S& b0, const Fp2S& b1, const Fp2S& b2, const FpS& bx, const FpS& by) {
     const LinePair m = line_pair_product(a2, fp2_mul_fp(a1, ax), fp2_mul_fp(a0, ay), b2, fp2_mul_fp(b1, bx), fp2_mul_fp(b0, by));
-    const Fp12S g = fp12_store(fp12_mul_by_line_pair(f, m));
-    if (SQR) f = fp12_store(fp12_sqr(g)); else f = g;
+    const Fp12W g = fp12_work(fp12_mul_by_line_pair(f, m));
+    if (SQR) f = fp12_work(fp12_sqr(g)); else f = g;
 }
 
 struct NoTick { BLSMI_DEV void operator()(int) const {} };
@@ -147,14 +147,14 @@
     return r;
 }
 template <int NP, bool PRE0 = false, bool EXACT = true, bool PRE1 = false, int YIELD = 0, class G1P, class G2P>
-BLSMI_DEV void miller_loop(Fp12S& f, const G1P (&p)[NP], const G2P (&q)[NP], const i32* pre = nullptr, const i32* pre1 = nullptr, i32* lds_r = nullptr) {
+BLSMI_DEV void miller_loop(Fp12S& out, const G1P (&p)[NP], const G2P (&q)[NP], const i32* pre = nullptr, const i32* pre1 = nullptr, i32* lds_r = nullptr) {
     static_assert(NP == 1 || NP == 2, "one pair, or two pairs sharing the squarings");
     constexpr int LAST = NP - 1;
     constexpr bool PRE_LAST = NP == 1 ? PRE0 : PRE1;
     G2Proj r[NP];
 #pragma unroll
     for (int k = 0; k < NP; k++) { r[k].x = q[k].x; r[k].y = q[k].y; r[k].z = fp2_one(); }
-    f = fp12_one();
+    Fp12W f = fp12_work(fp12_one());
     const bool in_lds = !EXACT && !PRE_LAST && lds_r != nullptr;
     if (in_lds) lds_put_proj(lds_r, r[LAST]);
     auto dbl_last = [&](Fp2S& a0, Fp2S& a1, Fp2S& a2) {
@@ -187,6 +187,7 @@
                    [&] { ell2<true>(f, o0, o1, o2, p[0].x, p[0].y, n0, n1, n2, p[1].x, p[1].y); }, tick);
     }
     fp12_conj_inplace(f);
+    out = fp12_widen(f);
 }
 BLSMI_DEV void prepare_lines(const Fp2S& qx, const Fp2S& qy, i32* table) {
     G2Proj r; r.x = qx; r.y = qy; r.z = fp2_one();
@@ -250,16 +251,16 @@
     O::mul(r, y1, y3);
 }
 
-BLSMI_DEV Fp12S cyc_sqr_run(const Fp12S& g, int m) {
-    CycCompressed c = cyc_compress(g);
+BLSMI_DEV Fp12W cyc_sqr_run(const Fp12W& g, int m) {
+    CycCompressedW c = cyc_compress(g);
     for (int j = 0; j < m; j++) c = cyc_compressed_sqr(c);
     Fp2S num, den;
     cyc_z1_fraction(c, num, den);
-    return cyc_decompress(c, fp2_store(fp2_mul(num, fp2_store(fp2_inv(den)))));
-}
-BLSMI_NOINLINE void exp_by_x(Fp12S& out, const Fp12S& f, u64 e);
+    return cyc_decompress(c, fp2_mul(num, fp2_store(fp2_inv(den))));
+}
+BLSMI_NOINLINE void exp_by_x(Fp12W& out, const Fp12W& f, u64 e);
 struct Fp12Ops {
-    using T = Fp12S;
+    using T = Fp12W;
     static constexpr int MIN_RUN = 12;
     static BLSMI_DEV void inv(T& r, const T& a) { nf_fp12_inv(r, a); }
     static BLSMI_DEV void mul(T& r, const T& a, const T& b) { nf_fp12_mul(r, a, b); }
@@ -272,5 +273,9 @@
     static BLSMI_DEV void conj(T& a) { fp12_conj_inplace(a); }
     static BLSMI_DEV void exp_x(T& r, const T& a, u64 e) { exp_by_x(r, a, e); }
 };
-BLSMI_NOINLINE void exp_by_x(Fp12S& out, const Fp12S& f, u64 e) { exp_by_x_loop<Fp12Ops>(out, f, e); }
-BLSMI_DEV void final_exponentiation(Fp12S& r) { final_exp_chain<Fp12Ops>(r); }
+BLSMI_NOINLINE void exp_by_x(Fp12W& out, const Fp12W& f, u64 e) { exp_by_x_loop<Fp12Ops>(out, f, e); }
+BLSMI_DEV void final_exponentiation(Fp12S& r) {
+    Fp12W w = fp12_work(r);
+    final_exp_chain<Fp12Ops>(w);
+    r = fp12_widen(w);
+}
diff --git a/bls_amd/csrc/tower_body.inc b/bls_amd/csrc/tower_body.inc
--- a/bls_amd/csrc/tower_body.inc
+++ b/bls_amd/csrc/tower_body.inc
@@ -29,6 +29,20 @@
 template <int L, int V> BLSMI_DEV auto fp6_neg(const Fp6<L, V>& a) { return make_fp6(fp2_neg(a.c0), fp2_neg(a.c1), fp2_neg(a.c2)); }
 template <int L, int V> BLSMI_DEV auto fp6_norm(const Fp6<L, V>& a) { return make_fp6(fp2_norm(a.c0), fp2_norm(a.c1), fp2_norm(a.c2)); }
 template <int L, int V> BLSMI_DEV Fp6S fp6_store(const Fp6<L, V>& a) { Fp6S r; r.c0 = fp2_store(a.c0); r.c1 = fp2_store(a.c1); r.c2 = fp2_store(a.c2); return r; }
+template <int L, int V> BLSMI_DEV Fp6R fp6_reduced(const Fp6<L, V>& a) { Fp6R r; r.c0 = fp2_reduced(a.c0); r.c1 = fp2_reduced(a.c1); r.c2 = fp2_reduced(a.c2); return r; }
+template <class F2, int L, int V> BLSMI_DEV F2 fp2_as(const Fp2<L, V>& a) {
+    static_assert(std::is_same<F2, Fp2R>::value || std::is_same<F2, Fp2S>::value, "the reduced or the storage type");
+    if constexpr (std::is_same<F2, Fp2R>::value) return fp2_reduced(a); else return fp2_store(a);
+}
+template <int L, int V> BLSMI_DEV Fp2W fp2_work(const Fp2<L, V>& a) { return fp2_as<Fp2W>(a); }
+template <int L, int V> BLSMI_DEV auto fp2_trim(const Fp2<L, V>& a) {
+#ifdef BLSMI_LIMBS28
+    return fp2_reduced(a);
+#else
+    return fp2_norm(a);
+#endif
+}
+template <int L, int V> BLSMI_DEV Fp6W fp6_work(const Fp6<L, V>& a) { Fp6W r; r.c0 = fp2_work(a.c0); r.c1 = fp2_work(a.c1); r.c2 = fp2_work(a.c2); return r; }
 BLSMI_DEV Fp6S fp6_zero() { Fp6S r; r.c0 = fp2_zero(); r.c1 = fp2_zero(); r.c2 = fp2_zero(); return r; }
 BLSMI_DEV Fp6S fp6_one() { Fp6S r; r.c0 = fp2_one(); r.c1 = fp2_zero(); r.c2 = fp2_zero(); return r; }
 template <int L, int V> BLSMI_DEV auto fp6_mul_nr(const Fp6<L, V>& a) { return make_fp6(fp2_mul_nr(a.c2), a.c0, a.c1); }
@@ -85,6 +99,11 @@
 }
 
 template <int L, int V> BLSMI_DEV Fp12S fp12_store(const Fp12<L, V>& a) { Fp12S r; r.c0 = fp6_store(a.c0); r.c1 = fp6_store(a.c1); return r; }
+template <int L, int V> BLSMI_DEV Fp12R fp12_reduced(const Fp12<L, V>& a) { Fp12R r; r.c0 = fp6_reduced(a.c0); r.c1 = fp6_reduced(a.c1); return r; }
+template <int L, int V> BLSMI_DEV Fp12W fp12_work(const Fp12<L, V>& a) { Fp12W r; r.c0 = fp6_work(a.c0); r.c1 = fp6_work(a.c1); return r; }
+template <int L2, int V2, int L, int V>
+BLSMI_DEV Fp12<L2, V2> fp12_relabel(const Fp12<L, V>& a) { Fp12<L2, V2> r; r.c0 = fp6_relabel<L2, V2>(a.c0); r.c1 = fp6_relabel<L2, V2>(a.c1); return r; }
+BLSMI_DEV Fp12S fp12_widen(const Fp12W& a) { return fp12_relabel<FpS::L, FpS::V>(a); }
 BLSMI_DEV Fp12S fp12_one() { Fp12S r; r.c0 = fp6_one(); r.c1 = fp6_zero(); return r; }
 template <int L, int V> BLSMI_DEV auto fp12_conj(const Fp12<L, V>& a) { return make_fp12(a.c0, fp6_neg(a.c1)); }
 template <int La, int Va, int Lb, int Vb>
@@ -166,49 +185,53 @@
     return Pair<decltype(c0), decltype(c1)>{c0, c1};
 #endif
 }
-BLSMI_DEV Fp12S fp12_cyclotomic_sqr(const Fp12S& f) {
-    const Fp2S z0 = f.c0.c0, z4 = f.c0.c1, z3 = f.c0.c2, z2 = f.c1.c0, z1 = f.c1.c1, z5 = f.c1.c2;
-    Fp12S r;
+BLSMI_DEV Fp12W fp12_cyclotomic_sqr(const Fp12W& f) {
+    const Fp2W z0 = f.c0.c0, z4 = f.c0.c1, z3 = f.c0.c2, z2 = f.c1.c0, z1 = f.c1.c1, z5 = f.c1.c2;
+    Fp12W r;
     const auto a = fp4_sqr(z0, z1);
-    r.c0.c0 = fp2_store(fp2_add(fp2_dbl(fp2_sub(a.first, z0)), a.first));
-    r.c1.c1 = fp2_store(fp2_add(fp2_dbl(fp2_add(a.second, z1)), a.second));
+    r.c0.c0 = fp2_work(fp2_add(fp2_dbl(fp2_sub(a.first, z0)), a.first));
+    r.c1.c1 = fp2_work(fp2_add(fp2_dbl(fp2_add(a.second, z1)), a.second));
     const auto b = fp4_sqr(z2, z3);
     const auto c = fp4_sqr(z4, z5);
-    r.c0.c1 = fp2_store(fp2_add(fp2_dbl(fp2_sub(b.first, z4)), b.first));
-    r.c1.c2 = fp2_store(fp2_add(fp2_dbl(fp2_add(b.second, z5)), b.second));
+    r.c0.c1 = fp2_work(fp2_add(fp2_dbl(fp2_sub(b.first, z4)), b.first));
+    r.c1.c2 = fp2_work(fp2_add(fp2_dbl(fp2_add(b.second, z5)), b.second));
     const auto t3n = fp2_mul_nr(c.second);
-    r.c1.c0 = fp2_store(fp2_add(fp2_dbl(fp2_add(t3n, z2)), t3n));
-    r.c0.c2 = fp2_store(fp2_add(fp2_dbl(fp2_sub(c.first, z3)), c.first));
-    return r;
-}
-struct CycCompressed { Fp2S z2, z3, z4, z5; };
-BLSMI_DEV CycCompressed cyc_compress(const Fp12S& f) {
-    CycCompressed c; c.z4 = f.c0.c1; c.z3 = f.c0.c2; c.z2 = f.c1.c0; c.z5 = f.c1.c2; return c;
-}
-BLSMI_DEV CycCompressed cyc_compressed_sqr(const CycCompressed& g) {
-    CycCompressed r;
+    r.c1.c0 = fp2_work(fp2_add(fp2_dbl(fp2_add(t3n, z2)), t3n));
+    r.c0.c2 = fp2_work(fp2_add(fp2_dbl(fp2_sub(c.first, z3)), c.first));
+    return r;
+}
+template <class F2> struct CycCompressedT { F2 z2, z3, z4, z5; };
+using CycCompressed = CycCompressedT<Fp2S>;
+using CycCompressedW = CycCompressedT<Fp2W>;
+BLSMI_DEV CycCompressedW cyc_compress(const Fp12W& f) {
+    CycCompressedW c; c.z4 = f.c0.c1; c.z3 = f.c0.c2; c.z2 = f.c1.c0; c.z5 = f.c1.c2; return c;
+}
+BLSMI_DEV CycCompressedW cyc_compressed_sqr(const CycCompressedW& g) {
+    CycCompressedW r;
     const auto b = fp4_sqr(g.z2, g.z3);
     const auto c = fp4_sqr(g.z4, g.z5);
-    r.z4 = fp2_store(fp2_add(fp2_dbl(fp2_sub(b.first, g.z4)), b.first));
-    r.z5 = fp2_store(fp2_add(fp2_dbl(fp2_add(b.second, g.z5)), b.second));
+    r.z4 = fp2_work(fp2_add(fp2_dbl(fp2_sub(b.first, g.z4)), b.first));
+    r.z5 = fp2_work(fp2_add(fp2_dbl(fp2_add(b.second, g.z5)), b.second));
     const auto t3n = fp2_mul_nr(c.second);
-    r.z2 = fp2_store(fp2_add(fp2_dbl(fp2_add(t3n, g.z2)), t3n));
-    r.z3 = fp2_store(fp2_add(fp2_dbl(fp2_sub(c.first, g.z3)), c.first));
-    return r;
-}
-BLSMI_DEV void cyc_z1_fraction(const CycCompressed& g, Fp2S& num, Fp2S& den) {
+    r.z2 = fp2_work(fp2_add(fp2_dbl(fp2_add(t3n, g.z2)), t3n));
+    r.z3 = fp2_work(fp2_add(fp2_dbl(fp2_sub(c.first, g.z3)), c.first));
+    return r;
+}
+template <class F2>
+BLSMI_DEV void cyc_z1_fraction(const CycCompressedT<F2>& g, Fp2S& num, Fp2S& den) {
     const i32 z2zero = fp2_is_zero(g.z2) ? -1 : 0;
     const Fp2S n_reg = fp2_store(fp2_sub(fp2_add(fp2_mul_nr(fp2_sqr(g.z5)), fp2_muls<3>(fp2_sqr(g.z4))), fp2_dbl(g.z3)));
     const Fp2S n_alt = fp2_store(fp2_dbl(fp2_mul(g.z4, g.z5)));
     const Fp2S d_reg = fp2_store(fp2_muls<4>(g.z2));
     num = fp2_select(z2zero, n_alt, n_reg);
-    den = fp2_select(z2zero, g.z3, d_reg);
+    den = fp2_select(z2zero, fp2_relabel<FpS::L, FpS::V>(g.z3), d_reg);
     den = fp2_select(fp2_is_zero(den) ? -1 : 0, fp2_one(), den);
 }
-BLSMI_DEV Fp12S cyc_decompress(const CycCompressed& g, const Fp2S& z1) {
-    const Fp2S z0 = fp2_store(fp2_add(fp2_mul_nr(fp2_sub(fp2_add(fp2_dbl(fp2_sqr(z1)), fp2_mul(g.z2, g.z5)), fp2_muls<3>(fp2_mul(g.z3, g.z4)))), fp2_one()));
-    Fp12S r;
-    r.c0.c0 = z0; r.c0.c1 = g.z4; r.c0.c2 = g.z3; r.c1.c0 = g.z2; r.c1.c1 = z1; r.c1.c2 = g.z5;
+template <class F2, int L1, int V1>
+BLSMI_DEV Fp12<F2::L, F2::V> cyc_decompress(const CycCompressedT<F2>& g, const Fp2<L1, V1>& z1) {
+    const F2 z0 = fp2_as<F2>(fp2_add(fp2_mul_nr(fp2_sub(fp2_add(fp2_dbl(fp2_sqr(z1)), fp2_mul(g.z2, g.z5)), fp2_muls<3>(fp2_mul(g.z3, g.z4)))), fp2_one()));
+    Fp12<F2::L, F2::V> r;
+    r.c0.c0 = z0; r.c0.c1 = g.z4; r.c0.c2 = g.z3; r.c1.c0 = g.z2; r.c1.c1 = fp2_as<F2>(z1); r.c1.c2 = g.z5;
     return r;
 }
 template <int La, int Va, int Lb, int Vb>
diff --git a/bls_amd/csrc/tower_fwd.cuh b/bls_amd/csrc/tower_fwd.cuh
--- a/bls_amd/csrc/tower_fwd.cuh
+++ b/bls_amd/csrc/tower_fwd.cuh
@@ -6,4 +6,10 @@
 using Fp2S = Fp2<FpS::L, FpS::V>;
 using Fp6S = Fp6<FpS::L, FpS::V>;
 using Fp12S = Fp12<FpS::L, FpS::V>;
+using Fp2R = Fp2<FpR::L, FpR::V>;
+using Fp6R = Fp6<FpR::L, FpR::V>;
+using Fp12R = Fp12<FpR::L, FpR::V>;
+using Fp2W = Fp2<FpW::L, FpW::V>;
+using Fp6W = Fp6<FpW::L, FpW::V>;
+using Fp12W = Fp12<FpW::L, FpW::V>;
 }
diff --git a/bls_amd/engine.py b/bls_amd/engine.py
--- a/bls_amd/engine.py
+++ b/bls_amd/engine.py
@@ -638,7 +638,7 @@
     return _compress("blsmi_g2_compress_batch", 192, 96, pts, n, in_inf)
 
 
-OPS = dict(FQ_MUL=1, FQ_SQR=2, FQ_ADD=3, FQ_SUB=4, FQ_NEG=5, FQ_INV=6, FQ_SQRT=7, FQ_DBL=8, FQ_CMP=9, FQ_PARITY=10,
+OPS = dict(FQ_MUL=1, FQ_SQR=2, FQ_ADD=3, FQ_SUB=4, FQ_NEG=5, FQ_INV=6, FQ_SQRT=7, FQ_DBL=8, FQ_CMP=9, FQ_PARITY=10, FQ_LAZY=11,
            FQ2_MUL=16, FQ2_SQR=17, FQ2_INV=18, FQ2_MUL_NR=19, FQ2_SQRT=20, FQ2_SQRT_ANY=21, FQ2_PARITY=22,
            FQ6_MUL=32, FQ6_SQR=33, FQ6_INV=34, FQ6_FROB1=35, FQ6_MUL_BY_1=36, FQ6_MUL_BY_01=37,
            FQ12_MUL=48, FQ12_SQR=49, FQ12_INV=50, FQ12_FROB1=51, FQ12_FROB2=52, FQ12_FROB3=53, FQ12_CYCLO_SQR=54, FQ12_CYCLO_RUN16=55,
diff --git a/include/blsmi.h b/include/blsmi.h
--- a/include/blsmi.h
+++ b/include/blsmi.h
@@ -230,6 +230,7 @@
 enum blsmi_debug_op {
     BLSMI_OP_FQ_MUL = 1, BLSMI_OP_FQ_SQR, BLSMI_OP_FQ_ADD, BLSMI_OP_FQ_SUB, BLSMI_OP_FQ_NEG, BLSMI_OP_FQ_INV, BLSMI_OP_FQ_SQRT,
     BLSMI_OP_FQ_DBL , BLSMI_OP_FQ_CMP , BLSMI_OP_FQ_PARITY ,
+    BLSMI_OP_FQ_LAZY ,
     BLSMI_OP_FQ2_MUL = 16, BLSMI_OP_FQ2_SQR, BLSMI_OP_FQ2_INV, BLSMI_OP_FQ2_MUL_NR, BLSMI_OP_FQ2_SQRT, BLSMI_OP_FQ2_SQRT_ANY , BLSMI_OP_FQ2_PARITY ,
     BLSMI_OP_FQ6_MUL = 32, BLSMI_OP_FQ6_SQR, BLSMI_OP_FQ6_INV, BLSMI_OP_FQ6_FROB1,
     BLSMI_OP_FQ6_MUL_BY_1 , BLSMI_OP_FQ6_MUL_BY_01 ,
```

Result: faster. 3.996 million (median of 6 runs) (+2.2%).
